# DeepGraphLearning/ultra_torchdrug

Measured on AMD Instinct MI355X. Metric: edges aggregated/sec, FB15k237-shaped 6L x 64d rspmm Bellman-Ford (predict: the reference's 18 rspmm layers per batch as 6 relation-graph + 6 entity-graph launches, tails and heads in one pass), higher is better.
Workload: dtype f32

## Files before the change

### include/ultra_rspmm.h

```cpp
#ifndef ULTRA_RSPMM_H
#define ULTRA_RSPMM_H

#include <stddef.h>
#include <stdint.h>

#ifdef __cplusplus
extern "C" {
#endif
#pragma GCC visibility push(default)

#define ULTRA_RSPMM_ABI_VERSION 8

enum ultra_sum_op { ULTRA_SUM_ADD = 0, ULTRA_SUM_MIN = 1, ULTRA_SUM_MAX = 2 };
enum ultra_mul_op { ULTRA_MUL_MUL = 0, ULTRA_MUL_ADD = 1 };

enum ultra_status {
    ULTRA_OK = 0,
    ULTRA_ERR_BAD_OP = 1,
    ULTRA_ERR_BAD_SHAPE = 2,
    ULTRA_ERR_NULL_POINTER = 3,
    ULTRA_ERR_WORKSPACE = 4,
    ULTRA_ERR_HIP = 5,
    ULTRA_ERR_NO_DEVICE = 6,
    ULTRA_ERR_ABI = 7
// ... 172 lines not shown
                                void *stream);

int ultra_candidate_tiles(const int64_t *t_index, int64_t n_batch, int64_t per_row, int64_t n_query, int64_t n_rows, int32_t *out,
                          void *stream);

int ultra_gather_boundary_rows_f32(const float *rows, const int32_t *node, int64_t n_query, float *out, void *stream);

int ultra_score_rows_forward_f32(const float *hidden, const float *query, const int64_t *t_index, const float *w1, const float *b1,
                                 const float *w2, const float *b2, float *h, float *in_rows, float *score, int64_t n_batch,
                                 int64_t per_row, void *stream);
int ultra_score_rows_backward_f32(const float *hidden, const float *query, const int64_t *t_index, const float *w1, const float *w2,
                                  const float *h, const float *in_rows, const float *grad, float *d_pre, float *partial,
                                  float *d_hidden, float *d_query, float *d_w1, float *d_b1, float *d_w2, float *d_b2,
                                  int64_t n_node, int64_t n_batch, int64_t per_row, void *stream);

int ultra_statistics_blocks(int64_t n_a);
int ultra_statistics_f32(const float *a, int64_t n_a, const float *b, int64_t n_b, int64_t b_repeat, double *partials,
                         float *out, void *stream);

int ultra_bce_adversarial_f32(const float *pred, int64_t rows, int64_t cols, float temperature, float *loss_rows,
                              float *dpred, void *stream);

int ultra_relation_project_backward_blocks(int device, int64_t batch, int64_t n_rel, int64_t n_layers, int64_t *blocks);
int ultra_relation_project_backward_f32(const float *relation, const float *const *w1, const float *const *b1,
                                        const float *const *w2, const float *const *grad, float *d_relation_layers,
                                        float *const *d_w1, float *const *d_b1, float *const *d_w2, float *const *d_b2,
                                        void *workspace, size_t workspace_bytes, int64_t n_layers, int64_t batch,
                                        int64_t n_rel, int64_t dim, void *stream);

int ultra_filtered_rank(const float *pred, int64_t n_query, int64_t n_cand, int64_t row_stride, const int64_t *target,
                        const int32_t *filt_ptr, const int32_t *filt_node, int64_t *rank, void *stream);


int ultra_filtered_rank_keys(const float *pred, int64_t n_query, int64_t n_cand, int64_t row_stride, const int64_t *target,
                             int64_t target_stride, const int64_t *keys, int64_t n_keys, const int64_t *anchor,
                             const int64_t *rel, int64_t index_stride, int64_t n_rel, int64_t *rank, int64_t rank_stride,
                             void *stream);
int ultra_strict_negative(const int64_t *keys, int64_t n_keys, const int64_t *anchor, const int64_t *rel, int64_t n_query,
                          int64_t n_rel, int64_t n_node, const float *rand, int64_t n_sample, int64_t *out, void *stream);
int ultra_edge_removal_weights(const ultra_segments *fwd, const ultra_segments *by_src, const ultra_segments *by_rel,
                               const int64_t *h, const int64_t *t, const int64_t *r, int64_t n_pattern,
                               int64_t n_base_rel, float *w_fwd, float *w_src, float *w_rel, int64_t slack, void *stream);
int ultra_edge_removal_marks(const ultra_segments *fwd, const ultra_segments *by_src, const ultra_segments *by_rel,
                             const int64_t *h, const int64_t *t, const int64_t *r, int64_t n_pattern, int64_t n_base_rel,
                             float *w_fwd, float *w_src, float *w_rel, int64_t slack, uint32_t *words_fwd, uint32_t *words_src,
                             uint32_t *words_rel, int64_t n_node, void *stream);


size_t ultra_relcsr_coalesce_temp_bytes(int64_t n_edges);
int ultra_relcsr_coalesce(const int64_t *row, const int64_t *col, const int64_t *rel, const float *weight,
                          int64_t n_edges, int64_t n_rows, int64_t n_cols, int64_t n_rel, int32_t *out_row,
                          int32_t *out_col, int32_t *out_rel, float *out_weight, int64_t *edge_of_input,
                          int64_t *n_unique_host, int *unit_weight_host, void *temp, size_t temp_bytes, void *stream);
size_t ultra_relcsr_plan_temp_bytes(int64_t n_edges, int64_t n_rows, int64_t piece_len);
int ultra_relcsr_plan(const int32_t *row, const int32_t *node_a, const int32_t *rel, int64_t n_edges, int64_t n_rows,
                      int64_t n_node_a, int64_t n_rel, int is_relation_plan, int wide_ids, int balance,
                      int64_t chunk_edges, int64_t chunk_rows, int64_t piece_len, int32_t *chunks,
                      int64_t cap_chunks, int32_t *long_rows, int64_t cap_long, int32_t *packed,
                      int64_t packed_slack, int64_t *counts_host, void *temp, size_t temp_bytes, void *stream);

size_t ultra_relcsr_dense_bytes(int64_t n_rows, int64_t n_cols, int kind);
int ultra_relcsr_dense(const ultra_segments *plan, int64_t n_rows, int64_t n_cols, int kind, uint32_t *dense, void *stream);

int ultra_dense_layer_supported(const ultra_segments *fwd, int64_t n_query);
int ultra_dense_layer_forward_f32(const ultra_segments *fwd, const float *relation, const float *input,
                                  const int32_t *boundary_node, const float *boundary_value, int64_t n_query, const float *weight,
                                  const float *bias, const float *ln_weight, const float *ln_bias, float ln_eps, int relu,
                                  int shortcut, float *out, void *stream);

int ultra_layer_forward_supported(const ultra_segments *fwd, int64_t n_query, int64_t n_rel);
int ultra_layer_forward_f32(const ultra_segments *fwd, const float *relation, const float *input, const int32_t *boundary_node,
                            const float *boundary_value, int64_t n_query, const float *weight, const float *bias,
                            const float *ln_weight, const float *ln_bias, float ln_eps, int relu, int shortcut, float *out,
                            int64_t n_rel, void *stream);

int ultra_second_layer_sources(const int32_t *col, int64_t n_edges, int64_t slack, const int32_t *row_list, const int32_t *list_count,
                               int64_t list_len, int64_t n_query, int64_t n_node, uint32_t *bitmap, int32_t *c_node,
                               int32_t *sources, void *stream);
int ultra_layer_forward_sources_f32(const ultra_segments *fwd, const int32_t *sources, const float *relation, const float *input,
                                    const int32_t *boundary_node, const float *boundary_value, int64_t n_query, const float *weight,
                                    const float *bias, const float *ln_weight, const float *ln_bias, float ln_eps, int relu,
                                    int shortcut, float *out, int64_t n_rel, void *stream);

int ultra_layer_score_supported(const ultra_segments *fwd, int64_t n_query, int64_t n_rel);
int ultra_layer_score_forward_f32(const ultra_segments *fwd, const float *relation, const float *input, const int32_t *boundary_node,
                                  const float *boundary_value, int64_t n_query, const float *weight, const float *bias,
                                  const float *ln_weight, const float *ln_bias, float ln_eps, int relu, int shortcut,
                                  const float *query, const float *w1, const float *b1, const float *w2, const float *b2,
                                  float *qbias, float *score, int64_t n_rel, void *stream);

int ultra_relation_graph_marks(const int32_t *head_ptr, const int32_t *head_rel, const int32_t *tail_ptr, const int32_t *tail_rel,
                               int64_t n_node, int64_t n_rel, uint8_t *marks, void *stream);

int ultra_calibrate_gather_f32(const float *table, int64_t n_rows, const int32_t *index, int64_t n_index, float *out,
                               int64_t *n_waves_host, void *stream);

#pragma GCC visibility pop
#ifdef __cplusplus
}
#endif
#endif
```

### ultra_torchdrug_amd/_lib.py

```python
import ctypes
import os

_HERE = os.path.dirname(os.path.abspath(__file__))
LIB_PATH = os.environ.get("ULTRA_RSPMM_LIB") or os.path.join(_HERE, "libultra_rspmm.so")
ABI_VERSION = 8

SUM_OPS = {"add": 0, "min": 1, "max": 2}
MUL_OPS = {"mul": 0, "add": 1}


class UltraSegments(ctypes.Structure):
    _fields_ = [
        ("struct_bytes", ctypes.c_uint32),
        ("abi_version", ctypes.c_uint32),
        ("n_rows", ctypes.c_int64),
        ("n_edges", ctypes.c_int64),
        ("row", ctypes.c_void_p),
        ("node_a", ctypes.c_void_p),
        ("node_b", ctypes.c_void_p),
        ("rel", ctypes.c_void_p),
        ("weight", ctypes.c_void_p),
        ("n_chunks", ctypes.c_int64),
        ("chunks", ctypes.c_void_p),
        ("n_long_rows", ctypes.c_int64),
# ... 11 lines not shown
        ("packed_dead", ctypes.c_void_p),
    ]

    def __init__(self, *args, **kwargs):
        super().__init__(*args, **kwargs)
        if not self.struct_bytes:
            self.struct_bytes = ctypes.sizeof(type(self))
        if not self.abi_version:
            self.abi_version = ABI_VERSION


EXPORTS = (
    "ultra_rspmm_abi_version",
    "ultra_segments_bytes",
    "ultra_rspmm_status_string",
    "ultra_rspmm_last_hip_error",
    "ultra_rspmm_device_info",
    "ultra_rspmm_profile_next",
    "ultra_rspmm_event_create",
    "ultra_rspmm_event_destroy",
    "ultra_rspmm_event_elapsed_ms",
    "ultra_rspmm_force_general_path",
    "ultra_rspmm_reserve_cus",
    "ultra_rspmm_workspace_bytes",
    "ultra_rspmm_forward_f32",
    "ultra_rspmm_fwd_f32",
    "ultra_rspmm_forward_boundary_f32",
    "ultra_rspmm_frontier_f32",
    "ultra_first_layer_sparse_supported",
    "ultra_first_layer_sparse_f32",
    "ultra_rspmm_backward_boundary_rows_f32",
    "ultra_rspmm_backward_boundary_rows_workspace",
    "ultra_rspmm_backward_f32",
    "ultra_rspmm_backward_accumulate_f32",
    "ultra_rspmm_backward_weight_f32",
    "ultra_beam_search_step_f32",
    "ultra_rspmm_backward_active_f32",
    "ultra_node_bitmap",
    "ultra_rspmm_drelation_boundary_f32",
    "ultra_combine_forward_f32",
    "ultra_combine_forward_boundary_f32",
    "ultra_combine_backward_waves",
    "ultra_combine_backward_f32",
    "ultra_combine_dxdu_f32",
    "ultra_combine_backward_fused_waves",
    "ultra_combine_backward_fused_f32",
    "ultra_linear_forward_f32",
    "ultra_score_forward_f32",
    "ultra_relation_project_f32",
    "ultra_relation_project_backward_blocks",
    "ultra_relation_project_backward_f32",
    "ultra_filtered_rank",
    "ultra_filtered_rank_keys",
    "ultra_strict_negative",
    "ultra_edge_removal_weights",
    "ultra_edge_removal_marks",
    "ultra_prepare_queries",
    "ultra_relation_stack_inputs",
    "ultra_statistics_blocks",
    "ultra_statistics_f32",
    "ultra_bce_adversarial_f32",
    "ultra_candidate_tiles",
    "ultra_score_rows_forward_f32",
    "ultra_score_rows_backward_f32",
    "ultra_gather_boundary_rows_f32",
    "ultra_relcsr_coalesce_temp_bytes",
    "ultra_relcsr_coalesce",
    "ultra_relcsr_plan_temp_bytes",
    "ultra_relcsr_plan",
    "ultra_relcsr_dense_bytes",
    "ultra_relcsr_dense",
    "ultra_relation_graph_marks",
    "ultra_calibrate_gather_f32",
    "ultra_first_layer_sparse_train_f32",
    "ultra_first_layer_epilogue_backward_workspace",
    "ultra_first_layer_epilogue_backward_f32",
    "ultra_column_sum_blocks",
    "ultra_column_sum_f32",
    "ultra_dense_layer_supported",
    "ultra_dense_layer_forward_f32",
    "ultra_layer_forward_supported",
    "ultra_layer_forward_f32",
    "ultra_second_layer_sources",
    "ultra_layer_forward_sources_f32",
    "ultra_layer_score_supported",
    "ultra_layer_score_forward_f32",
)

_lib = None


class UltraLibraryError(RuntimeError):
    pass


def load():
    global _lib
    if _lib is not None:
        return _lib
    if not os.path.exists(LIB_PATH):
        raise UltraLibraryError(
            "%s not found: build it with `make -C ultra_torchdrug_amd/csrc` (hipcc --offload-arch=gfx950) or "
            "`python -c 'import __graft_entry__ as g; g.build()'`. There is no CPU/PyTorch fallback." % LIB_PATH)
    try:
        lib = ctypes.CDLL(LIB_PATH)
    except OSError as err:
        raise UltraLibraryError("cannot load %s: %s" % (LIB_PATH, err)) from err
    missing = [name for name in EXPORTS if not hasattr(lib, name)]
    if missing:
        raise UltraLibraryError("%s lacks symbols %s" % (LIB_PATH, missing))

    vp, i64, i32, sz = ctypes.c_void_p, ctypes.c_int64, ctypes.c_int, ctypes.c_size_t
    seg = ctypes.POINTER(UltraSegments)
    lib.ultra_rspmm_abi_version.restype = i32
    lib.ultra_rspmm_abi_version.argtypes = []
    lib.ultra_layer_forward_supported.restype = i32
    lib.ultra_layer_forward_supported.argtypes = [seg, i64, i64]
    lib.ultra_layer_forward_f32.restype = i32
    lib.ultra_layer_forward_f32.argtypes = [seg, vp, vp, vp, vp, i64, vp, vp, vp, vp, ctypes.c_float, i32, i32, vp, i64, vp]
    lib.ultra_second_layer_sources.restype = i32
    lib.ultra_second_layer_sources.argtypes = [vp, i64, i64, vp, vp, i64, i64, i64, vp, vp, vp, vp]
    lib.ultra_layer_forward_sources_f32.restype = i32
    lib.ultra_layer_forward_sources_f32.argtypes = [seg, vp, vp, vp, vp, vp, i64, vp, vp, vp, vp, ctypes.c_float, i32, i32, vp, i64, vp]
    lib.ultra_layer_score_supported.restype = i32
    lib.ultra_layer_score_supported.argtypes = [seg, i64, i64]
    lib.ultra_layer_score_forward_f32.restype = i32
    lib.ultra_layer_score_forward_f32.argtypes = [seg, vp, vp, vp, vp, i64, vp, vp, vp, vp, ctypes.c_float, i32, i32, vp, vp, vp, vp,
                                                  vp, vp, vp, i64, vp]
    lib.ultra_relation_graph_marks.restype = i32
    lib.ultra_relation_graph_marks.argtypes = [vp, vp, vp, vp, i64, i64, vp, vp]
    lib.ultra_segments_bytes.restype = sz
    lib.ultra_segments_bytes.argtypes = []
    lib.ultra_rspmm_status_string.restype = ctypes.c_char_p
    lib.ultra_rspmm_status_string.argtypes = [i32]
    lib.ultra_rspmm_last_hip_error.restype = i32
    lib.ultra_rspmm_last_hip_error.argtypes = []
    lib.ultra_rspmm_device_info.restype = i32
    lib.ultra_rspmm_device_info.argtypes = [i32, ctypes.POINTER(i32), ctypes.POINTER(i32), ctypes.c_char_p, sz]
    lib.ultra_rspmm_profile_next.restype = i32
    lib.ultra_rspmm_profile_next.argtypes = [vp, vp]
    lib.ultra_rspmm_event_create.restype = i32
    lib.ultra_rspmm_event_create.argtypes = [ctypes.POINTER(vp)]
    lib.ultra_rspmm_event_destroy.restype = i32
    lib.ultra_rspmm_event_destroy.argtypes = [vp]
    lib.ultra_rspmm_event_elapsed_ms.restype = i32
    lib.ultra_rspmm_event_elapsed_ms.argtypes = [vp, vp, ctypes.POINTER(ctypes.c_float)]
    lib.ultra_rspmm_force_general_path.restype = i32
    lib.ultra_rspmm_force_general_path.argtypes = [i32]
    lib.ultra_rspmm_reserve_cus.restype = i32
    lib.ultra_rspmm_reserve_cus.argtypes = [i32]
    lib.ultra_rspmm_workspace_bytes.restype = sz
    lib.ultra_rspmm_workspace_bytes.argtypes = [seg, i64]
    lib.ultra_rspmm_forward_f32.restype = i32
    lib.ultra_rspmm_forward_f32.argtypes = [seg, vp, vp, vp, vp, vp, sz, i64, i64, i64, i32, i32, vp]
    lib.ultra_rspmm_fwd_f32.restype = i32
    lib.ultra_rspmm_fwd_f32.argtypes = [vp, vp, vp, vp, vp, vp, vp, i64, i64, i64, i64, i32, i32, vp]
    lib.ultra_rspmm_forward_boundary_f32.restype = i32
    lib.ultra_rspmm_forward_boundary_f32.argtypes = [seg, vp, vp, vp, vp, i64, vp, vp, sz, i64, i64, i64, i32, i32, vp]
    lib.ultra_rspmm_backward_boundary_rows_f32.restype = i32
    lib.ultra_rspmm_backward_boundary_rows_f32.argtypes = [seg, vp, vp, vp, vp, vp, vp, sz, i64, i64, i64, i32, vp]
    lib.ultra_rspmm_backward_boundary_rows_workspace.restype = sz
    lib.ultra_rspmm_backward_boundary_rows_workspace.argtypes = [i64]
    lib.ultra_rspmm_frontier_f32.restype = i32
    lib.ultra_rspmm_frontier_f32.argtypes = [seg, vp, vp, vp, vp, vp, i64, vp, i64, i64, i64, vp]
    lib.ultra_first_layer_sparse_supported.restype = i32
    lib.ultra_first_layer_sparse_supported.argtypes = [i64, i64, i64]
    lib.ultra_first_layer_sparse_f32.restype = i32
    lib.ultra_first_layer_sparse_f32.argtypes = [seg, vp, vp, vp, vp, vp, vp, i64, vp, vp, vp, vp, ctypes.c_float, i32, i32, vp, vp, i64, i64,
                                                 vp, i64, i64, vp]
    lib.ultra_rspmm_backward_f32.restype = i32
    lib.ultra_rspmm_backward_f32.argtypes = [seg, seg, vp, vp, vp, vp, vp, vp, vp, sz, i64, i64, i64, i64, i32, i32, vp]
    lib.ultra_rspmm_backward_accumulate_f32.restype = i32
    lib.ultra_rspmm_backward_accumulate_f32.argtypes = [seg, seg, vp, vp, vp, vp, vp, vp, vp, vp, sz, i64, i64, i64, i64, i32,
                                                        i32, vp]
    lib.ultra_rspmm_backward_active_f32.restype = i32
    lib.ultra_rspmm_backward_active_f32.argtypes = [seg, seg, vp, vp, vp, vp, vp, vp, vp, sz, i64, i64, i64, i64, i32, vp, i64, vp, vp]
    lib.ultra_node_bitmap.restype = i32
    lib.ultra_node_bitmap.argtypes = [vp, i64, i64, i64, vp, vp]
    lib.ultra_rspmm_drelation_boundary_f32.restype = i32
    lib.ultra_rspmm_drelation_boundary_f32.argtypes = [seg, vp, i64, vp, vp, vp, vp, vp, vp, vp, sz, i64, i64, i64, vp]
    lib.ultra_rspmm_backward_weight_f32.restype = i32
    lib.ultra_rspmm_backward_weight_f32.argtypes = [seg, vp, vp, vp, vp, vp, i64, i64, i32, i32, vp]
    lib.ultra_beam_search_step_f32.restype = i32
    lib.ultra_beam_search_step_f32.argtypes = [vp, vp, vp, vp, i64, i64, i64, i64, vp, vp, vp, vp]
    lib.ultra_combine_forward_f32.restype = i32
    lib.ultra_combine_forward_f32.argtypes = [vp, vp, vp, vp, vp, vp, ctypes.c_float, i32, i32, vp, vp, i64, i64, vp]
    lib.ultra_combine_forward_boundary_f32.restype = i32
    lib.ultra_combine_forward_boundary_f32.argtypes = [vp, vp, i64, vp, vp, vp, vp, vp, ctypes.c_float, i32, i32, vp, i64, i64, vp]
    lib.ultra_prepare_queries.restype = i32
    lib.ultra_prepare_queries.argtypes = [vp, vp, i64, i64, i64, i64, i64, vp, vp, vp, vp, vp]
    lib.ultra_statistics_blocks.restype = i32
    lib.ultra_statistics_blocks.argtypes = [i64]
    lib.ultra_statistics_f32.restype = i32
    lib.ultra_statistics_f32.argtypes = [vp, i64, vp, i64, i64, vp, vp, vp]
    lib.ultra_gather_boundary_rows_f32.restype = i32
    lib.ultra_gather_boundary_rows_f32.argtypes = [vp, vp, i64, vp, vp]
    lib.ultra_score_rows_forward_f32.restype = i32
    lib.ultra_score_rows_forward_f32.argtypes = [vp] * 10 + [i64, i64, vp]
    lib.ultra_score_rows_backward_f32.restype = i32
    lib.ultra_score_rows_backward_f32.argtypes = [vp] * 16 + [i64, i64, i64, vp]
    lib.ultra_candidate_tiles.restype = i32
    lib.ultra_candidate_tiles.argtypes = [vp, i64, i64, i64, i64, vp, vp]
    lib.ultra_bce_adversarial_f32.restype = i32
    lib.ultra_bce_adversarial_f32.argtypes = [vp, i64, i64, ctypes.c_float, vp, vp, vp]
# ... 90 lines not shown
```

### ultra_torchdrug_amd/csrc/frontier.inc

```

struct FrontierParams {
    const int32_t *src_ptr;
    const int32_t *dst;
    const int32_t *rel;
    const float *weight;
    const int32_t *fwd_rank;
    const float *relation;
    const int32_t *bnode;
    const float *bvec;
    float *out;
    long long F;
    int piece_len;
    int slices;
    int n_rel;
    int piece_shift;
    const int32_t *run_prefix;
    int32_t *row_list;
    const int32_t *list_offset;
    int list_len;
};

constexpr int kFrontierThreads = 256;
constexpr int kFrontierU = 4;

// ... 229 lines not shown
        r = p.rel[eu];
        k = p.fwd_rank[eu];
        w = 1.0f;
        if constexpr (!UNIT_W) w = p.weight[eu];
    };
    const int bp = (lane & 48) * 4;
    const int grp_shift = (lane >> 4) * 16;
    auto from = [&](int u, int v) -> int { return __builtin_amdgcn_ds_bpermute(bp + 4 * u, v); };

    int nd, nr, nk;
    float nw;
    load_ids(e, nd, nr, nk, nw);
    bool done = false;
    while (!done) {
        const int md = nd, mr = nr, mk = nk;
        const float mw = nw;
        load_ids(e + 16, nd, nr, nk, nw);
        const int mp = p.piece_shift >= 0 ? (mk >> p.piece_shift) : (mk / p.piece_len);
        const int prev_d = __builtin_amdgcn_update_dpp(cur, md, 0x111, 0xf, 0xf, false);
        const int prev_p = __builtin_amdgcn_update_dpp(cur_piece, mp, 0x111, 0xf, 0xf, false);
        const int n_valid = min(16, hi - e);
        const bool starts_run = (md != prev_d) && sub < n_valid;
        const bool starts_piece = (starts_run || mp != prev_p) && sub < n_valid;
        const uint32_t run_bits = (uint32_t)(__builtin_amdgcn_ballot_w64(starts_run) >> grp_shift) & 0xffffu;
        const uint32_t piece_bits = (uint32_t)(__builtin_amdgcn_ballot_w64(starts_piece) >> grp_shift) & 0xffffu;
        const int room = end - e;
        const uint32_t beyond = room >= 16 ? 0u : (room <= 0 ? 0xffffu : (0xffffu << room) & 0xffffu);
        const uint32_t stop_bits = run_bits & beyond;
        const int n_sum = min(n_valid, stop_bits ? __builtin_ctz(stop_bits) : 16);
        done = n_sum < 16;
#pragma unroll
        for (int half = 0; half < 2; ++half) {
            qf4 y[8];
#pragma unroll
            for (int v = 0; v < 8; ++v) {
                const int u = 8 * half + v;
                y[v] = msg[from(u, mr) * 16];
                if constexpr (!UNIT_W) y[v] = __builtin_bit_cast(float, from(u, __builtin_bit_cast(int, mw))) * y[v];
            }
            const uint32_t any = (run_bits | piece_bits) >> (8 * half) & 0xffu;
            if (any == 0u && n_sum >= 8 * half + 8) {
#pragma unroll
                for (int v = 0; v < 8; ++v) piece = piece + y[v];
                continue;
            }
#pragma unroll
            for (int v = 0; v < 8; ++v) {
                const int u = 8 * half + v;
                if (u < n_sum) {
                    if ((run_bits >> u) & 1u) {
                        close_run(u == 0 ? cur : from(u - 1, md));
                        have_total = false;
                        open = false;
                    }
                    if ((piece_bits >> u) & 1u) {
                        close_piece();
                        open = true;
                        piece = qf4{0.0f, 0.0f, 0.0f, 0.0f};
                    }
                    piece = piece + y[v];
                }
            }
        }
        if (n_sum > 0) {
            cur = from(n_sum - 1, md);
            cur_piece = from(n_sum - 1, mp);
        }
        e += 16;
    }
    close_run(cur);
}

constexpr int kSparseMaxQueries = 128;
struct ConstFillParams {
    qf4 *out;
    long long n4;
    const float *bias, *gamma, *beta;
    float eps;
    int relu, shortcut;
    const int32_t *src_ptr, *run_prefix, *bnode;
    int n_query;
    int list_len;
    int32_t *list_offset;
};

__global__ __launch_bounds__(256) void const_fill_kernel(const ConstFillParams p) {
    __shared__ __attribute__((aligned(16))) float c[64];
    __shared__ int slots[kSparseMaxQueries];
    if (threadIdx.x < 64) {
        const int j = threadIdx.x;
        float v = p.bias[j];
        if (p.gamma != nullptr) {
            float s0 = 0.0f, s1 = 0.0f;
            for (int k = 0; k < 32; ++k) { s0 = s0 + p.bias[k]; s1 = s1 + p.bias[32 + k]; }
            const float mean = (s0 + s1) * (1.0f / 64.0f);
            float q0 = 0.0f, q1 = 0.0f;
            for (int k = 0; k < 32; ++k) {
                const float d0 = p.bias[k] - mean, d1 = p.bias[32 + k] - mean;
                q0 = q0 + d0 * d0;
                q1 = q1 + d1 * d1;
            }
            const float var = (q0 + q1) * (1.0f / 64.0f);
            const float inv = 1.0f / sqrtf(var + p.eps);
            v = ((v - mean) * inv) * p.gamma[j] + p.beta[j];
        }
        if (p.relu) v = !(v <= 0.0f) ? v : 0.0f;
        c[j] = p.shortcut ? v + 0.0f : v;
    }
    if (blockIdx.x == 0) {
        if ((int)threadIdx.x < p.n_query) {
            const int h = p.bnode[threadIdx.x];
            const int lo = p.src_ptr[h], hi = p.src_ptr[h + 1];
            slots[threadIdx.x] = (hi > lo ? p.run_prefix[hi - 1] - p.run_prefix[lo] + 1 : 0) + 1;
        }
        __syncthreads();
        if (threadIdx.x == 0) {
            int total = 0;
            for (int b = 0; b < p.n_query; ++b) {
                p.list_offset[b] = total;
                total += slots[b];
            }
            p.list_offset[p.n_query] = total;
        }
    }
    __syncthreads();
    const qf4 *c4 = reinterpret_cast<const qf4 *>(c);
    for (long long i = (long long)blockIdx.x * 256 + threadIdx.x; i < p.n4; i += (long long)gridDim.x * 256) p.out[i] = c4[i & 15];
}

__global__ __launch_bounds__(256) void zero_fill_kernel(qf4 *out, long long n4) {
    const qf4 zero = {0.0f, 0.0f, 0.0f, 0.0f};
    for (long long i = (long long)blockIdx.x * 256 + threadIdx.x; i < n4; i += (long long)gridDim.x * 256) out[i] = zero;
}

struct BoundaryRowsParams {
    const int32_t *src_ptr;
    const int32_t *dst;
    const int32_t *rel;
    const float *weight;
    const float *relation;
    const float *grad;
    const int32_t *bnode;
    float *partial;
    float *d_input;
    long long F;
};

constexpr int kBRowsSlices = 64;
constexpr int kBRowsWaves = kBRowsSlices * 4;

template <bool UNIT_W, bool HAS_REL>
__global__ __launch_bounds__(256) void boundary_rows_partial_kernel(const BoundaryRowsParams p) {
    const int lane = threadIdx.x & 63;
    const int g = blockIdx.x * 4 + uniform(threadIdx.x >> 6);
    const int q = blockIdx.y;
    const int u = uniform(p.bnode[q]);
    const int lo = uniform(p.src_ptr[u]), hi = uniform(p.src_ptr[u + 1]);
    const int per = (hi - lo + kBRowsWaves - 1) / kBRowsWaves;
    const int a = lo + g * per;
    const int z = a + per < hi ? a + per : hi;
    const long long col = (long long)q * 64 + lane;
    float acc = 0.0f;
    auto ids = [&](int e0, int &v, int &r, float &wt) {
        int e = e0 + (lane & 7);
        e = e < z ? e : z - 1;
        v = p.dst[e];
        r = 0;
        if constexpr (HAS_REL) r = p.rel[e];
        wt = 1.0f;
        if constexpr (!UNIT_W) wt = p.weight[e];
    };
    int v = 0, r = 0;
    float wt = 1.0f;
    if (a < z) ids(a, v, r, wt);
    for (int e0 = a; e0 < z; e0 += 8) {
        int v_next = 0, r_next = 0;
        float wt_next = 1.0f;
        if (e0 + 8 < z) ids(e0 + 8, v_next, r_next, wt_next);
        float gr[8], rr[8];
#pragma unroll
        for (int k = 0; k < 8; ++k) {
            const long long vk = __builtin_amdgcn_readlane(v, k);
            gr[k] = p.grad[vk * p.F + col];
            rr[k] = 1.0f;
            if constexpr (HAS_REL) rr[k] = p.relation[(long long)__builtin_amdgcn_readlane(r, k) * p.F + col];
        }
#pragma unroll
        for (int k = 0; k < 8; ++k) {
            if (e0 + k < z) {
                float y = gr[k];
                if constexpr (!UNIT_W) y = y * __builtin_bit_cast(float, __builtin_amdgcn_readlane(__builtin_bit_cast(int, wt), k));
                if constexpr (HAS_REL) y = y * rr[k];
                acc = acc + y;
            }
        }
        v = v_next; r = r_next; wt = wt_next;
    }
    p.partial[((long long)q * kBRowsWaves + g) * 64 + lane] = acc;
}

__global__ __launch_bounds__(64) void boundary_rows_reduce_kernel(const BoundaryRowsParams p) {
    const int lane = threadIdx.x;
    const int q = blockIdx.x;
    const float *part = p.partial + (long long)q * kBRowsWaves * 64 + lane;
    float total = 0.0f;
#pragma unroll 16
    for (int g = 0; g < kBRowsWaves; ++g) total = total + part[g * 64];
    float *dst = p.d_input + (long long)p.bnode[q] * p.F + (long long)q * 64 + lane;
    *dst = *dst + total;
}
// ... 1 lines not shown
```

### ultra_torchdrug_amd/csrc/quad.inc

```
#ifndef ULTRA_QUAD_WORD_AUX
#define ULTRA_QUAD_WORD_AUX 0
#endif
#ifndef ULTRA_QUAD_STORE_AUX
#define ULTRA_QUAD_STORE_AUX 2
#endif
#ifndef ULTRA_QUAD_DEDUP
#define ULTRA_QUAD_DEDUP 0
#endif
typedef float qf4 __attribute__((ext_vector_type(4)));
typedef uint32_t qu4 __attribute__((ext_vector_type(4)));
typedef __attribute__((address_space(3))) const qf4 *lds_qf4_ptr;
typedef __attribute__((address_space(3))) char *lds_char_ptr;

__device__ __forceinline__ qf4 lds_read4(uint32_t byte_addr) { return *(lds_qf4_ptr)byte_addr; }

template <int RED>
__device__ __forceinline__ qf4 reduce4(qf4 a, qf4 y) {
    if constexpr (RED == ULTRA_SUM_ADD) {
        return a + y;
    } else {
        qf4 r;
        r.x = reduce<RED>(a.x, y.x); r.y = reduce<RED>(a.y, y.y); r.z = reduce<RED>(a.z, y.z); r.w = reduce<RED>(a.w, y.w);
        return r;
    }
}

template <int RED>
__device__ __forceinline__ qf4 identity4() {
    const float v = identity<RED>();
    qf4 r = {v, v, v, v};
    return r;
}

typedef __attribute__((address_space(3))) const uint32_t *lds_u32_ptr;
__device__ __forceinline__ uint32_t lds_read1(uint32_t byte_addr) { return *(lds_u32_ptr)byte_addr; }

template <int KIND, int SUM, int MUL, bool UNIT_W, bool X_LDS, int U, int ACT = 0, bool DEAD = false>
__global__ __launch_bounds__(kBlock) void quad_kernel(const PParams p) {
    static_assert(KIND == KIND_FWD || SUM == ULTRA_SUM_ADD, "quad path: forward, or the backward of sum-aggregation");
    static_assert(!DEAD || (UNIT_W && !X_LDS && SUM == ULTRA_SUM_ADD && MUL == ULTRA_MUL_MUL && ACT != 1),
                  "marked words: unit weights, gathers through descriptors, summed DistMult messages");
    static_assert(ACT == 0 || (!X_LDS && ((KIND == KIND_DX && ACT == 1) || (KIND == KIND_DREL && (ACT == 2 || ACT == 3)))),
                  "activity masks: d_input by destination, d_relation by destination or by the tile's source node");
    constexpr int RED = (KIND == KIND_FWD) ? SUM : ULTRA_SUM_ADD;
    constexpr bool TWO_GATHERS = (KIND == KIND_DREL);
    constexpr bool DIRECT_WORDS = X_LDS && !TWO_GATHERS;
    constexpr bool NEEDS_REL = (KIND == KIND_FWD) || (KIND == KIND_DX && MUL == ULTRA_MUL_MUL);
    extern __shared__ __attribute__((aligned(16))) float lds_raw[];
    int *ticket = reinterpret_cast<int *>(lds_raw);
    float *lds_rel = lds_raw + kLdsHeader / sizeof(float);
    const int lane = threadIdx.x & 63;
    const int grp = lane >> 4;
    const uint32_t lane_bytes = (uint32_t)(lane & 15) * 16u;
    const int label = blockIdx.x % kXcd;
    const int conc = p.concurrent > 1 ? p.concurrent : 1;
    const int team = (int)(blockIdx.x / kXcd) % conc;
    const int bl = (int)(blockIdx.x / kXcd) / conc;
    const int nb = p.blocks_per_label / conc;
    const long long F = p.F;
    const __amdgpu_buffer_rsrc_t rsrc =
        __builtin_amdgcn_make_buffer_rsrc(const_cast<float *>(p.gather), 0, p.gather_bytes, 0x00020000);
    const __amdgpu_buffer_rsrc_t rsrc_meta =
        __builtin_amdgcn_make_buffer_rsrc(const_cast<uint32_t *>(p.meta), 0, p.meta_bytes, 0x00020000);
    const __amdgpu_buffer_rsrc_t rsrc2 =
        __builtin_amdgcn_make_buffer_rsrc(const_cast<float *>(TWO_GATHERS ? p.gather2 : p.gather), 0,
                                          TWO_GATHERS ? p.gather2_bytes : 0u, 0x00020000);
    const __amdgpu_buffer_rsrc_t rsrc_meta2 =
        __builtin_amdgcn_make_buffer_rsrc(const_cast<uint32_t *>(TWO_GATHERS ? p.meta2 : p.meta), 0,
                                          TWO_GATHERS ? p.meta2_bytes : 0u, 0x00020000);
    const __amdgpu_buffer_rsrc_t rsrc_out = __builtin_amdgcn_make_buffer_rsrc(p.out, 0, p.out_bytes, 0x00020000);
    const __amdgpu_buffer_rsrc_t rsrc_add =
        __builtin_amdgcn_make_buffer_rsrc(const_cast<float *>(p.add_rows != nullptr ? p.add_rows : p.out), 0,
                                          p.add_rows != nullptr ? p.out_bytes : 0u, 0x00020000);
    const __amdgpu_buffer_rsrc_t rsrc_wt =
        __builtin_amdgcn_make_buffer_rsrc(const_cast<float *>(UNIT_W ? p.gather : p.weight), 0, UNIT_W ? 0u : p.meta_bytes, 0x00020000);
    if ((uint32_t)(uintptr_t)(lds_char_ptr)lds_raw != 0u) __builtin_trap();

    for (int s = label + kXcd * team; s < p.n_slots; s += kXcd * conc) {
        const int tile = s / p.split;
        const int part = s - tile * p.split;
        const long long col = (long long)tile * kTile + (lane & 15) * 4;
        const bool active = col < F;
        const uint32_t voff = (uint32_t)((active ? col : 0) * 4);
        float *lds_x = lds_rel + (NEEDS_REL ? p.n_rel * kTile : 0);
        if constexpr (NEEDS_REL) {
            const int total = p.n_rel * kTile;
            for (int i = threadIdx.x; i < total; i += kBlock) {
                const int r = i >> 6;
                const long long c = (long long)tile * kTile + (i & 63);
                lds_rel[i] = (c < F) ? p.relation[(long long)r * F + c] : 0.0f;
            }
        }
        if constexpr (X_LDS) {
            const int total = p.n_gather_rows * kTile;
            for (int i = threadIdx.x; i < total; i += kBlock) {
                const int r = i >> 6;
                const long long c = (long long)tile * kTile + (i & 63);
                lds_x[i] = (c < F) ? p.gather[(long long)r * F + c] : 0.0f;
            }
        }
        int b_node = -1;
        qf4 b_val = {0.0f, 0.0f, 0.0f, 0.0f};
        if (KIND == KIND_FWD && p.bnode != nullptr && active) {
            b_node = p.bnode[col / p.bdim];
            b_val = *reinterpret_cast<const qf4 *>(p.bvec + col);
        }
        int act_node = -1;
        if constexpr (ACT == 1 || ACT == 2) {
            uint32_t *lds_act = reinterpret_cast<uint32_t *>(lds_x);
            const uint32_t *bits = p.act_bits + (long long)tile * p.act_words;
            for (int i = threadIdx.x; i < p.act_words; i += kBlock) lds_act[i] = bits[i];
        }
        if constexpr (ACT == 3) act_node = p.act_node[tile];
        if (threadIdx.x == 0) *ticket = 0;
        __syncthreads();
        const uint32_t rel_base = (uint32_t)kLdsHeader;
        const uint32_t x_base = rel_base + (NEEDS_REL ? (uint32_t)p.n_rel * 256u : 0u);
        auto dead = [&](uint32_t key) -> uint32_t {
            if constexpr (ACT == 1 || ACT == 2) return ((lds_read1(x_base + (key >> 5) * 4u) >> (key & 31u)) & 1u) ? 0u : 0xffffffffu;
            if constexpr (ACT == 3) return (int)key == act_node ? 0u : 0xffffffffu;
            return 0u;
        };

        for (;;) {
            int t = 0;
            if (lane == 0) t = __hip_atomic_fetch_add(ticket, 1, __ATOMIC_RELAXED, __HIP_MEMORY_SCOPE_WORKGROUP);
            t = uniform(t);
            const int k_first = part + p.split * (4 * t * nb + bl);
            if (k_first >= p.n_chunks) break;
            const int q = 4 * t + grp;
            const int k = part + p.split * (q * nb + ((q & 1) ? (nb - 1 - bl) : bl));
            const bool has = k < p.n_chunks;
            int4 d = {0, 0, 0, 0};
            if (has) d = p.chunks[k];
            const int n = d.y - d.x;
            const uint32_t e_begin = (uint32_t)d.x;
            const bool is_piece = d.w < 0;
            const int row_base = d.z;
            const int n01 = max(__builtin_amdgcn_readlane(n, 0), __builtin_amdgcn_readlane(n, 16));
            const int n23 = max(__builtin_amdgcn_readlane(n, 32), __builtin_amdgcn_readlane(n, 48));
            const int m01 = min(__builtin_amdgcn_readlane(n, 0), __builtin_amdgcn_readlane(n, 16));
            const int m23 = min(__builtin_amdgcn_readlane(n, 32), __builtin_amdgcn_readlane(n, 48));
            const int n_max = uniform(max(n01, n23)), n_min = uniform(min(m01, m23));
            const uint32_t e_bytes = e_begin * 4u;

            uint32_t cur = 0;
            qf4 acc = identity4<RED>();
            const bool adds = (KIND != KIND_DREL) && p.add_rows != nullptr;
            const bool sparse_b = (KIND == KIND_FWD) && p.add_rows == nullptr && p.bnode != nullptr;
            const uint32_t base_off = (uint32_t)row_base * p.row_bytes + voff;
            auto load_add = [&](uint32_t off) -> qf4 {
                return __builtin_bit_cast(qf4, __builtin_amdgcn_raw_buffer_load_b128(rsrc_add, off, 0, 0));
            };

            auto store_row = [&](uint32_t dl, qf4 v) {
                if (active) {
                    if (adds) v = reduce4<RED>(v, load_add(base_off + __umul24(dl, p.row_bytes)));
                    if (sparse_b) v = reduce4<RED>(v, (row_base + (int)dl == b_node) ? b_val : qf4{0.0f, 0.0f, 0.0f, 0.0f});
                    __builtin_amdgcn_raw_buffer_store_b128(__builtin_bit_cast(qu4, v), rsrc_out, base_off + __umul24(dl, p.row_bytes), 0, ULTRA_QUAD_STORE_AUX);
                }
            };
            auto store_empty = [&](uint32_t dl) {
                if (active) {
                    const uint32_t off = base_off + dl * p.row_bytes;
                    qf4 v = identity4<RED>();
                    if (adds) v = reduce4<RED>(v, load_add(off));
                    if (sparse_b) v = reduce4<RED>(v, (row_base + (int)dl == b_node) ? b_val : qf4{0.0f, 0.0f, 0.0f, 0.0f});
                    __builtin_amdgcn_raw_buffer_store_b128(__builtin_bit_cast(qu4, v), rsrc_out, off, 0, ULTRA_QUAD_STORE_AUX);
                }
            };
            auto contribute = [&](qf4 a, qf4 rv, qf4 gv, float w) -> qf4 {
                if constexpr (KIND == KIND_FWD) {
                    qf4 y;
                    if constexpr (MUL == ULTRA_MUL_MUL) y = rv * gv; else y = rv + gv;
                    if constexpr (!UNIT_W) y = w * y;
                    return reduce4<RED>(a, y);
                } else {
                    qf4 c = gv;
                    if constexpr (!UNIT_W) c = c * w;
                    if constexpr (MUL == ULTRA_MUL_MUL) c = c * rv;
                    return a + c;
                }
            };
            const float ident = identity<RED>();
            auto next_row = [&](uint32_t dl) {
                store_row(cur, acc);
                for (uint32_t r = cur + 1; r < dl; ++r) store_empty(r);
                asm volatile("v_mov_b32 %0, %1" : "+v"(cur) : "v"(dl));
                asm volatile("v_mov_b32 %0, %1" : "+v"(acc.x) : "v"(ident));
                asm volatile("v_mov_b32 %0, %1" : "+v"(acc.y) : "v"(ident));
                asm volatile("v_mov_b32 %0, %1" : "+v"(acc.z) : "v"(ident));
                asm volatile("v_mov_b32 %0, %1" : "+v"(acc.w) : "v"(ident));
            };

            const uint32_t lane_word = (uint32_t)min(lane & 15, U - 1) * 4u;
            const int bp_base = (lane & 48) * 4;
            auto load_compact = [&](int i, uint32_t &m, uint32_t &m2) {
                const uint32_t off = e_bytes + (uint32_t)i * 4u + lane_word;
                m = __builtin_amdgcn_raw_buffer_load_b32(rsrc_meta, off, 0, ULTRA_QUAD_WORD_AUX);
                m2 = 0;
                if constexpr (TWO_GATHERS) m2 = __builtin_amdgcn_raw_buffer_load_b32(rsrc_meta2, off, 0, 0);
            };
            auto distribute = [&](uint32_t m, uint32_t m2, uint32_t (&w)[U], uint32_t (&w2)[U]) {
#pragma unroll
                for (int u = 0; u < U; ++u) {
                    w[u] = (uint32_t)__builtin_amdgcn_ds_bpermute(bp_base + 4 * u, (int)m);
                    w2[u] = 0;
                    if constexpr (TWO_GATHERS) w2[u] = (uint32_t)__builtin_amdgcn_ds_bpermute(bp_base + 4 * u, (int)m2);
                }
            };
            auto load_words = [&](int i, uint32_t (&w)[U], uint32_t (&w2)[U]) {
                const uint32_t w_off = e_bytes + (uint32_t)i * 4u;
#pragma unroll
                for (int u = 0; u < U; ++u) {
                    w[u] = __builtin_amdgcn_raw_buffer_load_b32(rsrc_meta, w_off + 4u * u, 0, ULTRA_QUAD_WORD_AUX);
                    w2[u] = 0;
                }
            };
            uint32_t wn[U], w2n[U];
            uint32_t mw = 0, mw2 = 0;
            constexpr bool DEDUP = ULTRA_QUAD_DEDUP && !TWO_GATHERS && !X_LDS && ACT == 0 && !DEAD;
            uint32_t prev_node = 0xffffffffu;
            qu4 prev_x = {0u, 0u, 0u, 0u};
            if constexpr (DIRECT_WORDS) {
                load_words(0, wn, w2n);
            } else {
                load_compact(0, mw, mw2);
                distribute(mw, mw2, wn, w2n);
                load_compact(U, mw, mw2);
            }

            auto batch = [&](auto tail_tag, int i) {
                constexpr bool TAIL = decltype(tail_tag)::value;
                uint32_t w[U], w2[U];
                float wt[U];
                qf4 xv[U], rv[U];
                uint32_t killm[U];
#pragma unroll
                for (int u = 0; u < U; ++u) { w[u] = wn[u]; w2[u] = w2n[u]; killm[u] = 0u; }
#pragma unroll
                for (int u = 0; u < U; ++u) {
                    const uint32_t node = w[u] >> p.src_shift;
                    if constexpr (TWO_GATHERS) {
                        uint32_t kill = 0u;
                        if constexpr (ACT == 2) kill = dead(w2[u]);
                        if constexpr (ACT == 3) kill = dead(node);
                        if constexpr (DEAD) kill |= (uint32_t)((int32_t)w[u] >> 31);
                        xv[u] = __builtin_bit_cast(qf4, __builtin_amdgcn_raw_buffer_load_b128(
                                                            rsrc2, (__umul24(w2[u], p.row_bytes) + voff) | kill, 0, 0));
                        rv[u] = qf4{0.0f, 0.0f, 0.0f, 0.0f};
                        if constexpr (MUL == ULTRA_MUL_MUL) {
                            if constexpr (X_LDS)
                                rv[u] = lds_read4(((node << 8) | lane_bytes) + x_base);
                            else
                                rv[u] = __builtin_bit_cast(qf4, __builtin_amdgcn_raw_buffer_load_b128(
                                                                    rsrc, (__umul24(node, p.row_bytes) + voff) | kill, 0, 0));
                        }
                        continue;
                    }
                    if constexpr (X_LDS) {
                        xv[u] = lds_read4(((node << 8) | lane_bytes) + x_base);
                    } else {
                        uint32_t kill = 0u;
                        if constexpr (ACT == 1) kill = dead(node);
                        if constexpr (DEAD) kill = (uint32_t)((int32_t)w[u] >> 31);
                        if constexpr (DEDUP) {
                            const uint32_t before = (u == 0) ? prev_node : (w[u > 0 ? u - 1 : 0] >> p.src_shift);
                            kill = (node == before) ? 0xffffffffu : 0u;
                            killm[u] = kill;
                        }
                        xv[u] = __builtin_bit_cast(qf4, __builtin_amdgcn_raw_buffer_load_b128(
                                                            rsrc, (__umul24(node, p.row_bytes) + voff) | kill, 0, 0));
                    }
                    if constexpr (NEEDS_REL)
                        rv[u] = lds_read4(((w[u] & p.rel_mask) | lane_bytes) + rel_base);
                    else
                        rv[u] = qf4{0.0f, 0.0f, 0.0f, 0.0f};
                }
                if constexpr (!UNIT_W && !DIRECT_WORDS) {
                    const int mine = (int)__builtin_amdgcn_raw_buffer_load_b32(rsrc_wt, e_bytes + (uint32_t)i * 4u + lane_word, 0, 0);
#pragma unroll
                    for (int u = 0; u < U; ++u) wt[u] = __builtin_bit_cast(float, __builtin_amdgcn_ds_bpermute(bp_base + 4 * u, mine));
                } else {
#pragma unroll
                    for (int u = 0; u < U; ++u) {
                        wt[u] = 1.0f;
                        if constexpr (!UNIT_W)
                            wt[u] = __builtin_bit_cast(float, __builtin_amdgcn_raw_buffer_load_b32(
                                                                  rsrc_wt, e_bytes + (uint32_t)i * 4u + 4u * u, 0, 0));
                    }
                }
                if constexpr (DIRECT_WORDS) {
                    if (i + U < n_max) load_words(i + U, wn, w2n);
                } else {
                    const uint32_t m = mw, m2 = mw2;
                    load_compact(i + 2 * U, mw, mw2);
                    distribute(m, m2, wn, w2n);
                }
                if constexpr (DEDUP) {
#pragma unroll
                    for (int u = 0; u < U; ++u) {
                        const qu4 before = (u == 0) ? prev_x : __builtin_bit_cast(qu4, xv[u > 0 ? u - 1 : 0]);
                        const qu4 got = __builtin_bit_cast(qu4, xv[u]);
                        qu4 v;
                        v.x = (before.x & killm[u]) | got.x; v.y = (before.y & killm[u]) | got.y;
                        v.z = (before.z & killm[u]) | got.z; v.w = (before.w & killm[u]) | got.w;
                        xv[u] = __builtin_bit_cast(qf4, v);
                    }
                    prev_x = __builtin_bit_cast(qu4, xv[U - 1]);
                    prev_node = w[U - 1] >> p.src_shift;
                }
                bool same_row = false;
                if constexpr (!TAIL) same_row = __builtin_amdgcn_ballot_w64((w[U - 1] & 0xffu) != cur) == 0ull;
                if (same_row) {
#pragma unroll
                    for (int u = 0; u < U; ++u) acc = contribute(acc, rv[u], xv[u], wt[u]);
                } else {
#pragma unroll
                    for (int u = 0; u < U; ++u) {
                        const bool valid = !TAIL || (i + u < n);
                        const uint32_t dl = w[u] & 0xffu;
                        if (valid) {
                            if (dl != cur) next_row(dl);
                            acc = contribute(acc, rv[u], xv[u], wt[u]);
                        }
                    }
                }
            };

            int i = 0;
            for (; i + U <= n_min; i += U) batch(std::false_type{}, i);
            for (; i < n_max; i += U) batch(std::true_type{}, i);

            if (has) {
                if (is_piece) {
                    if (active) *reinterpret_cast<qf4 *>(p.partial + (long long)(-d.w - 1) * F + col) = acc;
                } else {
                    store_row(cur, acc);
                    for (uint32_t r = cur + 1; r < (uint32_t)(d.w - row_base); ++r) store_empty(r);
                }
            }
        }
        __syncthreads();
    }
}
```

### ultra_torchdrug_amd/csrc/rspmm_kernels.hip

```cpp
#include <hip/hip_runtime.h>
#include <type_traits>

#include <algorithm>
#include <cstdint>
#include <cstdlib>
#include <cstring>
#include <mutex>

#include "relgraph_dense.h"
#include "ultra_rspmm.h"

thread_local int ultra_detail_last_hip_error = 0;

namespace {

constexpr int kTile = 64;
#ifndef ULTRA_BLOCK
#define ULTRA_BLOCK 1024
#endif
constexpr int kBlock = ULTRA_BLOCK;
#ifndef ULTRA_UNROLL
#define ULTRA_UNROLL 8
#endif
constexpr int kUnroll = ULTRA_UNROLL;
#ifndef ULTRA_UNROLL_BIG
#define ULTRA_UNROLL_BIG 8
#endif
#ifndef ULTRA_BIG_GATHER_AUX
#define ULTRA_BIG_GATHER_AUX 0
#endif
constexpr int kUnrollBig = ULTRA_UNROLL_BIG;
constexpr int kXcd = 8;
constexpr int kFixUnroll = 16;
constexpr int kMaxLdsBytes = 156 * 1024;
constexpr int kLdsHeader = 16;

enum Kind { KIND_FWD = 0, KIND_DX = 1, KIND_DREL = 2 };

struct KParams {
    const int32_t *row;
    const int32_t *node_a;
    const int32_t *node_b;
    const int32_t *rel;
    const float *weight;
    const int4 *chunks;
    const float *relation;
    const float *input;
    const float *output;
    const float *grad;
    const float *add_rows;
    const int32_t *bnode;
    const float *bvec;
    int bdim;
    float *out;
    float *partial;
    long long F;
    int n_chunks;
    int n_rel;
    int n_tiles;
    int split;
    int n_slots;
    int blocks_per_label;
    const uint32_t *act_bits;
    int act_words;
    const int32_t *act_node;
};

struct FixParams {
    const int32_t *long_rows;
    const float *partial;
    const float *add_rows;
    const int32_t *bnode;
    const float *bvec;
    int bdim;
    float *out;
    long long F;
    int n_long;
    int n_tiles;
};

template <int SUM>
__device__ __forceinline__ float identity() {
    if constexpr (SUM == ULTRA_SUM_ADD) return 0.0f;
    else if constexpr (SUM == ULTRA_SUM_MIN) return 3.402823466e+38f;
    else return -3.402823466e+38f;
}

template <int SUM>
__device__ __forceinline__ float reduce(float acc, float y) {
    if constexpr (SUM == ULTRA_SUM_ADD) return acc + y;
    else if constexpr (SUM == ULTRA_SUM_MIN) return (y < acc) ? y : acc;
    else return (y > acc) ? y : acc;
}

template <int MUL>
__device__ __forceinline__ float binary(float r, float x) {
    if constexpr (MUL == ULTRA_MUL_MUL) return r * x;
    else return r + x;
}

__device__ __forceinline__ int uniform(int v) { return __builtin_amdgcn_readfirstlane(v); }

template <int KIND, int SUM, int MUL, bool UNIT_W, bool REL_LDS>
struct ChunkWalker {
    static constexpr int RED = (KIND == KIND_FWD) ? SUM : ULTRA_SUM_ADD;
    static constexpr bool MASKED = (KIND != KIND_FWD) && (SUM != ULTRA_SUM_ADD);
    static constexpr bool NEED_REL_ID = (KIND == KIND_FWD) || (KIND == KIND_DX && (MASKED || MUL == ULTRA_MUL_MUL));

    const KParams &p;
    const long long F;
    const long long col;
    const long long lcol;
    const bool active;
    const float *lds_rel;
    const int lane;
    int cur;
    float acc;
    bool is_piece;

    __device__ __forceinline__ float load_rel(int r) const {
        if constexpr (REL_LDS) return lds_rel[r * kTile + lane];
        else return p.relation[(long long)r * F + lcol];
    }
    __device__ __forceinline__ void store_row(int r, float v) const {
        if (active) {
            if constexpr (KIND != KIND_DREL) {
                if (p.add_rows != nullptr) v = reduce<RED>(v, p.add_rows[(long long)r * F + col]);
                else if (KIND == KIND_FWD && p.bnode != nullptr) v = reduce<RED>(v, (r == p.bnode[col / p.bdim]) ? p.bvec[col] : 0.0f);
            }
            p.out[(long long)r * F + col] = v;
        }
    }

    template <bool FULL>
    __device__ __forceinline__ void batch(const int e0, const int n) {
        int ia[kUnroll], ib[kUnroll], ir[kUnroll], irow[kUnroll];
        float wv[kUnroll];
        float v0[kUnroll], v1[kUnroll], v2[kUnroll];
#pragma unroll
        for (int u = 0; u < kUnroll; ++u) {
            const int e = FULL ? e0 + u : e0 + min(u, n - 1);
            ia[u] = p.node_a[e];
            irow[u] = p.row[e];
            if constexpr (NEED_REL_ID) ir[u] = p.rel[e];
            if constexpr (KIND == KIND_DREL) ib[u] = p.node_b[e];
            if constexpr (!UNIT_W) wv[u] = p.weight[e];
        }
#pragma unroll
// ... 60 lines not shown
            store_row(cur, acc);
            for (int q = cur + 1; q < d.w; ++q) store_row(q, identity<RED>());
        }
    }
};

template <int KIND, int SUM, int MUL, bool UNIT_W, bool REL_LDS>
__global__ __launch_bounds__(kBlock) void segment_kernel(const KParams p) {
    extern __shared__ __attribute__((aligned(16))) float lds_raw[];
    int *ticket = reinterpret_cast<int *>(lds_raw);
    float *lds_rel = lds_raw + kLdsHeader / sizeof(float);
    const int lane = threadIdx.x & 63;
    const int label = blockIdx.x % kXcd;
    const int bl = blockIdx.x / kXcd;
    const int nb = p.blocks_per_label;

    for (int s = label; s < p.n_slots; s += kXcd) {
        const int tile = s / p.split;
        const int part = s - tile * p.split;
        const long long col = (long long)tile * kTile + lane;
        const bool active = col < p.F;
        if constexpr (REL_LDS) {
            const int total = p.n_rel * kTile;
            for (int i = threadIdx.x; i < total; i += kBlock) {
                const int r = i >> 6;
                const long long c = (long long)tile * kTile + (i & 63);
                lds_rel[i] = (c < p.F) ? p.relation[(long long)r * p.F + c] : 0.0f;
            }
        }
        if (threadIdx.x == 0) *ticket = 0;
        __syncthreads();
        for (;;) {
            int t = 0;
            if (lane == 0) t = __hip_atomic_fetch_add(ticket, 1, __ATOMIC_RELAXED, __HIP_MEMORY_SCOPE_WORKGROUP);
            t = uniform(t);
            const int k = part + p.split * (t * nb + ((t & 1) ? (nb - 1 - bl) : bl));
            if (k >= p.n_chunks) break;
            const int4 d = p.chunks[uniform(k)];
            ChunkWalker<KIND, SUM, MUL, UNIT_W, REL_LDS> walker{p, p.F, col, active ? col : p.F - 1, active, lds_rel, lane,
                                                                0, 0.0f, false};
            walker.run(d);
        }
        __syncthreads();
    }
}

struct PParams {
    const uint32_t *meta;
    const uint32_t *meta2;
    const float *weight;
    const int4 *chunks;
    const float *relation;
    const float *gather;
    const float *gather2;
    const float *add_rows;
    const int32_t *bnode;
    const float *bvec;
    int bdim;
    float *out;
    float *partial;
    long long F;
    uint32_t gather_bytes;
    uint32_t meta_bytes;
    uint32_t meta2_bytes;
    uint32_t out_bytes;
    uint32_t gather2_bytes;
    uint32_t relation_bytes;
    int n_gather_rows;
    const int32_t *hot_nodes;
    int n_hot;
    uint32_t row_bytes;
    uint32_t src_shift;
    uint32_t rel_mask;
    int n_chunks;
    int n_rel;
    int n_tiles;
    int split;
    int n_slots;
    int blocks_per_label;
    int concurrent;
    const uint32_t *act_bits;
    int act_words;
    const int32_t *act_node;
};

template <int KIND, int SUM, int MUL, bool UNIT_W, int VAR, int UN = kUnroll>
__global__ __launch_bounds__(kBlock) void packed_kernel(const PParams p) {
    constexpr bool X_LDS = (VAR == 1);
    constexpr bool BIG = (VAR == 2 || VAR == 3);
    constexpr bool REL_GLOBAL = (VAR == 2);
    constexpr bool HOT = (VAR == 4);
    static_assert(VAR == 0 || KIND != KIND_DREL, "variants 1-4 are for the single-gather kinds");
    static_assert(KIND == KIND_FWD || SUM == ULTRA_SUM_ADD, "packed path: forward, or the backward of sum-aggregation");
    constexpr int RED = (KIND == KIND_FWD) ? SUM : ULTRA_SUM_ADD;
    constexpr bool NEEDS_REL = (KIND == KIND_FWD) || (KIND == KIND_DX && MUL == ULTRA_MUL_MUL);
    constexpr bool TWO_GATHERS = (KIND == KIND_DREL);
    extern __shared__ __attribute__((aligned(16))) float lds_raw[];
    int *ticket = reinterpret_cast<int *>(lds_raw);
    float *lds_rel = lds_raw + kLdsHeader / sizeof(float);
    const int lane = threadIdx.x & 63;
    const int label = blockIdx.x % kXcd;
    const int bl = blockIdx.x / kXcd;
    const int nb = p.blocks_per_label;
    const long long F = p.F;
    const __amdgpu_buffer_rsrc_t rsrc =
        __builtin_amdgcn_make_buffer_rsrc(const_cast<float *>(p.gather), 0, p.gather_bytes, 0x00020000);
    const __amdgpu_buffer_rsrc_t rsrc2 =
        __builtin_amdgcn_make_buffer_rsrc(const_cast<float *>(TWO_GATHERS ? p.gather2 : p.gather), 0,
                                          TWO_GATHERS ? p.gather2_bytes : p.gather_bytes, 0x00020000);
    const __amdgpu_buffer_rsrc_t rsrc_rel =
        __builtin_amdgcn_make_buffer_rsrc(const_cast<float *>(p.relation), 0, p.relation_bytes, 0x00020000);

    for (int s = label; s < p.n_slots; s += kXcd) {
        const int tile = s / p.split;
        const int part = s - tile * p.split;
        const long long col = (long long)tile * kTile + lane;
        const bool active = col < F;
        const uint32_t voff = (uint32_t)((active ? col : F - 1) * 4);
        float *lds_x = lds_rel + (NEEDS_REL ? p.n_rel * kTile : 0);
        if constexpr (NEEDS_REL && !REL_GLOBAL) {
            const int total = p.n_rel * kTile;
            for (int i = threadIdx.x; i < total; i += kBlock) {
                const int r = i >> 6;
                const long long c = (long long)tile * kTile + (i & 63);
                lds_rel[i] = (c < F) ? p.relation[(long long)r * F + c] : 0.0f;
            }
        }
        if constexpr (X_LDS) {
            const int total = p.n_gather_rows * kTile;
            for (int i = threadIdx.x; i < total; i += kBlock) {
                const int r = i >> 6;
                const long long c = (long long)tile * kTile + (i & 63);
                lds_x[i] = (c < F) ? p.gather[(long long)r * F + c] : 0.0f;
            }
        }
        if constexpr (HOT) {
            const int total = p.n_hot * kTile;
            for (int i = threadIdx.x; i < total; i += kBlock) {
                const long long r = p.hot_nodes[i >> 6];
                const long long c = (long long)tile * kTile + (i & 63);
                lds_x[i] = (c < F) ? p.gather[r * F + c] : 0.0f;
            }
        }
        if (threadIdx.x == 0) *ticket = 0;
        __syncthreads();
        const char *lds_lane = reinterpret_cast<const char *>(lds_rel) + lane * 4;
        const char *lds_x_lane = reinterpret_cast<const char *>(lds_x) + lane * 4;
        auto gather_one = [&](uint32_t word) -> float {
            if constexpr (X_LDS) {
                return *reinterpret_cast<const float *>(lds_x_lane + ((word >> p.src_shift) << 8));
            } else if constexpr (HOT) {
                const uint32_t g = word >> p.src_shift;
                if (g < (uint32_t)p.n_hot) return *reinterpret_cast<const float *>(lds_x_lane + (g << 8));
                return __builtin_bit_cast(float, __builtin_amdgcn_raw_buffer_load_b32(
                                                     rsrc, voff, (g - (uint32_t)p.n_hot) * p.row_bytes, 0));
            } else {
                return __builtin_bit_cast(float, __builtin_amdgcn_raw_buffer_load_b32(
                                                     rsrc, voff, (word >> p.src_shift) * p.row_bytes, 0));
            }
        };

        int b_node = -1;
        float b_val = 0.0f;
        if (KIND == KIND_FWD && p.bnode != nullptr && active) {
            b_node = p.bnode[col / p.bdim];
            b_val = p.bvec[col];
// ... 157 lines not shown
    const int row = p.long_rows[lr * 3 + 0];
    const int first = p.long_rows[lr * 3 + 1];
    const int n = p.long_rows[lr * 3 + 2];
    float acc = identity<RED>();
    for (int k0 = 0; k0 < n; k0 += UN) {
        float v[UN];
#pragma unroll
        for (int u = 0; u < UN; ++u) {
            const int k = min(k0 + u, n - 1);
            v[u] = p.partial[(long long)(first + k) * p.F + col];
        }
#pragma unroll
        for (int u = 0; u < UN; ++u)
            if (k0 + u < n) acc = reduce<RED>(acc, v[u]);
    }
    if (p.add_rows != nullptr) acc = reduce<RED>(acc, p.add_rows[(long long)row * p.F + col]);
    else if (p.bnode != nullptr) acc = reduce<RED>(acc, (row == p.bnode[col / p.bdim]) ? p.bvec[col] : 0.0f);
    p.out[(long long)row * p.F + col] = acc;
}

#include "quad.inc"
#include "frontier.inc"
#include "rowgroup.inc"

template <int SUM, int MUL, bool UNIT_W>
__global__ __launch_bounds__(256) void weight_grad_kernel(const int32_t *row, const int32_t *src, const int32_t *rel,
                                                          const float *weight, const float *relation,
                                                          const float *input, const float *output, const float *grad,
                                                          float *d_weight, long long F, long long n_edges) {
    const int lane = threadIdx.x & 63;
    const long long waves_total = ((long long)gridDim.x * blockDim.x) >> 6;
    long long e = ((long long)blockIdx.x * blockDim.x + threadIdx.x) >> 6;
    for (; e < n_edges; e += waves_total) {
        const int v = row[e], u = src[e], r = rel[e];
        float wk = 1.0f;
        if constexpr (!UNIT_W) wk = weight[e];
        float acc = 0.0f;
        for (long long f = lane; f < F; f += 64) {
            const float m = binary<MUL>(relation[(long long)r * F + f], input[(long long)u * F + f]);
            float g = grad[(long long)v * F + f];
            if constexpr (SUM != ULTRA_SUM_ADD) {
                float y = m;
                if constexpr (!UNIT_W) y = wk * m;
                g = g * ((output[(long long)v * F + f] == y) ? 1.0f : 0.0f);
            }
            acc = acc + g * m;
        }
#pragma unroll
        for (int off = 32; off > 0; off >>= 1) acc += __shfl_down(acc, off, 64);
        if (lane == 0) d_weight[e] = acc;
    }
}


constexpr int kCbRows = 32;
constexpr int kCbStride = 132;
constexpr int kCbWaves = 4;
constexpr int kCbTileFloats = kCbRows * kCbStride;
constexpr int kCbLdsQueries = 128;
static_assert(kCbLdsQueries == kSparseMaxQueries, "const_fill_kernel lays out one slot range per LDS-resident query");

typedef float f32x4 __attribute__((ext_vector_type(4)));
typedef float f32x16 __attribute__((ext_vector_type(16)));

struct CombineParams {
    const float *input;
    const float *update;
    const float *weight;
    const float *bias;
    const float *gamma;
    const float *beta;
    float *out;
    long long rows;
    float eps;
    int relu;
    int shortcut;
    float *z_out;
    const int32_t *in_bnode;
    const float *in_bvec;
    int rpn;
    const int32_t *row_list;
    const int32_t *list_count;
    int list_len;
};

template <bool PF, int BND = 0, bool ZOUT = false>
__global__ __launch_bounds__(kCbWaves * 64, PF ? 1 : 2) void combine_kernel(const CombineParams p) {
    extern __shared__ __attribute__((aligned(16))) float cb_lds[];
    const int lane = threadIdx.x & 63;
    const int wl = uniform(threadIdx.x >> 6);
    float *tile = cb_lds + wl * kCbTileFloats;
    const int i = lane & 31, h = lane >> 5;
    int n_list = 0;
    if constexpr (BND == 3) n_list = min(uniform(p.list_count[0]), p.list_len);
    const long long n_tiles = BND == 3 ? ((long long)n_list + kCbRows - 1) / kCbRows : (p.rows + kCbRows - 1) / kCbRows;
    const long long wave_global = (long long)blockIdx.x * kCbWaves + wl;
    const long long wave_total = (long long)gridDim.x * kCbWaves;

    float w0[64], w1[64];
#pragma unroll
    for (int q = 0; q < 16; ++q) {
        const f32x4 a = *reinterpret_cast<const f32x4 *>(p.weight + (long long)i * 128 + 64 * h + 4 * q);
        const f32x4 b = *reinterpret_cast<const f32x4 *>(p.weight + (long long)(i + 32) * 128 + 64 * h + 4 * q);
        w0[4 * q + 0] = a.x; w0[4 * q + 1] = a.y; w0[4 * q + 2] = a.z; w0[4 * q + 3] = a.w;
        w1[4 * q + 0] = b.x; w1[4 * q + 1] = b.y; w1[4 * q + 2] = b.z; w1[4 * q + 3] = b.w;
    }
    const float bias0 = p.bias[i], bias1 = p.bias[i + 32];
    const int ln_row = lane >> 1, ln_half = lane & 1;
    float *gb = cb_lds + kCbWaves * kCbTileFloats;
    if (p.gamma != nullptr && threadIdx.x < 128) gb[threadIdx.x] = threadIdx.x < 64 ? p.gamma[threadIdx.x] : p.beta[threadIdx.x - 64];
    float *bv_lds = gb + 128;
    int *bn_lds = reinterpret_cast<int *>(bv_lds + (size_t)p.rpn * 64);
    if constexpr (BND == 1 || BND == 3) {
        for (int j = threadIdx.x; j < p.rpn; j += kCbWaves * 64) bn_lds[j] = p.in_bnode[j];
        for (int j = threadIdx.x; j < p.rpn * 16; j += kCbWaves * 64)
            reinterpret_cast<f32x4 *>(bv_lds)[j] = reinterpret_cast<const f32x4 *>(p.in_bvec)[j];
    }
    __syncthreads();

    const long long last = p.rows - 1;
    f32x4 pa[8], pb[8];
    int rid[8];
    auto fetch = [&](long long t) {
        if constexpr (BND == 3) {
#pragma unroll
            for (int q = 0; q < 8; ++q) {
                const int r = 4 * q + (lane >> 4), c = (lane & 15) * 4;
                const long long slot = t * kCbRows + r;
                int row = slot < n_list ? p.row_list[slot] : -1;
                if ((long long)row >= p.rows) row = -1;
                rid[q] = row;
                const unsigned gr = row >= 0 ? (unsigned)row : 0u;
                const unsigned node = gr / (unsigned)p.rpn, query = gr - node * (unsigned)p.rpn;
                const f32x4 zero = {0.0f, 0.0f, 0.0f, 0.0f};
                const f32x4 v = *reinterpret_cast<const f32x4 *>(bv_lds + query * 64 + c);
                pa[q] = ((int)node == bn_lds[query]) ? v : zero;
                pb[q] = *reinterpret_cast<const f32x4 *>(p.update + (long long)gr * 64 + c);
            }
            return;
        }
        long long node0 = 0;
        int query0 = 0;
        if constexpr (BND != 0) {
            node0 = (t * kCbRows) / p.rpn;
            query0 = (int)(t * kCbRows - node0 * p.rpn);
        }
#pragma unroll
        for (int q = 0; q < 8; ++q) {
            const int r = 4 * q + (lane >> 4), c = (lane & 15) * 4;
            long long gr = t * kCbRows + r;
            gr = gr < last ? gr : last;
            if constexpr (BND == 0) {
                pa[q] = *reinterpret_cast<const f32x4 *>(p.input + gr * 64 + c);
            } else {
                const unsigned qq = (unsigned)(query0 + r);
                const unsigned step = p.rpn >= kCbRows ? (qq >= (unsigned)p.rpn ? 1u : 0u) : qq / (unsigned)p.rpn;
                const int query = (int)(qq - step * (unsigned)p.rpn);
                const f32x4 zero = {0.0f, 0.0f, 0.0f, 0.0f};
                if constexpr (BND == 1) {
                    const f32x4 v = *reinterpret_cast<const f32x4 *>(bv_lds + query * 64 + c);
                    pa[q] = (node0 + step == (long long)bn_lds[query]) ? v : zero;
                } else {
                    pa[q] = (node0 + step == (long long)p.in_bnode[query]) ? *reinterpret_cast<const f32x4 *>(p.in_bvec + query * 64 + c) : zero;
                }
            }
            pb[q] = *reinterpret_cast<const f32x4 *>(p.update + gr * 64 + c);
        }
    };
    if constexpr (PF) {
        if (wave_global < n_tiles) fetch(wave_global);
    }
    for (long long t = wave_global; t < n_tiles; t += wave_total) {
        const long long row0 = t * kCbRows;
        if constexpr (!PF) fetch(t);
#pragma unroll
        for (int q = 0; q < 8; ++q) {
            const int r = 4 * q + (lane >> 4), c = (lane & 15) * 4;
            *reinterpret_cast<f32x4 *>(tile + r * kCbStride + c) = pa[q];
            *reinterpret_cast<f32x4 *>(tile + r * kCbStride + 64 + c) = pb[q];
        }
        if constexpr (PF) {
            asm volatile("s_waitcnt lgkmcnt(0)" ::: "memory");
            if (t + wave_total < n_tiles) fetch(t + wave_total);
        } else {
            asm volatile("s_waitcnt vmcnt(0) lgkmcnt(0)" ::: "memory");
        }

        f32x16 acc0, acc1;
#pragma unroll
        for (int r = 0; r < 16; ++r) { acc0[r] = bias0; acc1[r] = bias1; }
#pragma unroll
        for (int q = 0; q < 16; ++q) {
            const f32x4 av = *reinterpret_cast<const f32x4 *>(tile + i * kCbStride + 64 * h + 4 * q);
            acc0 = __builtin_amdgcn_mfma_f32_32x32x2f32(av.x, w0[4 * q + 0], acc0, 0, 0, 0);
            acc1 = __builtin_amdgcn_mfma_f32_32x32x2f32(av.x, w1[4 * q + 0], acc1, 0, 0, 0);
            acc0 = __builtin_amdgcn_mfma_f32_32x32x2f32(av.y, w0[4 * q + 1], acc0, 0, 0, 0);
            acc1 = __builtin_amdgcn_mfma_f32_32x32x2f32(av.y, w1[4 * q + 1], acc1, 0, 0, 0);
            acc0 = __builtin_amdgcn_mfma_f32_32x32x2f32(av.z, w0[4 * q + 2], acc0, 0, 0, 0);
            acc1 = __builtin_amdgcn_mfma_f32_32x32x2f32(av.z, w1[4 * q + 2], acc1, 0, 0, 0);
            acc0 = __builtin_amdgcn_mfma_f32_32x32x2f32(av.w, w0[4 * q + 3], acc0, 0, 0, 0);
            acc1 = __builtin_amdgcn_mfma_f32_32x32x2f32(av.w, w1[4 * q + 3], acc1, 0, 0, 0);
        }
        asm volatile("s_waitcnt lgkmcnt(0)" ::: "memory");

#pragma unroll
        for (int r = 0; r < 16; ++r) {
            const int row = (r & 3) + 8 * (r >> 2) + 4 * h;
            tile[row * kCbStride + 64 + i] = acc0[r];
            tile[row * kCbStride + 96 + i] = acc1[r];
        }
        asm volatile("s_waitcnt lgkmcnt(0)" ::: "memory");

        float v[32];
#pragma unroll
        for (int q = 0; q < 8; ++q) {
            const f32x4 d = *reinterpret_cast<const f32x4 *>(tile + ln_row * kCbStride + 64 + 32 * ln_half + 4 * q);
            v[4 * q + 0] = d.x; v[4 * q + 1] = d.y; v[4 * q + 2] = d.z; v[4 * q + 3] = d.w;
            if constexpr (ZOUT) {
                const long long left_z = p.rows - row0;
                const __amdgpu_buffer_rsrc_t rsrc_z = __builtin_amdgcn_make_buffer_rsrc(
                    p.z_out + row0 * 64, 0, (int)(left_z < kCbRows ? left_z : kCbRows) * 256, 0x00020000);
                __builtin_amdgcn_raw_buffer_store_b128(__builtin_bit_cast(qu4, d), rsrc_z, ln_row * 256 + ln_half * 128 + 16 * q, 0, 0);
            }
        }
        if (p.gamma != nullptr) {
            float s = 0.0f;
#pragma unroll
            for (int c = 0; c < 32; ++c) s = s + v[c];
            const float so = __shfl_xor(s, 1, 64);
            const float mean = (ln_half == 0 ? s + so : so + s) * (1.0f / 64.0f);
            float ss = 0.0f;
#pragma unroll
            for (int c = 0; c < 32; ++c) { const float dlt = v[c] - mean; ss = ss + dlt * dlt; }
            const float sso = __shfl_xor(ss, 1, 64);
            const float var = (ln_half == 0 ? ss + sso : sso + ss) * (1.0f / 64.0f);
            const float inv = 1.0f / sqrtf(var + p.eps);
#pragma unroll
            for (int q = 0; q < 8; ++q) {
                const f32x4 gq = *reinterpret_cast<const f32x4 *>(gb + 32 * ln_half + 4 * q);
                const f32x4 bq = *reinterpret_cast<const f32x4 *>(gb + 64 + 32 * ln_half + 4 * q);
                v[4 * q + 0] = ((v[4 * q + 0] - mean) * inv) * gq.x + bq.x;
                v[4 * q + 1] = ((v[4 * q + 1] - mean) * inv) * gq.y + bq.y;
                v[4 * q + 2] = ((v[4 * q + 2] - mean) * inv) * gq.z + bq.z;
                v[4 * q + 3] = ((v[4 * q + 3] - mean) * inv) * gq.w + bq.w;
            }
        }
        if (p.relu) {
#pragma unroll
            for (int c = 0; c < 32; ++c) v[c] = !(v[c] <= 0.0f) ? v[c] : 0.0f;
// ... 167 lines not shown
            if (rel_lds) return launch_instance<KIND, SUM, MUL, true, true>(p, grid, lds, stream);
            return launch_instance<KIND, SUM, MUL, true, false>(p, grid, lds, stream);
        }
        if (rel_lds) return launch_instance<KIND, SUM, MUL, false, true>(p, grid, lds, stream);
        return launch_instance<KIND, SUM, MUL, false, false>(p, grid, lds, stream);
    }
}

template <int KIND>
int launch_ops(const KParams &p, int sum_op, int mul_op, bool unit_w, bool rel_lds, int grid, size_t lds,
               hipStream_t stream) {
#define ULTRA_CASE(S, M)                                                    \
    if (sum_op == S && mul_op == M) return launch_wl<KIND, S, M>(p, unit_w, rel_lds, grid, lds, stream);
    ULTRA_CASE(ULTRA_SUM_ADD, ULTRA_MUL_MUL)
    ULTRA_CASE(ULTRA_SUM_ADD, ULTRA_MUL_ADD)
    ULTRA_CASE(ULTRA_SUM_MIN, ULTRA_MUL_MUL)
    ULTRA_CASE(ULTRA_SUM_MIN, ULTRA_MUL_ADD)
    ULTRA_CASE(ULTRA_SUM_MAX, ULTRA_MUL_MUL)
    ULTRA_CASE(ULTRA_SUM_MAX, ULTRA_MUL_ADD)
#undef ULTRA_CASE
    return ULTRA_ERR_BAD_OP;
}

inline bool segments_abi_ok(const ultra_segments *s) {
    return s->struct_bytes == (uint32_t)sizeof(ultra_segments) && s->abi_version == (uint32_t)ULTRA_RSPMM_ABI_VERSION;
}

int check_segments(const ultra_segments *s) {
    if (s == nullptr) return ULTRA_ERR_NULL_POINTER;
    if (!segments_abi_ok(s)) return ULTRA_ERR_ABI;
    if (s->n_rows < 0 || s->n_edges < 0 || s->n_chunks < 0 || s->n_pieces < 0 || s->n_long_rows < 0)
        return ULTRA_ERR_BAD_SHAPE;
    if (s->n_rows > 0x7fffffffLL || s->n_edges > 0x7fffffffLL || s->n_chunks > 0x7fffffffLL) return ULTRA_ERR_BAD_SHAPE;
    if (s->n_edges > 0 && (s->row == nullptr || s->node_a == nullptr || s->rel == nullptr)) return ULTRA_ERR_NULL_POINTER;
    if (s->n_chunks > 0 && s->chunks == nullptr) return ULTRA_ERR_NULL_POINTER;
    if (s->n_long_rows > 0 && s->long_rows == nullptr) return ULTRA_ERR_NULL_POINTER;
    return ULTRA_OK;
}

template <int KIND, int SUM, int MUL>
int launch_packed_w(const PParams &p, bool unit_w, int var, int grid, size_t lds, hipStream_t stream) {
#define ULTRA_VAR(V)                                                                                                  \
    if (var == V) {                                                                                                   \
        constexpr int UN = (V == 2 || V == 3) ? kUnrollBig : kUnroll;                                                 \
        if (unit_w) return launch_with_lds(packed_kernel<KIND, SUM, MUL, true, V, UN>, p, grid, lds, stream);        \
        return launch_with_lds(packed_kernel<KIND, SUM, MUL, false, V, UN>, p, grid, lds, stream);                   \
    }
    if constexpr (KIND != KIND_DREL) {
        ULTRA_VAR(1)
        ULTRA_VAR(2)
        ULTRA_VAR(3)
        ULTRA_VAR(4)
    }
    ULTRA_VAR(0)
#undef ULTRA_VAR
    return ULTRA_ERR_BAD_OP;
}

template <int KIND>
int launch_packed(const PParams &p, int sum_op, int mul_op, bool unit_w, int var, int grid, size_t lds,
                  hipStream_t stream) {
    if constexpr (KIND == KIND_FWD) {
#define ULTRA_PCASE(S, M) \
    if (sum_op == S && mul_op == M) return launch_packed_w<KIND_FWD, S, M>(p, unit_w, var, grid, lds, stream);
        ULTRA_PCASE(ULTRA_SUM_ADD, ULTRA_MUL_MUL)
        ULTRA_PCASE(ULTRA_SUM_ADD, ULTRA_MUL_ADD)
        ULTRA_PCASE(ULTRA_SUM_MIN, ULTRA_MUL_MUL)
        ULTRA_PCASE(ULTRA_SUM_MIN, ULTRA_MUL_ADD)
        ULTRA_PCASE(ULTRA_SUM_MAX, ULTRA_MUL_MUL)
        ULTRA_PCASE(ULTRA_SUM_MAX, ULTRA_MUL_ADD)
#undef ULTRA_PCASE
    } else if constexpr (KIND == KIND_DX) {
        if (mul_op == ULTRA_MUL_MUL) return launch_packed_w<KIND_DX, ULTRA_SUM_ADD, ULTRA_MUL_MUL>(p, unit_w, var, grid, lds, stream);
        return launch_packed_w<KIND_DX, ULTRA_SUM_ADD, ULTRA_MUL_ADD>(p, unit_w, var, grid, lds, stream);
    } else {
        if (mul_op == ULTRA_MUL_MUL) return launch_packed_w<KIND_DREL, ULTRA_SUM_ADD, ULTRA_MUL_MUL>(p, unit_w, 0, grid, kLdsHeader, stream);
        return launch_packed_w<KIND_DREL, ULTRA_SUM_ADD, ULTRA_MUL_ADD>(p, unit_w, 0, grid, kLdsHeader, stream);
    }
    return ULTRA_ERR_BAD_OP;
}

template <int KIND, int SUM, int MUL>
int launch_quad_w(const PParams &p, bool unit_w, bool x_lds, int grid, size_t lds, hipStream_t stream, bool dead = false) {
    if constexpr (SUM == ULTRA_SUM_ADD && MUL == ULTRA_MUL_MUL) {
        if (dead && !x_lds && p.act_node == nullptr) {
            if constexpr (KIND == KIND_DREL) {
                if (p.act_bits != nullptr)
                    return launch_with_lds(quad_kernel<KIND, SUM, MUL, true, false, kQuadU, 2, true>, p, grid, lds, stream);
            }
            return launch_with_lds(quad_kernel<KIND, SUM, MUL, true, false, kQuadU, 0, true>, p, grid, lds, stream);
        }
    }
    if constexpr (KIND == KIND_DREL) {
        if (p.act_bits != nullptr && !x_lds) {
            if (unit_w) return launch_with_lds(quad_kernel<KIND, SUM, MUL, true, false, kQuadU, 2>, p, grid, lds, stream);
            return launch_with_lds(quad_kernel<KIND, SUM, MUL, false, false, kQuadUW, 2>, p, grid, lds, stream);
        }
        if (p.act_node != nullptr && !x_lds) {
            if (unit_w) return launch_with_lds(quad_kernel<KIND, SUM, MUL, true, false, kQuadU, 3>, p, grid, lds, stream);
            return launch_with_lds(quad_kernel<KIND, SUM, MUL, false, false, kQuadUW, 3>, p, grid, lds, stream);
        }
    }
    if constexpr (KIND != KIND_DREL || MUL == ULTRA_MUL_MUL) {
        if (x_lds) {
            if (unit_w) return launch_with_lds(quad_kernel<KIND, SUM, MUL, true, true, kQuadUX>, p, grid, lds, stream);
            return launch_with_lds(quad_kernel<KIND, SUM, MUL, false, true, kQuadUW>, p, grid, lds, stream);
        }
    }
    if (unit_w) return launch_with_lds(quad_kernel<KIND, SUM, MUL, true, false, kQuadU>, p, grid, lds, stream);
    return launch_with_lds(quad_kernel<KIND, SUM, MUL, false, false, kQuadUW>, p, grid, lds, stream);
}

template <int KIND>
int launch_quad(const PParams &p, int sum_op, int mul_op, bool unit_w, bool x_lds, int grid, size_t lds,
                hipStream_t stream, bool dead = false) {
    if constexpr (KIND == KIND_FWD) {
#define ULTRA_QCASE(S, M) \
    if (sum_op == S && mul_op == M) return launch_quad_w<KIND_FWD, S, M>(p, unit_w, x_lds, grid, lds, stream, dead);
        ULTRA_QCASE(ULTRA_SUM_ADD, ULTRA_MUL_MUL)
        ULTRA_QCASE(ULTRA_SUM_ADD, ULTRA_MUL_ADD)
        ULTRA_QCASE(ULTRA_SUM_MIN, ULTRA_MUL_MUL)
        ULTRA_QCASE(ULTRA_SUM_MIN, ULTRA_MUL_ADD)
        ULTRA_QCASE(ULTRA_SUM_MAX, ULTRA_MUL_MUL)
        ULTRA_QCASE(ULTRA_SUM_MAX, ULTRA_MUL_ADD)
#undef ULTRA_QCASE
    } else if constexpr (KIND == KIND_DX) {
        if (mul_op == ULTRA_MUL_MUL) return launch_quad_w<KIND_DX, ULTRA_SUM_ADD, ULTRA_MUL_MUL>(p, unit_w, x_lds, grid, lds, stream, dead);
        return launch_quad_w<KIND_DX, ULTRA_SUM_ADD, ULTRA_MUL_ADD>(p, unit_w, x_lds, grid, lds, stream);
    } else {
        if (mul_op == ULTRA_MUL_MUL) return launch_quad_w<KIND_DREL, ULTRA_SUM_ADD, ULTRA_MUL_MUL>(p, unit_w, x_lds, grid, lds, stream, dead);
        return launch_quad_w<KIND_DREL, ULTRA_SUM_ADD, ULTRA_MUL_ADD>(p, unit_w, false, grid, p.act_bits != nullptr ? lds : (size_t)kLdsHeader, stream);
    }
    return ULTRA_ERR_BAD_OP;
}

template <int SUM, int MUL, bool BACKWARD, int G>
int launch_rowgroup_w(const RowGroupParams &p, bool unit_w, int rel, bool needs_rel, int grid, size_t lds,
                      hipStream_t stream) {
#define ULTRA_RG(UW, RL, NR) return launch_with_lds(rowgroup_kernel<SUM, MUL, UW, RL, NR, BACKWARD, G>, p, grid, lds, stream, kRgBlock)
    if (!needs_rel) {
        if (unit_w) ULTRA_RG(true, kRelL2, false);
        ULTRA_RG(false, kRelL2, false);
    }
    if (unit_w) {
        if (rel == kRelLds) ULTRA_RG(true, kRelLds, true);
        if (rel == kRelPart) ULTRA_RG(true, kRelPart, true);
        ULTRA_RG(true, kRelL2, true);
    }
    if (rel == kRelLds) ULTRA_RG(false, kRelLds, true);
    if (rel == kRelPart) ULTRA_RG(false, kRelPart, true);
    ULTRA_RG(false, kRelL2, true);
#undef ULTRA_RG
}

template <int G>
int launch_rowgroup_g(const RowGroupParams &p, bool backward, int sum_op, int mul_op, bool unit_w, int rel, int grid,
                      size_t lds, hipStream_t stream) {
    if (backward) {
        if (mul_op == ULTRA_MUL_MUL)
            return launch_rowgroup_w<ULTRA_SUM_ADD, ULTRA_MUL_MUL, true, G>(p, unit_w, rel, true, grid, lds, stream);
        return launch_rowgroup_w<ULTRA_SUM_ADD, ULTRA_MUL_ADD, true, G>(p, unit_w, kRelL2, false, grid, kLdsHeader, stream);
    }
#define ULTRA_RCASE(S, M) \
    if (sum_op == S && mul_op == M) return launch_rowgroup_w<S, M, false, G>(p, unit_w, rel, true, grid, lds, stream);
    ULTRA_RCASE(ULTRA_SUM_ADD, ULTRA_MUL_MUL)
    ULTRA_RCASE(ULTRA_SUM_ADD, ULTRA_MUL_ADD)
    ULTRA_RCASE(ULTRA_SUM_MIN, ULTRA_MUL_MUL)
    ULTRA_RCASE(ULTRA_SUM_MIN, ULTRA_MUL_ADD)
    ULTRA_RCASE(ULTRA_SUM_MAX, ULTRA_MUL_MUL)
    ULTRA_RCASE(ULTRA_SUM_MAX, ULTRA_MUL_ADD)
#undef ULTRA_RCASE
    return ULTRA_ERR_BAD_OP;
}

int launch_rowgroup(RowGroupParams &q, bool backward, int sum_op, int mul_op, bool unit_w, long long gather_rows, int n_cu,
                    hipStream_t stream) {
    const long long F = q.F;
    if (F >= (1LL << 30)) return ULTRA_ERR_BAD_SHAPE;
    const bool dram = g_wide_groups || (double)gather_rows * (double)F * 4.0 > 256.0 * 1024 * 1024;
    const int group = (dram && F % 256 == 0) ? 64 : ((dram && F % 128 == 0) ? 32 : 16);
    const int width = 4 * group;
    q.n_tiles = (int)((F + width - 1) / width);
    q.split = kXcd / gcd_int(q.n_tiles, kXcd);
    while (((long long)q.n_rows + q.split - 1) / q.split * F * 4 >= (1LL << 32) - 65536 && q.split < (1 << 20)) q.split *= 2;
    q.n_slots = q.n_tiles * q.split;
    q.blocks_per_label = (n_cu + kXcd - 1) / kXcd;
    const size_t lds_need = (size_t)q.n_rel * width * sizeof(float);
    const bool rel_fits = q.n_rel > 0 && lds_need <= (size_t)kMaxLdsBytes;
    const int grid = q.blocks_per_label * kXcd;
    int rel = rel_fits ? kRelLds : kRelL2;
    q.n_rel_lds = rel_fits ? q.n_rel : 0;
    size_t lds = kLdsHeader + (rel_fits ? lds_need : 0);
    const int part_rows = (int)((size_t)kMaxLdsBytes / ((size_t)width * sizeof(float)));
    if (!rel_fits && q.n_rel > 0 && (long long)part_rows * 4 >= q.n_rel) {
        rel = kRelPart;
        q.n_rel_lds = part_rows;
        lds = kLdsHeader + (size_t)part_rows * width * sizeof(float);
    }
    if (group == 64) return launch_rowgroup_g<64>(q, backward, sum_op, mul_op, unit_w, rel, grid, lds, stream);
    if (group == 32) return launch_rowgroup_g<32>(q, backward, sum_op, mul_op, unit_w, rel, grid, lds, stream);
    return launch_rowgroup_g<16>(q, backward, sum_op, mul_op, unit_w, rel, grid, lds, stream);
}

bool g_no_rowgroup = false;
bool g_no_concurrent_tiles = false;
bool g_no_dense = false;


template <int KIND>
int run_plan(const ultra_segments *seg, KParams p, int64_t gather_rows, int64_t gather2_rows, int64_t n_rel, int64_t F,
             int sum_op, int mul_op, bool wants_rel_lds, void *workspace, size_t workspace_bytes, hipStream_t stream) {
    int rc = check_segments(seg);
    if (rc) return rc;
    if (F <= 0 || n_rel < 0 || n_rel > 0x7fffffffLL) return ULTRA_ERR_BAD_SHAPE;
    if (sum_op < 0 || sum_op > 2 || mul_op < 0 || mul_op > 1) return ULTRA_ERR_BAD_OP;
    const size_t need = ultra_rspmm_workspace_bytes(seg, F);
    if (need > 0 && (workspace == nullptr || workspace_bytes < need)) return ULTRA_ERR_WORKSPACE;
    if (seg->n_rows == 0) return ULTRA_OK;

    int dev = 0;
    HIP_TRY(hipGetDevice(&dev));
    DeviceInfo *di = nullptr;
    rc = device_info(dev, &di);
    if (rc) return rc;

    const int n_tiles = (int)((F + kTile - 1) / kTile);
    const int split = kXcd / gcd_int(n_tiles, kXcd);
    const size_t lds_need = (size_t)n_rel * kTile * sizeof(float);
    const bool rel_lds = wants_rel_lds && n_rel > 0 && lds_need <= (size_t)kMaxLdsBytes;
    const int blocks_per_label = (di->n_cu + kXcd - 1) / kXcd;

    p.row = seg->row;
    p.node_a = seg->node_a;
    p.node_b = seg->node_b;
    p.rel = seg->rel;
    p.weight = seg->weight;
    p.chunks = reinterpret_cast<const int4 *>(seg->chunks);
    p.partial = static_cast<float *>(workspace);
    p.F = F;
    p.n_chunks = (int)seg->n_chunks;
    p.n_rel = (int)n_rel;
    p.n_tiles = n_tiles;
    p.split = split;
    p.n_slots = n_tiles * split;
    p.blocks_per_label = blocks_per_label;

    const int grid = blocks_per_label * kXcd;
    hipEvent_t ev_start = g_prof_start, ev_stop = g_prof_stop;
    g_prof_start = g_prof_stop = nullptr;
    if (ev_start != nullptr || ev_stop != nullptr) {
        hipStreamCaptureStatus cs = hipStreamCaptureStatusNone;
        HIP_TRY(hipStreamIsCapturing(stream, &cs));
        if (cs != hipStreamCaptureStatusNone) ev_start = ev_stop = nullptr;
    }
    auto stamp = [&](hipEvent_t ev) -> hipError_t { return hipEventRecord(ev, stream); };
    if (ev_start != nullptr) HIP_TRY(stamp(ev_start));
    if (seg->dense != nullptr && !g_no_dense && !g_force_general && !g_no_quad && !g_no_x_lds &&
        std::strncmp(di->arch, "gfx950", 6) == 0) {
        ultra_detail::DenseCall call{seg, KIND, sum_op, mul_op, p.relation, p.input, p.grad, p.add_rows, p.bnode, p.bvec, p.bdim,
                                     p.out, workspace, workspace_bytes, gather_rows, gather2_rows, n_rel, F};
        if (ultra_detail::dense_applies(call)) {
            rc = ultra_detail::dense_launch(call, stream);
            if (rc) return rc;
            if (ev_stop != nullptr) HIP_TRY(stamp(ev_stop));
            return ULTRA_OK;
        }
    }
    bool use_rowgroup = false;
    if constexpr (KIND != KIND_DREL) {
        auto aligned16 = [](const void *ptr) { return (reinterpret_cast<uintptr_t>(ptr) & 15u) == 0; };
        const float *gather = (KIND == KIND_DX) ? p.grad : p.input;
        use_rowgroup = !g_force_general && !g_no_rowgroup && seg->row_ptr != nullptr && seg->packed_src_shift >= 32 &&
                       seg->n_long_rows == 0 && (F % 4) == 0 && (KIND == KIND_FWD || sum_op == ULTRA_SUM_ADD) &&
                       aligned16(gather) && aligned16(p.out) && aligned16(p.relation) && aligned16(p.add_rows) &&
                       aligned16(p.bvec) && (p.bnode == nullptr || p.bdim % 4 == 0);
        if (use_rowgroup) {
            RowGroupParams q{};
            q.row_ptr = seg->row_ptr;
            q.col = seg->node_a;
            q.rel = seg->rel;
            q.weight = seg->weight;
            q.relation = p.relation;
            q.gather = gather;
            q.add_rows = p.add_rows;
            q.bnode = p.bnode;
            q.bvec = p.bvec;
            q.bdim = p.bdim;
            q.out = p.out;
            q.F = F;
            q.n_rows = (int)seg->n_rows;
            q.n_rel = (int)n_rel;
            rc = launch_rowgroup(q, KIND == KIND_DX, sum_op, mul_op, seg->weight == nullptr, gather_rows, di->n_cu, stream);
            if (rc) return rc;
        }
    }
    bool use_packed = false;
    if (!use_rowgroup) {
        const float *gather = (KIND == KIND_DX) ? p.grad : p.input;
        const unsigned long long gather_bytes = (unsigned long long)gather_rows * (unsigned long long)F * 4ull;
        const unsigned long long gather2_bytes = (unsigned long long)gather2_rows * (unsigned long long)F * 4ull;
// ... 8 lines not shown
            PParams q{};
            q.meta = seg->packed;
            q.meta2 = reinterpret_cast<const uint32_t *>(big ? seg->node_a : seg->node_b);
            q.weight = seg->weight;
            q.chunks = p.chunks;
            q.relation = p.relation;
            q.gather = gather;
            q.gather2 = p.grad;
            q.add_rows = p.add_rows;
            q.bnode = p.bnode;
            q.bvec = p.bvec;
            q.bdim = p.bdim;
            q.out = p.out;
            q.partial = p.partial;
            q.F = F;
            q.gather_bytes = (uint32_t)gather_bytes;
            q.gather2_bytes = (uint32_t)gather2_bytes;
            q.relation_bytes = (uint32_t)(relation_bytes < 0xffff0000ull ? relation_bytes : 0);
            q.row_bytes = (uint32_t)(F * 4);
            q.src_shift = (uint32_t)seg->packed_src_shift;
            q.rel_mask = big ? 0xffffff00u : ((1u << (seg->packed_src_shift - 8)) - 1u) << 8;
            q.n_chunks = p.n_chunks;
            q.n_rel = p.n_rel;
            q.n_tiles = n_tiles;
            q.split = split;
            q.n_slots = p.n_slots;
            q.blocks_per_label = blocks_per_label;
            const bool needs_rel = (KIND == KIND_FWD) || (KIND == KIND_DX && mul_op == ULTRA_MUL_MUL);
            const size_t lds_x_bytes = (size_t)gather_rows * kTile * sizeof(float);
            int var = 0;
            size_t lds_bytes = needs_rel ? lds_need : 0;
            if (big) {
                var = (needs_rel && !rel_fits) ? 2 : 3;
                if (var == 2) lds_bytes = 0;
            } else if (seg->n_hot > 0) {
                const size_t hot_bytes = (size_t)seg->n_hot * kTile * sizeof(float);
                if (lds_bytes + hot_bytes > (size_t)kMaxLdsBytes) return ULTRA_ERR_BAD_SHAPE;
                var = 4;
                lds_bytes += hot_bytes;
                q.hot_nodes = seg->hot_nodes;
                q.n_hot = (int)seg->n_hot;
            } else if ((KIND != KIND_DREL || mul_op == ULTRA_MUL_MUL) && !g_no_x_lds && gather_rows > 0 &&
                       lds_bytes + lds_x_bytes <= (size_t)kMaxLdsBytes) {
                var = 1;
                lds_bytes += lds_x_bytes;
            }
            q.n_gather_rows = (int)gather_rows;
            auto aligned16 = [](const void *ptr) { return (reinterpret_cast<uintptr_t>(ptr) & 15u) == 0; };
            const unsigned long long meta_bytes = ((unsigned long long)seg->n_edges + 16ull) * 4ull;
            q.meta_bytes = (uint32_t)(meta_bytes < 0xffff0000ull ? meta_bytes : 0);
            q.meta2_bytes = (uint32_t)((unsigned long long)seg->n_edges * 4ull);
            const unsigned long long out_bytes = (unsigned long long)seg->n_rows * (unsigned long long)F * 4ull;
            q.out_bytes = (uint32_t)(out_bytes < 0xffff0000ull ? out_bytes : 0);
            const bool quad = !g_no_quad && (var == 0 || var == 1) && (F % 4) == 0 && q.out_bytes != 0 &&
                              q.meta_bytes != 0 && (unsigned long long)F * 4ull < (1ull << 24) &&
                              (KIND != KIND_DREL || gather2_rows < (1ll << 24)) && aligned16(gather) && aligned16(p.grad) &&
                              aligned16(p.out) && aligned16(p.add_rows) && aligned16(p.partial) && aligned16(p.bvec) &&
                              (p.bnode == nullptr || p.bdim % 4 == 0);
            if (quad) {
                const int slots_per_label = (q.n_slots + kXcd - 1) / kXcd;
                int conc = 1;
                while (!g_no_concurrent_tiles && conc * 2 <= slots_per_label && blocks_per_label % (conc * 2) == 0 &&
                       blocks_per_label / (conc * 2) >= 4)
                    conc *= 2;
                if (const char *force = getenv("ULTRA_CONC")) {
                    const int want = atoi(force);
                    const char *min_rows = getenv("ULTRA_CONC_MIN_ROWS");
                    if (want >= 1 && blocks_per_label % want == 0 && (min_rows == nullptr || gather_rows >= atoll(min_rows)))
                        conc = want;
                }
                q.concurrent = conc;
                size_t act_bytes = 0;
                if (KIND == KIND_DREL && var == 0 && F % kTile == 0) {
                    if (p.act_bits != nullptr && p.act_words > 0 && lds_bytes + (size_t)p.act_words * 4 <= (size_t)kMaxLdsBytes) {
                        q.act_bits = p.act_bits;
                        q.act_words = p.act_words;
                        act_bytes = (size_t)p.act_words * 4;
                    } else if (KIND == KIND_DREL && p.act_node != nullptr && mul_op == ULTRA_MUL_MUL) {
                        q.act_node = p.act_node;
                    }
                }
                const bool dead = seg->packed_dead != nullptr && !g_no_dead_words && var == 0 && q.act_node == nullptr &&
                                  sum_op == ULTRA_SUM_ADD && mul_op == ULTRA_MUL_MUL;
                if (dead) { q.meta = seg->packed_dead; q.weight = nullptr; }
                rc = launch_quad<KIND>(q, sum_op, mul_op, dead || seg->weight == nullptr, var == 1, grid,
                                       kLdsHeader + lds_bytes + act_bytes, stream, dead);
            }
            if (!quad) rc = launch_packed<KIND>(q, sum_op, mul_op, seg->weight == nullptr, var, grid, kLdsHeader + lds_bytes, stream);
            if (rc) return rc;
        }
    }
    if (!use_packed && !use_rowgroup) {
        rc = launch_ops<KIND>(p, sum_op, mul_op, seg->weight == nullptr, rel_lds, grid,
                              kLdsHeader + (rel_lds ? lds_need : 0), stream);
        if (rc) return rc;
    }
    if (ev_stop != nullptr) HIP_TRY(stamp(ev_stop));

    if (seg->n_long_rows > 0) {
        FixParams fp;
        fp.long_rows = seg->long_rows;
        fp.partial = p.partial;
        fp.add_rows = p.add_rows;
        fp.bnode = p.bnode;
        fp.bvec = p.bvec;
        fp.bdim = p.bdim;
        fp.out = p.out;
        fp.F = F;
        fp.n_long = (int)seg->n_long_rows;
        fp.n_tiles = n_tiles;
        const long long waves = (long long)fp.n_long * n_tiles;
        const int fgrid = (int)((waves + 3) / 4);
        const int red = (KIND == KIND_FWD) ? sum_op : ULTRA_SUM_ADD;
        const bool many_pieces = seg->n_pieces >= 128 * seg->n_long_rows;
        if (red == ULTRA_SUM_ADD && many_pieces)
            hipLaunchKernelGGL((fixup_kernel<ULTRA_SUM_ADD, 64>), dim3(fgrid), dim3(256), 0, stream, fp);
        else if (red == ULTRA_SUM_ADD) hipLaunchKernelGGL(fixup_kernel<ULTRA_SUM_ADD>, dim3(fgrid), dim3(256), 0, stream, fp);
        else if (red == ULTRA_SUM_MIN) hipLaunchKernelGGL(fixup_kernel<ULTRA_SUM_MIN>, dim3(fgrid), dim3(256), 0, stream, fp);
        else hipLaunchKernelGGL(fixup_kernel<ULTRA_SUM_MAX>, dim3(fgrid), dim3(256), 0, stream, fp);
        HIP_TRY(hipGetLastError());
    }
    return ULTRA_OK;
}

}

namespace ultra_detail {
int persistent_cus(int *n_cu) {
    int dev = 0;
    HIP_TRY(hipGetDevice(&dev));
    DeviceInfo *di = nullptr;
    const int rc = device_info(dev, &di);
    if (rc) return rc;
    *n_cu = di->n_cu;
    return ULTRA_OK;
}
bool wide_groups_forced() { return g_wide_groups; }
}

extern "C" {

int ultra_rspmm_abi_version(void) { return ULTRA_RSPMM_ABI_VERSION; }

size_t ultra_segments_bytes(void) { return sizeof(ultra_segments); }

const char *ultra_rspmm_status_string(int status) {
    switch (status) {
        case ULTRA_OK: return "ok";
        case ULTRA_ERR_BAD_OP: return "unknown sum/mul operator code";
        case ULTRA_ERR_BAD_SHAPE: return "bad shape (negative size, F <= 0 or index range beyond int32)";
        case ULTRA_ERR_NULL_POINTER: return "required pointer is NULL";
        case ULTRA_ERR_WORKSPACE: return "workspace is NULL or smaller than ultra_rspmm_workspace_bytes()";
        case ULTRA_ERR_HIP: return "HIP runtime error (see ultra_rspmm_last_hip_error)";
        case ULTRA_ERR_NO_DEVICE: return "no usable HIP device";
        case ULTRA_ERR_ABI: return "ultra_segments.struct_bytes / abi_version are not this library's (binding written against another include/ultra_rspmm.h)";
        default: return "unknown status";
    }
}

int ultra_rspmm_last_hip_error(void) { return ultra_detail_last_hip_error; }

int ultra_rspmm_reserve_cus(int n) {
    if (n < 0) return ULTRA_ERR_BAD_SHAPE;
    g_reserve_cus = n;
    for (DeviceInfo &d : g_dev)
        if (d.valid) d.n_cu = std::max(kXcd, d.n_cu_total - n);
    return ULTRA_OK;
}

int ultra_rspmm_device_info(int device, int *n_cu, int *lds_bytes, char *arch_host, size_t arch_len) {
    DeviceInfo *di = nullptr;
    int rc = device_info(device, &di);
    if (rc) return rc;
    if (n_cu) *n_cu = di->n_cu_total;
    if (lds_bytes) *lds_bytes = di->lds_bytes;
// ... 101 lines not shown
    if (fwd == nullptr) return ULTRA_ERR_NULL_POINTER;
    if (!segments_abi_ok(fwd)) return ULTRA_ERR_ABI;
    if (boundary_node == nullptr || boundary_value == nullptr) return ULTRA_ERR_NULL_POINTER;
    if (fwd->n_rows > 0 && out == nullptr) return ULTRA_ERR_NULL_POINTER;
    if (fwd->n_edges > 0 && (relation == nullptr || input == nullptr)) return ULTRA_ERR_NULL_POINTER;
    if (block <= 0 || block > 0x7fffffffLL || F <= 0 || F % block != 0) return ULTRA_ERR_BAD_SHAPE;
    KParams p{};
    p.relation = relation;
    p.input = input;
    p.bnode = boundary_node;
    p.bvec = boundary_value;
    p.bdim = (int)block;
    p.out = out;
    return run_plan<KIND_FWD>(fwd, p, n_src, 0, n_rel, F, sum_op, mul_op, true, workspace, workspace_bytes,
                              static_cast<hipStream_t>(stream));
}

int ultra_rspmm_frontier_f32(const ultra_segments *by_src, const int32_t *src_ptr, const int32_t *fwd_rank,
                             const float *relation, const int32_t *boundary_node, const float *boundary_value,
                             int64_t block, float *out, int64_t n_dst, int64_t n_rel, int64_t F, void *stream) {
    int rc = check_segments(by_src);
    if (rc) return rc;
    if (src_ptr == nullptr || boundary_node == nullptr || boundary_value == nullptr) return ULTRA_ERR_NULL_POINTER;
    if (by_src->n_edges > 0 && (fwd_rank == nullptr || relation == nullptr)) return ULTRA_ERR_NULL_POINTER;
    if (block != 64 || F <= 0 || F % 64 != 0 || n_dst < 0 || n_rel < 0 || by_src->piece_len <= 0) return ULTRA_ERR_BAD_SHAPE;
    if (n_dst == 0) return ULTRA_OK;
    if (out == nullptr) return ULTRA_ERR_NULL_POINTER;
    if ((reinterpret_cast<uintptr_t>(out) | reinterpret_cast<uintptr_t>(relation) |
         reinterpret_cast<uintptr_t>(boundary_value)) & 15u) return ULTRA_ERR_BAD_SHAPE;
    hipStream_t s = static_cast<hipStream_t>(stream);
    hipEvent_t ev_start = g_prof_start, ev_stop = g_prof_stop;
    g_prof_start = g_prof_stop = nullptr;
    if (ev_start != nullptr || ev_stop != nullptr) {
        hipStreamCaptureStatus cs = hipStreamCaptureStatusNone;
        HIP_TRY(hipStreamIsCapturing(s, &cs));
        if (cs != hipStreamCaptureStatusNone) ev_start = ev_stop = nullptr;
    }
    if (ev_start != nullptr) HIP_TRY(hipEventRecord(ev_start, s));
    {
        const long long n4 = (long long)n_dst * F / 4;
        const unsigned blocks = (unsigned)((n4 + 256 * 8 - 1) / (256 * 8) < 4096 ? (n4 + 256 * 8 - 1) / (256 * 8) : 4096);
        hipLaunchKernelGGL(zero_fill_kernel, dim3(blocks ? blocks : 1), dim3(256), 0, s, reinterpret_cast<qf4 *>(out), n4);
        HIP_TRY(hipGetLastError());
    }
    FrontierParams p{};
    p.src_ptr = src_ptr;
    p.dst = by_src->node_a;
    p.rel = by_src->rel;
    p.weight = by_src->weight;
    p.fwd_rank = fwd_rank;
    p.relation = relation;
    p.bnode = boundary_node;
    p.bvec = boundary_value;
    p.out = out;
    p.F = F;
    p.piece_len = (int)by_src->piece_len;
    p.n_rel = (int)n_rel;
    p.piece_shift = -1;
    for (int sh = 0; sh < 31; ++sh)
        if ((1LL << sh) == by_src->piece_len) p.piece_shift = sh;
    const size_t msg_bytes = (size_t)n_rel * kTile * sizeof(float);
    if (!g_force_general && n_rel > 0 && msg_bytes <= (size_t)kMaxLdsBytes) {
        p.slices = kFrontierLdsSlices;
        const int grid = (int)(F / 64) * p.slices;
        int rc = by_src->weight == nullptr
                     ? launch_with_lds(frontier_lds_kernel<true>, p, grid, msg_bytes, s, kFrontierLdsThreads)
                     : launch_with_lds(frontier_lds_kernel<false>, p, grid, msg_bytes, s, kFrontierLdsThreads);
        if (rc) return rc;
    } else {
        p.slices = 64;
        const dim3 grid((unsigned)(F / 64), (unsigned)p.slices);
        if (by_src->weight == nullptr) hipLaunchKernelGGL(frontier_kernel<true>, grid, dim3(kFrontierThreads), 0, s, p);
        else hipLaunchKernelGGL(frontier_kernel<false>, grid, dim3(kFrontierThreads), 0, s, p);
        HIP_TRY(hipGetLastError());
    }
    if (ev_stop != nullptr) HIP_TRY(hipEventRecord(ev_stop, s));
    return ULTRA_OK;
}

int ultra_first_layer_sparse_supported(int64_t n_dst, int64_t n_rel, int64_t n_query) {
    return n_query > 0 && n_query <= kCbLdsQueries && n_rel > 0 && n_dst > 0 && n_dst * n_query < 0x7fffffffLL;
}

static int first_layer_sparse_impl(const ultra_segments *by_src, const int32_t *src_ptr, const int32_t *fwd_rank,
                                   const int32_t *run_prefix, const float *relation, const int32_t *boundary_node,
                                   const float *boundary_value, int64_t n_query, const float *weight, const float *bias,
                                   const float *ln_weight, const float *ln_bias, float ln_eps, int relu, int shortcut,
                                   float *update, float *out, int32_t *row_list, int64_t row_list_len, int64_t max_runs,
                                   int32_t *list_offset, int64_t n_dst, int64_t n_rel, void *stream) {
    int rc = check_segments(by_src);
    if (rc) return rc;
    if (!ultra_first_layer_sparse_supported(n_dst, n_rel, n_query) || by_src->piece_len <= 0 || max_runs < 0 ||
        max_runs > n_dst || row_list_len < n_query * (max_runs + 1) || row_list_len > 0x7fffffffLL)
        return ULTRA_ERR_BAD_SHAPE;
    if (src_ptr == nullptr || fwd_rank == nullptr || run_prefix == nullptr || relation == nullptr || boundary_node == nullptr ||
        boundary_value == nullptr || weight == nullptr || bias == nullptr || out == nullptr || update == nullptr ||
        row_list == nullptr || list_offset == nullptr)
        return ULTRA_ERR_NULL_POINTER;
    if (ln_weight != nullptr && ln_bias == nullptr) return ULTRA_ERR_NULL_POINTER;
    const long long F = n_query * 64;
    if ((reinterpret_cast<uintptr_t>(out) | reinterpret_cast<uintptr_t>(update) | reinterpret_cast<uintptr_t>(relation) |
         reinterpret_cast<uintptr_t>(boundary_value)) & 15u)
        return ULTRA_ERR_BAD_SHAPE;
    hipStream_t s = static_cast<hipStream_t>(stream);
    int dev = 0;
    HIP_TRY(hipGetDevice(&dev));
    DeviceInfo *di = nullptr;
    rc = device_info(dev, &di);
    if (rc) return rc;
    CombineParams cp{};
    cp.weight = weight; cp.bias = bias; cp.gamma = ln_weight; cp.beta = ln_bias;
    cp.eps = ln_eps; cp.relu = relu; cp.shortcut = shortcut;
    cp.in_bnode = boundary_node; cp.in_bvec = boundary_value; cp.rpn = (int)n_query;
    const size_t lds_cb = (size_t)(kCbWaves * kCbTileFloats + 128 + n_query * 65) * sizeof(float);
    rc = ensure_lds_attribute(reinterpret_cast<const void *>(combine_kernel<false, 3>), lds_cb);
    if (rc) return rc;
    {
        ConstFillParams fp{};
        fp.out = reinterpret_cast<qf4 *>(out); fp.n4 = (long long)n_dst * F / 4;
        fp.bias = bias; fp.gamma = ln_weight; fp.beta = ln_bias; fp.eps = ln_eps; fp.relu = relu; fp.shortcut = shortcut;
        fp.src_ptr = src_ptr; fp.run_prefix = run_prefix; fp.bnode = boundary_node; fp.n_query = (int)n_query;
        fp.list_offset = list_offset; fp.list_len = (int)row_list_len;
        const unsigned blocks = (unsigned)((fp.n4 + 256 * 8 - 1) / (256 * 8) < 4096 ? (fp.n4 + 256 * 8 - 1) / (256 * 8) : 4096);
        hipLaunchKernelGGL(const_fill_kernel, dim3(blocks ? blocks : 1), dim3(256), 0, s, fp);
        HIP_TRY(hipGetLastError());
    }
    FrontierParams p{};
    p.src_ptr = src_ptr; p.dst = by_src->node_a; p.rel = by_src->rel; p.weight = by_src->weight; p.fwd_rank = fwd_rank;
    p.relation = relation; p.bnode = boundary_node; p.bvec = boundary_value; p.out = update; p.F = F;
    p.piece_len = (int)by_src->piece_len; p.n_rel = (int)n_rel; p.piece_shift = -1;
    for (int sh = 0; sh < 31; ++sh)
        if ((1LL << sh) == by_src->piece_len) p.piece_shift = sh;
    p.run_prefix = run_prefix; p.row_list = row_list; p.list_offset = list_offset; p.list_len = (int)row_list_len;
    const size_t msg_bytes = (size_t)n_rel * kTile * sizeof(float);
    if (!g_force_general && msg_bytes <= (size_t)kMaxLdsBytes) {
        p.slices = kFrontierLdsSlices;
        const int fgrid = (int)n_query * p.slices;
        rc = by_src->weight == nullptr ? launch_with_lds(frontier_lds_kernel<true>, p, fgrid, msg_bytes, s, kFrontierLdsThreads)
                                       : launch_with_lds(frontier_lds_kernel<false>, p, fgrid, msg_bytes, s, kFrontierLdsThreads);
        if (rc) return rc;
    } else {
        p.slices = 64;
        const dim3 fgrid((unsigned)n_query, (unsigned)p.slices);
        if (by_src->weight == nullptr) hipLaunchKernelGGL(frontier_kernel<true>, fgrid, dim3(kFrontierThreads), 0, s, p);
        else hipLaunchKernelGGL(frontier_kernel<false>, fgrid, dim3(kFrontierThreads), 0, s, p);
        HIP_TRY(hipGetLastError());
    }
    cp.update = update; cp.out = out; cp.rows = n_dst * n_query; cp.row_list = row_list; cp.list_count = list_offset + n_query;
    cp.list_len = (int)row_list_len;
    hipLaunchKernelGGL((combine_kernel<false, 3>), dim3((unsigned)(2 * di->n_cu)), dim3(kCbWaves * 64), lds_cb, s, cp);
    HIP_TRY(hipGetLastError());
    return ULTRA_OK;
}

int ultra_first_layer_sparse_f32(const ultra_segments *by_src, const int32_t *src_ptr, const int32_t *fwd_rank,
                                 const int32_t *run_prefix, const float *relation, const int32_t *boundary_node,
                                 const float *boundary_value, int64_t n_query, const float *weight, const float *bias,
                                 const float *ln_weight, const float *ln_bias, float ln_eps, int relu, int shortcut,
                                 float *out, int32_t *row_list, int64_t row_list_len, int64_t max_runs, int32_t *list_offset,
                                 int64_t n_dst, int64_t n_rel, void *stream) {
    return first_layer_sparse_impl(by_src, src_ptr, fwd_rank, run_prefix, relation, boundary_node, boundary_value, n_query, weight,
                                   bias, ln_weight, ln_bias, ln_eps, relu, shortcut, out, out, row_list, row_list_len, max_runs,
                                   list_offset, n_dst, n_rel, stream);
}

int ultra_first_layer_sparse_train_f32(const ultra_segments *by_src, const int32_t *src_ptr, const int32_t *fwd_rank,
                                       const int32_t *run_prefix, const float *relation, const int32_t *boundary_node,
                                       const float *boundary_value, int64_t n_query, const float *weight, const float *bias,
                                       const float *ln_weight, const float *ln_bias, float ln_eps, int relu, int shortcut,
                                       float *update, float *out, int32_t *row_list, int64_t row_list_len, int64_t max_runs,
                                       int32_t *list_offset, int64_t n_dst, int64_t n_rel, void *stream) {
    if (update == nullptr) return ULTRA_ERR_NULL_POINTER;
    if (update == out) return ULTRA_ERR_BAD_SHAPE;
    return first_layer_sparse_impl(by_src, src_ptr, fwd_rank, run_prefix, relation, boundary_node, boundary_value, n_query, weight,
                                   bias, ln_weight, ln_bias, ln_eps, relu, shortcut, update, out, row_list, row_list_len, max_runs,
                                   list_offset, n_dst, n_rel, stream);
}

size_t ultra_rspmm_backward_boundary_rows_workspace(int64_t n_query) {
    return n_query <= 0 ? 0 : (size_t)n_query * kBRowsWaves * 64 * sizeof(float);
}

int ultra_rspmm_backward_boundary_rows_f32(const ultra_segments *by_src, const int32_t *src_ptr, const float *relation,
                                           const float *output_grad, const int32_t *boundary_node, float *d_input,
                                           float *workspace, size_t workspace_bytes, int64_t n_src, int64_t n_query, int64_t F,
                                           int mul_op, void *stream) {
    int rc = check_segments(by_src);
    if (rc) return rc;
    if (n_src < 0 || n_query < 0 || n_query > 65535 || F != n_query * 64 || (mul_op != ULTRA_MUL_MUL && mul_op != ULTRA_MUL_ADD))
        return ULTRA_ERR_BAD_SHAPE;
    if (n_query == 0 || n_src == 0) return ULTRA_OK;
    if (src_ptr == nullptr || boundary_node == nullptr || d_input == nullptr || workspace == nullptr) return ULTRA_ERR_NULL_POINTER;
    if (by_src->n_edges > 0 && (output_grad == nullptr || (mul_op == ULTRA_MUL_MUL && relation == nullptr))) return ULTRA_ERR_NULL_POINTER;
    if (workspace_bytes < ultra_rspmm_backward_boundary_rows_workspace(n_query)) return ULTRA_ERR_WORKSPACE;
    BoundaryRowsParams p;
    p.src_ptr = src_ptr; p.dst = by_src->node_a; p.rel = by_src->rel; p.weight = by_src->weight;
    p.relation = mul_op == ULTRA_MUL_MUL ? relation : nullptr; p.grad = output_grad; p.bnode = boundary_node;
    p.partial = workspace; p.d_input = d_input; p.F = F;
    hipStream_t s = static_cast<hipStream_t>(stream);
    const dim3 grid(kBRowsSlices, (unsigned)n_query), block(256);
    const bool unit_w = by_src->weight == nullptr, has_rel = mul_op == ULTRA_MUL_MUL;
    if (unit_w && has_rel) hipLaunchKernelGGL((boundary_rows_partial_kernel<true, true>), grid, block, 0, s, p);
    else if (unit_w) hipLaunchKernelGGL((boundary_rows_partial_kernel<true, false>), grid, block, 0, s, p);
    else if (has_rel) hipLaunchKernelGGL((boundary_rows_partial_kernel<false, true>), grid, block, 0, s, p);
    else hipLaunchKernelGGL((boundary_rows_partial_kernel<false, false>), grid, block, 0, s, p);
    HIP_TRY(hipGetLastError());
    hipLaunchKernelGGL(boundary_rows_reduce_kernel, dim3((unsigned)n_query), dim3(64), 0, s, p);
    HIP_TRY(hipGetLastError());
    return ULTRA_OK;
}

int ultra_rspmm_backward_f32(const ultra_segments *by_src, const ultra_segments *by_rel, const float *relation,
                             const float *input, const float *output, const float *output_grad, float *d_input,
                             float *d_relation, void *workspace, size_t workspace_bytes, int64_t n_src, int64_t n_dst,
                             int64_t n_rel, int64_t F, int sum_op, int mul_op, void *stream) {
    return ultra_rspmm_backward_accumulate_f32(by_src, by_rel, relation, input, output, output_grad, nullptr, d_input,
                                               d_relation, workspace, workspace_bytes, n_src, n_dst, n_rel, F, sum_op,
                                               mul_op, stream);
}

int ultra_rspmm_backward_accumulate_f32(const ultra_segments *by_src, const ultra_segments *by_rel, const float *relation,
                                        const float *input, const float *output, const float *output_grad,
                                        const float *d_input_add, float *d_input, float *d_relation, void *workspace,
                                        size_t workspace_bytes, int64_t n_src, int64_t n_dst, int64_t n_rel, int64_t F,
                                        int sum_op, int mul_op, void *stream) {
    if (output_grad == nullptr || relation == nullptr || input == nullptr) return ULTRA_ERR_NULL_POINTER;
    if (d_input_add != nullptr && sum_op != ULTRA_SUM_ADD) return ULTRA_ERR_BAD_OP;
    if (sum_op != ULTRA_SUM_ADD && output == nullptr) return ULTRA_ERR_NULL_POINTER;
    hipStream_t s = static_cast<hipStream_t>(stream);
    if (d_input != nullptr) {
        if (by_src == nullptr) return ULTRA_ERR_NULL_POINTER;
        KParams p{};
        p.relation = relation;
        p.input = input;
        p.output = output;
        p.grad = output_grad;
        p.out = d_input;
        p.add_rows = d_input_add;
        const bool needs_rel = (mul_op == ULTRA_MUL_MUL) || (sum_op != ULTRA_SUM_ADD);
        int rc = run_plan<KIND_DX>(by_src, p, n_dst, 0, n_rel, F, sum_op, mul_op, needs_rel, workspace, workspace_bytes, s);
        if (rc) return rc;
    }
    if (d_relation != nullptr) {
        if (by_rel == nullptr) return ULTRA_ERR_NULL_POINTER;
        if (!segments_abi_ok(by_rel)) return ULTRA_ERR_ABI;
        if (by_rel->n_edges > 0 && by_rel->node_b == nullptr) return ULTRA_ERR_NULL_POINTER;
// ... 30 lines not shown
    if (d_relation != nullptr) {
        if (by_rel == nullptr) return ULTRA_ERR_NULL_POINTER;
        if (!segments_abi_ok(by_rel)) return ULTRA_ERR_ABI;
        if (by_rel->n_edges > 0 && by_rel->node_b == nullptr) return ULTRA_ERR_NULL_POINTER;
        KParams p{};
        p.relation = relation; p.input = input; p.grad = output_grad; p.out = d_relation;
        p.act_bits = dst_active_bits; p.act_words = (int)active_words; p.act_node = src_active_node;
        int rc = run_plan<KIND_DREL>(by_rel, p, n_src, n_dst, n_rel, F, ULTRA_SUM_ADD, mul_op, false, workspace, workspace_bytes, s);
        if (rc) return rc;
    }
    return ULTRA_OK;
}

int ultra_rspmm_backward_weight_f32(const ultra_segments *fwd, const float *relation, const float *input,
                                    const float *output, const float *output_grad, float *d_weight, int64_t n_rel,
                                    int64_t F, int sum_op, int mul_op, void *stream) {
    int rc = check_segments(fwd);
    if (rc) return rc;
    (void)n_rel;
    if (F <= 0) return ULTRA_ERR_BAD_SHAPE;
    if (sum_op < 0 || sum_op > 2 || mul_op < 0 || mul_op > 1) return ULTRA_ERR_BAD_OP;
    if (fwd->n_edges == 0) return ULTRA_OK;
    if (relation == nullptr || input == nullptr || output_grad == nullptr || d_weight == nullptr)
        return ULTRA_ERR_NULL_POINTER;
    if (sum_op != ULTRA_SUM_ADD && output == nullptr) return ULTRA_ERR_NULL_POINTER;
    hipStream_t s = static_cast<hipStream_t>(stream);
    const bool unit = fwd->weight == nullptr;
    long long blocks = (fwd->n_edges + 3) / 4;
    if (blocks > 8192) blocks = 8192;
#define ULTRA_WCASE(S, M)                                                                                          \
    if (sum_op == S && mul_op == M) {                                                                              \
        if (unit)                                                                                                  \
            hipLaunchKernelGGL((weight_grad_kernel<S, M, true>), dim3((int)blocks), dim3(256), 0, s, fwd->row,     \
                               fwd->node_a, fwd->rel, fwd->weight, relation, input, output, output_grad, d_weight, \
                               (long long)F, (long long)fwd->n_edges);                                             \
        else                                                                                                       \
            hipLaunchKernelGGL((weight_grad_kernel<S, M, false>), dim3((int)blocks), dim3(256), 0, s, fwd->row,    \
                               fwd->node_a, fwd->rel, fwd->weight, relation, input, output, output_grad, d_weight, \
                               (long long)F, (long long)fwd->n_edges);                                             \
    }
    ULTRA_WCASE(ULTRA_SUM_ADD, ULTRA_MUL_MUL)
    ULTRA_WCASE(ULTRA_SUM_ADD, ULTRA_MUL_ADD)
    ULTRA_WCASE(ULTRA_SUM_MIN, ULTRA_MUL_MUL)
    ULTRA_WCASE(ULTRA_SUM_MIN, ULTRA_MUL_ADD)
    ULTRA_WCASE(ULTRA_SUM_MAX, ULTRA_MUL_MUL)
    ULTRA_WCASE(ULTRA_SUM_MAX, ULTRA_MUL_ADD)
#undef ULTRA_WCASE
    HIP_TRY(hipGetLastError());
    return ULTRA_OK;
}


static int combine_launch(const CombineParams &p, void *stream) {
    int dev = 0;
    HIP_TRY(hipGetDevice(&dev));
    DeviceInfo *di = nullptr;
    int rc = device_info(dev, &di);
    if (rc) return rc;
    const long long n_tiles = (p.rows + kCbRows - 1) / kCbRows;
    long long blocks = (n_tiles + kCbWaves - 1) / kCbWaves;
    const bool prefetch = n_tiles >= (long long)di->n_cu * kCbWaves * 4;
    const long long resident = (long long)di->n_cu * (prefetch ? 1 : 2);
    if (blocks > resident) blocks = resident;
    const size_t lds_max = (size_t)(kCbWaves * kCbTileFloats + 128 + kCbLdsQueries * 65) * sizeof(float);
    const size_t lds = (size_t)(kCbWaves * kCbTileFloats + 128 + (p.in_bnode != nullptr && p.rpn <= kCbLdsQueries ? p.rpn * 65 : 0)) * sizeof(float);
    static bool attr_set[16] = {false};
    if (dev >= 0 && dev < 16 && !attr_set[dev]) {
        HIP_TRY(hipFuncSetAttribute(reinterpret_cast<const void *>(combine_kernel<false, 0>),
                                    hipFuncAttributeMaxDynamicSharedMemorySize, (int)lds_max));
        HIP_TRY(hipFuncSetAttribute(reinterpret_cast<const void *>(combine_kernel<true, 0>),
                                    hipFuncAttributeMaxDynamicSharedMemorySize, (int)lds_max));
        HIP_TRY(hipFuncSetAttribute(reinterpret_cast<const void *>(combine_kernel<false, 1>),
                                    hipFuncAttributeMaxDynamicSharedMemorySize, (int)lds_max));
        HIP_TRY(hipFuncSetAttribute(reinterpret_cast<const void *>(combine_kernel<true, 1>),
                                    hipFuncAttributeMaxDynamicSharedMemorySize, (int)lds_max));
        HIP_TRY(hipFuncSetAttribute(reinterpret_cast<const void *>(combine_kernel<false, 2>),
                                    hipFuncAttributeMaxDynamicSharedMemorySize, (int)lds_max));
        HIP_TRY(hipFuncSetAttribute(reinterpret_cast<const void *>(combine_kernel<true, 2>),
                                    hipFuncAttributeMaxDynamicSharedMemorySize, (int)lds_max));
        HIP_TRY(hipFuncSetAttribute(reinterpret_cast<const void *>(combine_kernel<false, 0, true>),
                                    hipFuncAttributeMaxDynamicSharedMemorySize, (int)lds_max));
        HIP_TRY(hipFuncSetAttribute(reinterpret_cast<const void *>(combine_kernel<true, 0, true>),
                                    hipFuncAttributeMaxDynamicSharedMemorySize, (int)lds_max));
        attr_set[dev] = true;
    }
    const dim3 grid((unsigned)blocks), block(kCbWaves * 64);
    hipStream_t st = static_cast<hipStream_t>(stream);
    if (p.in_bnode != nullptr && p.rpn <= kCbLdsQueries) {
        if (prefetch) hipLaunchKernelGGL((combine_kernel<true, 1>), grid, block, lds, st, p);
        else hipLaunchKernelGGL((combine_kernel<false, 1>), grid, block, lds, st, p);
    } else if (p.in_bnode != nullptr) {
        if (prefetch) hipLaunchKernelGGL((combine_kernel<true, 2>), grid, block, lds, st, p);
        else hipLaunchKernelGGL((combine_kernel<false, 2>), grid, block, lds, st, p);
    } else if (p.z_out != nullptr) {
        if (prefetch) hipLaunchKernelGGL((combine_kernel<true, 0, true>), grid, block, lds, st, p);
        else hipLaunchKernelGGL((combine_kernel<false, 0, true>), grid, block, lds, st, p);
    } else {
        if (prefetch) hipLaunchKernelGGL((combine_kernel<true, 0>), grid, block, lds, st, p);
        else hipLaunchKernelGGL((combine_kernel<false, 0>), grid, block, lds, st, p);
    }
    HIP_TRY(hipGetLastError());
    return ULTRA_OK;
}

int ultra_combine_forward_f32(const float *input, const float *update, const float *weight, const float *bias,
                              const float *ln_weight, const float *ln_bias, float ln_eps, int relu, int shortcut,
                              float *out, float *z_out, int64_t rows, int64_t dim, void *stream) {
    if (dim != 64) return ULTRA_ERR_BAD_SHAPE;
    if (rows < 0) return ULTRA_ERR_BAD_SHAPE;
    if (rows == 0) return ULTRA_OK;
    if (input == nullptr || update == nullptr || weight == nullptr || bias == nullptr || out == nullptr)
        return ULTRA_ERR_NULL_POINTER;
    if (ln_weight != nullptr && ln_bias == nullptr) return ULTRA_ERR_NULL_POINTER;
    CombineParams p{};
    p.input = input; p.update = update; p.weight = weight; p.bias = bias; p.gamma = ln_weight; p.beta = ln_bias;
    p.out = out; p.rows = rows; p.eps = ln_eps; p.relu = relu; p.shortcut = shortcut;
    p.z_out = z_out;
    return combine_launch(p, stream);
}

int ultra_combine_forward_boundary_f32(const int32_t *boundary_node, const float *boundary_value, int64_t n_query,
                                       const float *update, const float *weight, const float *bias, const float *ln_weight,
                                       const float *ln_bias, float ln_eps, int relu, int shortcut, float *out, int64_t rows,
                                       int64_t dim, void *stream) {
    if (dim != 64 || rows < 0 || n_query <= 0 || n_query > 0x7fffffffLL || rows % n_query != 0) return ULTRA_ERR_BAD_SHAPE;
    if (rows == 0) return ULTRA_OK;
    if (boundary_node == nullptr || boundary_value == nullptr || update == nullptr || weight == nullptr || bias == nullptr ||
        out == nullptr)
        return ULTRA_ERR_NULL_POINTER;
    if (ln_weight != nullptr && ln_bias == nullptr) return ULTRA_ERR_NULL_POINTER;
    if (reinterpret_cast<uintptr_t>(boundary_value) & 15u) return ULTRA_ERR_BAD_SHAPE;
    CombineParams p{};
    p.input = nullptr; p.update = update; p.weight = weight; p.bias = bias; p.gamma = ln_weight; p.beta = ln_bias;
    p.out = out; p.rows = rows; p.eps = ln_eps; p.relu = relu; p.shortcut = shortcut;
    p.in_bnode = boundary_node; p.in_bvec = boundary_value; p.rpn = (int)n_query;
    return combine_launch(p, stream);
}

}

#include "combine_train.inc"
#include "combine_fused_bwd.inc"
#include "first_layer_train.inc"
#include "dense.inc"
#include "project_bwd.inc"
#include "sampler.inc"
#include "score_rows.inc"
```

### ultra_torchdrug_amd/functional.py

```python
import collections

import torch

from . import _lib, _torch_ext
from .relcsr import RelCSR

__all__ = ["generalized_rspmm", "rspmm_forward", "first_layer_forward", "dense_layer_forward", "combine_forward", "combine", "linear_forward", "linear_supported", "score_all_entities", "relation_stack_inputs", "statistics", "bce_adversarial_loss", "candidate_tiles", "candidate_rows", "score_candidates", "RelCSR"]

_sparse_cache = collections.OrderedDict()
_SPARSE_CACHE_ENTRIES = 4


def accepts(tensor):
    return bool(tensor.is_cuda)


def _ops(sum, mul):
    if sum not in _lib.SUM_OPS:
        raise ValueError("Can't find a rspmm operator for sum=`%s` (expected add, min or max)" % sum)
    if mul not in _lib.MUL_OPS:
        raise ValueError("Can't find a rspmm operator for mul=`%s` (expected mul or add)" % mul)
    return _lib.SUM_OPS[sum], _lib.MUL_OPS[mul]


# ... 80 lines not shown
    if boundary is not None:
        with torch.cuda.device(input.device):
            _lib.check(lib.ultra_rspmm_forward_boundary_f32(
                seg.pointer, relation.data_ptr(), input.data_ptr(), b_node.data_ptr(), b_value.data_ptr(),
                b_value.shape[1], out.data_ptr(), ws.data_ptr() if ws is not None else None, ws_bytes, csr.shape[1],
                csr.shape[2], F, sum_op, mul_op, _stream()))
        return out
    with torch.cuda.device(input.device):
        _lib.check(lib.ultra_rspmm_forward_f32(
            seg.pointer, relation.data_ptr(), input.data_ptr(), add_rows.data_ptr() if add_rows is not None else None,
            out.data_ptr(), ws.data_ptr() if ws is not None else None, ws_bytes, csr.shape[1], csr.shape[2], F, sum_op,
            mul_op, _stream()))
    return out


def rspmm_forward_csr(row_ptr, src, rel, weight, relation, input, sum="add", mul="mul"):
    sum_op, mul_op = _ops(sum, mul)
    if input.dim() != 2 or relation.dim() != 2 or relation.shape[1] != input.shape[1]:
        raise RuntimeError("relation (R, F) and input (N_src, F) expected, got %s and %s"
                           % (tuple(relation.shape), tuple(input.shape)))
    tensors = [row_ptr, src, rel, relation, input] + ([weight] if weight is not None else [])
    if any(not t.is_cuda or t.device != input.device for t in tensors):
        raise RuntimeError("rspmm_forward_csr runs on an MI355X (HIP) device only. There is no CPU fallback.")
    if row_ptr.dtype != torch.int32 or src.dtype != torch.int32 or rel.dtype != torch.int32:
        raise RuntimeError("rspmm_forward_csr: row_ptr / src / rel must be int32")
    if input.dtype != torch.float32 or relation.dtype != torch.float32 or (weight is not None and weight.dtype != torch.float32):
        raise RuntimeError("rspmm is fp32 only (TF32 is disabled in the reference, script/run_full.py:19-20)")
    F = input.shape[1]
    if F % 4:
        raise RuntimeError("rspmm_forward_csr needs 16-byte rows (F % 4 == 0); use a RelCSR plan for other widths")
    n_rows, n_edges = row_ptr.numel() - 1, src.numel()
    relation, input = relation.contiguous(), input.contiguous()
    out = torch.empty(n_rows, F, dtype=torch.float32, device=input.device)
    if out.numel() == 0:
        return out
    lib = _lib.load()
    with torch.cuda.device(input.device):
        _lib.check(lib.ultra_rspmm_fwd_f32(
            row_ptr.contiguous().data_ptr(), src.contiguous().data_ptr(), rel.contiguous().data_ptr(),
            weight.contiguous().data_ptr() if weight is not None else None, relation.data_ptr(), input.data_ptr(),
            out.data_ptr(), n_rows, n_edges, relation.shape[0], F, sum_op, mul_op, _stream()))
    return out


def frontier_supported(sum, mul, F):
    return sum == "add" and mul == "mul" and F % 64 == 0


def rspmm_frontier(csr, relation, boundary):
    b_node, b_value = boundary
    b_value = b_value.contiguous()
    n_dst, n_src, n_rel = csr.shape
    F = b_value.numel()
    if relation.dim() != 2 or relation.shape != (n_rel, F) or relation.dtype != torch.float32 or not relation.is_cuda:
        raise RuntimeError("rspmm_frontier: relation must be fp32 (%d, %d) on the HIP device" % (n_rel, F))
    if (b_node.dtype != torch.int32 or b_node.dim() != 1 or b_value.dtype != torch.float32 or b_value.dim() != 2
            or b_value.shape != (b_node.shape[0], 64) or not b_node.is_contiguous()
            or b_node.device != relation.device or b_value.device != relation.device or csr.device != relation.device):
        raise RuntimeError("rspmm_frontier: boundary must be (int32 (B,), fp32 (B, 64)) on %s" % relation.device)
    if n_dst != n_src:
        raise RuntimeError("rspmm_frontier: the boundary rows index the source nodes of a square adjacency")
    relation = relation.contiguous()
    out = torch.empty(n_dst, F, dtype=torch.float32, device=relation.device)
    if out.numel() == 0:
        return out
    src_ptr, fwd_rank = csr.frontier_index
    lib = _lib.load()
    with torch.cuda.device(relation.device):
        _lib.check(lib.ultra_rspmm_frontier_f32(
            csr.by_src.pointer, src_ptr.data_ptr(), fwd_rank.data_ptr(), relation.data_ptr(), b_node.data_ptr(),
            b_value.data_ptr(), 64, out.data_ptr(), n_dst, n_rel, F, _stream()))
    return out


SPARSE_FIRST_LAYER = __import__("os").environ.get("ULTRA_SPARSE_FIRST_LAYER", "1") != "0"
SPARSE_FIRST_LAYER_MIN_ROWS = 1 << 17


SPARSE_FIRST_LAYER_MAX_LIST = float(__import__("os").environ.get("ULTRA_SPARSE_FIRST_LAYER_MAX_LIST", "1.0"))
SPARSE_FIRST_LAYER_TRAIN_MAX_BYTES = int(__import__("os").environ.get("ULTRA_SPARSE_FIRST_LAYER_TRAIN_MAX_BYTES", str(2 << 30)))


def first_layer_forward(csr, relation, boundary, weight, bias, ln_weight=None, ln_bias=None, ln_eps=1e-5, relu=True,
                        shortcut=False, want_list=False):
    if not SPARSE_FIRST_LAYER:
        return None
    b_node, b_value = boundary
    n_dst, n_src, n_rel = csr.shape
    n_query = b_node.shape[0]
    lib = _lib.load()
    if (n_dst != n_src or n_dst * n_query < SPARSE_FIRST_LAYER_MIN_ROWS
            or not lib.ultra_first_layer_sparse_supported(n_dst, n_rel, n_query)
            or csr.frontier_runs[1] + 1 > SPARSE_FIRST_LAYER_MAX_LIST * n_dst):
        return None
    F = n_query * 64
    b_value = b_value.contiguous()
    tensors = [relation, b_value, weight, bias] + ([ln_weight, ln_bias] if ln_weight is not None else [])
    if (relation.dim() != 2 or tuple(relation.shape) != (n_rel, F) or tuple(b_value.shape) != (n_query, 64) or b_node.dtype != torch.int32
            or not b_node.is_contiguous() or tuple(weight.shape) != (64, 128)
            or any(t.dtype != torch.float32 or not t.is_cuda or t.device != relation.device for t in tensors)
            or b_node.device != relation.device or csr.device != relation.device):
        raise RuntimeError("first_layer_forward: relation fp32 (%d, %d), boundary (int32 (Q,), fp32 (Q, 64)), a (64, 128) weight, "
                           "all on one HIP device" % (n_rel, F))
    relation = relation.contiguous()
    dev = relation.device
    src_ptr, fwd_rank = csr.frontier_index
    run_prefix, max_runs = csr.frontier_runs
    out = torch.empty(n_dst, n_query, 64, dtype=torch.float32, device=dev)
    row_list = torch.empty(n_query * (max_runs + 1), dtype=torch.int32, device=dev)
    list_offset = torch.empty(n_query + 1, dtype=torch.int32, device=dev)
    with torch.cuda.device(dev):
        _lib.check(lib.ultra_first_layer_sparse_f32(
            csr.by_src.pointer, src_ptr.data_ptr(), fwd_rank.data_ptr(), run_prefix.data_ptr(), relation.data_ptr(),
            b_node.data_ptr(), b_value.data_ptr(), n_query, weight.contiguous().data_ptr(), bias.contiguous().data_ptr(),
            ln_weight.contiguous().data_ptr() if ln_weight is not None else None,
            ln_bias.contiguous().data_ptr() if ln_weight is not None else None, float(ln_eps), int(bool(relu)), int(bool(shortcut)),
            out.data_ptr(), row_list.data_ptr(), row_list.numel(), int(max_runs), list_offset.data_ptr(), n_dst, n_rel, _stream()))
    if want_list:
        return out, row_list, list_offset[n_query:]
    return out


SPARSE_FIRST_LAYER_TRAIN = __import__("os").environ.get("ULTRA_SPARSE_FIRST_LAYER_TRAIN", "1") != "0"
SPARSE_FIRST_LAYER_TRAIN_MAX_FRACTION = float(__import__("os").environ.get("ULTRA_SPARSE_FIRST_LAYER_TRAIN_MAX_FRACTION", "0.2"))


def first_layer_train_forward(csr, relation, boundary, weight, bias, ln_weight=None, ln_bias=None, ln_eps=1e-5, relu=True,
                              shortcut=False):
    if not SPARSE_FIRST_LAYER_TRAIN:
        return None
    b_node, b_value = boundary
    n_dst, n_src, n_rel = csr.shape
    n_query = b_node.shape[0]
    lib = _lib.load()
    if (n_dst != n_src or n_dst * n_query < SPARSE_FIRST_LAYER_MIN_ROWS or n_dst * n_query > (1 << 24) - 64
            or not lib.ultra_first_layer_sparse_supported(n_dst, n_rel, n_query)
            or csr.frontier_fraction > SPARSE_FIRST_LAYER_TRAIN_MAX_FRACTION
            or csr.frontier_runs[1] + 1 > SPARSE_FIRST_LAYER_MAX_LIST * n_dst
            or n_query * (csr.frontier_runs[1] + 1) * 5 * 256 > SPARSE_FIRST_LAYER_TRAIN_MAX_BYTES):
        return None
    F = n_query * 64
    b_value = b_value.contiguous()
    if (tuple(relation.shape) != (n_rel, F) or tuple(b_value.shape) != (n_query, 64) or b_node.dtype != torch.int32
            or not b_node.is_contiguous() or tuple(weight.shape) != (64, 128)):
        return None
    relation = relation.contiguous()
    dev = relation.device
    src_ptr, fwd_rank = csr.frontier_index
    run_prefix, max_runs = csr.frontier_runs
    update = torch.empty(n_dst, n_query, 64, dtype=torch.float32, device=dev)
    out = torch.empty(n_dst, n_query, 64, dtype=torch.float32, device=dev)
    row_list = torch.empty(n_query * (max_runs + 1), dtype=torch.int32, device=dev)
    list_offset = torch.empty(n_query + 1, dtype=torch.int32, device=dev)
    with torch.cuda.device(dev):
        _lib.check(lib.ultra_first_layer_sparse_train_f32(
            csr.by_src.pointer, src_ptr.data_ptr(), fwd_rank.data_ptr(), run_prefix.data_ptr(), relation.data_ptr(),
            b_node.data_ptr(), b_value.data_ptr(), n_query, weight.contiguous().data_ptr(), bias.contiguous().data_ptr(),
            ln_weight.contiguous().data_ptr() if ln_weight is not None else None,
            ln_bias.contiguous().data_ptr() if ln_weight is not None else None, float(ln_eps), int(bool(relu)), int(bool(shortcut)),
            update.data_ptr(), out.data_ptr(), row_list.data_ptr(), row_list.numel(), int(max_runs), list_offset.data_ptr(),
            n_dst, n_rel, _stream()))
    return update, out, row_list, list_offset[n_query:]


FUSED_LAYER = __import__("os").environ.get("ULTRA_FUSED_LAYER", "1") != "0"
FUSED_SCORE = __import__("os").environ.get("ULTRA_FUSED_SCORE", "1") != "0"


SECOND_LAYER_SOURCES = __import__("os").environ.get("ULTRA_SECOND_LAYER_SOURCES", "1") != "0"


def second_layer_sources(csr, row_list, list_count, n_query):
    if not SECOND_LAYER_SOURCES or not FUSED_LAYER:
        return None
    n_dst, n_src, n_rel = csr.shape
    plan = csr.fwd
    lib = _lib.load()
    if (n_dst != n_src or not lib.ultra_layer_forward_supported(plan.pointer, n_query, n_rel)
            or row_list.numel() * 64 > n_src or row_list.numel() + 1 >= n_src):
        return None
    dev = row_list.device
    E = plan.n_edges
    slack = plan.node_a.numel() - E
    sources = torch.empty(E + slack, dtype=torch.int32, device=dev)
    bitmap = torch.empty((n_src + 31) // 32, dtype=torch.int32, device=dev)
    c_node = torch.empty(1, dtype=torch.int32, device=dev)
    with torch.cuda.device(dev):
        _lib.check(lib.ultra_second_layer_sources(plan.node_a.data_ptr(), E, slack, row_list.data_ptr(), list_count.data_ptr(),
                                                  row_list.numel(), n_query, n_src, bitmap.data_ptr(), c_node.data_ptr(),
                                                  sources.data_ptr(), _stream()))
    return sources


def layer_forward(csr, relation, input, boundary, weight, bias, ln_weight=None, ln_bias=None, ln_eps=1e-5, relu=True,
                  shortcut=False, sources=None):
    if not FUSED_LAYER or input.dim() != 3 or input.shape[-1] != 64:
        return None
    n_dst, n_src, n_rel = csr.shape
    n_query = input.shape[1]
    lib = _lib.load()
    plan = csr.fwd
    if n_dst != n_src or input.shape[0] != n_src or not lib.ultra_layer_forward_supported(plan.pointer, n_query, n_rel):
        return None
    F = n_query * 64
    b_node, b_value = (None, None) if boundary is None else boundary
    tensors = [relation, input, weight, bias] + ([ln_weight, ln_bias] if ln_weight is not None else []) + ([b_value] if b_value is not None else [])
    if (ln_weight is not None and ln_bias is None) or any(t.numel() != 64 for t in tensors[3:4 + (2 if ln_weight is not None else 0)]):
        return None
    if (tuple(relation.shape) != (n_rel, F) or tuple(weight.shape) != (64, 128)
            or any(t.dtype != torch.float32 or not t.is_cuda or t.device != input.device for t in tensors)
            or (b_node is not None and (b_node.dtype != torch.int32 or tuple(b_node.shape) != (n_query,) or tuple(b_value.shape) != (n_query, 64)))):
        return None
    relation, input = relation.contiguous(), input.contiguous()
    out = torch.empty_like(input)
    if sources is not None:
        if sources.dtype != torch.int32 or sources.numel() != plan.node_a.numel() or sources.device != input.device:
            raise RuntimeError("layer_forward: sources must be second_layer_sources() of this plan")
        with torch.cuda.device(input.device):
            _lib.check(lib.ultra_layer_forward_sources_f32(
                plan.pointer, sources.data_ptr(), relation.data_ptr(), input.data_ptr(),
                b_node.contiguous().data_ptr() if b_node is not None else None,
                b_value.contiguous().data_ptr() if b_value is not None else None, n_query, weight.contiguous().data_ptr(),
                bias.contiguous().data_ptr(), ln_weight.contiguous().data_ptr() if ln_weight is not None else None,
                ln_bias.contiguous().data_ptr() if ln_weight is not None else None, float(ln_eps), int(bool(relu)), int(bool(shortcut)),
                out.data_ptr(), n_rel, _stream()))
        return out
    with torch.cuda.device(input.device):
        _lib.check(lib.ultra_layer_forward_f32(
            plan.pointer, relation.data_ptr(), input.data_ptr(), b_node.contiguous().data_ptr() if b_node is not None else None,
            b_value.contiguous().data_ptr() if b_value is not None else None, n_query, weight.contiguous().data_ptr(),
            bias.contiguous().data_ptr(), ln_weight.contiguous().data_ptr() if ln_weight is not None else None,
            ln_bias.contiguous().data_ptr() if ln_weight is not None else None, float(ln_eps), int(bool(relu)), int(bool(shortcut)),
            out.data_ptr(), n_rel, _stream()))
    return out


def layer_score_forward(csr, relation, input, boundary, weight, bias, ln_weight, ln_bias, ln_eps, relu, shortcut, query, w1, b1, w2,
                        b2):
    if not FUSED_LAYER or not FUSED_SCORE or input.dim() != 3 or input.shape[-1] != 64:
        return None
    n_dst, n_src, n_rel = csr.shape
    n_query = input.shape[1]
    lib = _lib.load()
    plan = csr.fwd
    if n_dst != n_src or input.shape[0] != n_src or not lib.ultra_layer_score_supported(plan.pointer, n_query, n_rel):
        return None
    F = n_query * 64
    b_node, b_value = (None, None) if boundary is None else boundary
    tensors = [relation, input, weight, bias, query, w1, b1, w2, b2] + ([ln_weight, ln_bias] if ln_weight is not None else []) \
        + ([b_value] if b_value is not None else [])
    if (ln_weight is not None and ln_bias is None) or bias.numel() != 64 or b1.numel() != 128 \
            or (ln_weight is not None and (ln_weight.numel() != 64 or ln_bias.numel() != 64)):
        return None
    if (tuple(relation.shape) != (n_rel, F) or tuple(weight.shape) != (64, 128) or tuple(w1.shape) != (128, 128) or w2.numel() != 128
            or b2.numel() != 1 or tuple(query.shape) != (n_query, 64)
            or any(t.dtype != torch.float32 or not t.is_cuda or t.device != input.device for t in tensors)
            or (b_node is not None and (b_node.dtype != torch.int32 or tuple(b_node.shape) != (n_query,) or tuple(b_value.shape) != (n_query, 64)))):
        return None
    relation, input = relation.contiguous(), input.contiguous()
    score = torch.empty(n_query, n_src, dtype=torch.float32, device=input.device)
    qbias = torch.empty(n_query, 128, dtype=torch.float32, device=input.device)
    with torch.cuda.device(input.device):
        _lib.check(lib.ultra_layer_score_forward_f32(
            plan.pointer, relation.data_ptr(), input.data_ptr(), b_node.contiguous().data_ptr() if b_node is not None else None,
            b_value.contiguous().data_ptr() if b_value is not None else None, n_query, weight.contiguous().data_ptr(),
            bias.contiguous().data_ptr(), ln_weight.contiguous().data_ptr() if ln_weight is not None else None,
            ln_bias.contiguous().data_ptr() if ln_weight is not None else None, float(ln_eps), int(bool(relu)), int(bool(shortcut)),
            query.contiguous().data_ptr(), w1.contiguous().data_ptr(), b1.contiguous().data_ptr(), w2.contiguous().data_ptr(),
            b2.contiguous().data_ptr(), qbias.data_ptr(), score.data_ptr(), n_rel, _stream()))
    return score


DENSE_LAYER = __import__("os").environ.get("ULTRA_DENSE_LAYER", "1") != "0"

# ... 940 lines not shown
```

### ultra_torchdrug_amd/model.py

```python
from collections.abc import Sequence

import torch
from torch import nn
from torch.nn import functional as F

from . import backend, layer
from .graph import Graph


class TransferNBFNet(nn.Module):
    check_indices = True
    cut_after = "auto"
    last_cuts = None
    record_cuts = False

    def cut_at(self):
        if self.cut_after == "auto":
            return len(self.layers) // 2
        return self.cut_after

    def __init__(self, input_dim, hidden_dims, num_relation=None, symmetric=False, message_func="distmult",
                 aggregate_func="pna", short_cut=False, layer_norm=False, activation="relu", concat_hidden=False,
                 num_mlp_layer=2, project=True, remove_one_hop=False, num_beam=10, path_topk=10, mod=False):
        super().__init__()
# ... 236 lines not shown
        triples = packed[n_val:].view(n_layer, take, n_layer, 3).tolist()
        weights, paths = [], []
        for i in range(n_layer):
            for k in range(take):
                d = values[i][k]
                if d == float("-inf"):
                    break
                paths.append([tuple(x) for x in triples[i][k][:i + 1]])
                weights.append(d / (i + 1))
        if not paths:
            return (), ()
        weights, paths = zip(*sorted(zip(weights, paths), reverse=True)[:topk])
        return paths, weights

    def _relation_tables(self, batch_size):
        ops = backend.get()
        convs = list(self.layers)
        training = torch.is_grad_enabled()
        if not convs or (training and len(convs) > 8):
            return None
        relation = getattr(convs[0], "relation", None)
        if relation is None or not ops.accepts(relation) or relation.dim() != 3 or relation.shape[0] != batch_size \
                or relation.shape[-1] != 64 or relation.dtype != torch.float32:
            return None
        weights = []
        for conv in convs:
            mlp = getattr(conv, "relation_projection", None)
            ok = (getattr(conv, "project", False) and conv.relation is relation and mlp is not None
                  and len(mlp.layers) == 2 and not mlp.short_cut and mlp.activation is torch.nn.functional.relu
                  and all(l.in_features == 64 and l.out_features == 64 and l.bias is not None for l in mlp.layers))
            if not ok:
                return None
            weights.append((mlp.layers[0].weight, mlp.layers[0].bias, mlp.layers[1].weight, mlp.layers[1].bias))
        tables = ops.relation_project_train(relation, weights) if training else ops.relation_project(relation, weights)
        return {id(conv): table for conv, table in zip(convs, tables)}

    def _fast_stack(self):
        F = torch.nn.functional
        if not self.layers or self.concat_hidden or self.symmetric or not layer.FRONTIER_FIRST_LAYER:
            return None
        stack = []
        for conv in self.layers:
            mlp = getattr(conv, "relation_projection", None)
            ok = (isinstance(conv, layer.GeneralizedRelationalConvNBFMod) and conv.project and conv.message_func == "distmult"
                  and conv.aggregate_func == "sum" and conv.input_dim == 64 and conv.output_dim == 64
                  and tuple(conv.linear.weight.shape) == (64, 128) and conv.linear.bias is not None
                  and (conv.activation is F.relu or not conv.activation)
                  and (conv.layer_norm is None or (conv.layer_norm.elementwise_affine and conv.layer_norm.bias is not None))
                  and mlp is not None and len(mlp.layers) == 2 and not mlp.short_cut and mlp.activation is F.relu
                  and all(l.in_features == 64 and l.out_features == 64 and l.bias is not None for l in mlp.layers))
            if not ok:
                return None
            ln = conv.layer_norm
            stack.append(dict(
                project=(mlp.layers[0].weight, mlp.layers[0].bias, mlp.layers[1].weight, mlp.layers[1].bias),
                combine=(conv.linear.weight, conv.linear.bias, ln.weight if ln else None, ln.bias if ln else None,
                         ln.eps if ln else 1e-5, conv.activation is F.relu)))
        return stack

    def score_both_sides(self, graph, rel_rep, batch):
        ops = backend.get()
        if (not getattr(ops, "FAST_INFERENCE", False) or torch.is_grad_enabled() or not graph.num_relation
                or not self._fused_head_ok(batch, None) or rel_rep.dim() != 3 or rel_rep.shape[0] != batch.shape[0]
                or rel_rep.shape[-1] != 64 or rel_rep.dtype != torch.float32 or rel_rep.shape[1] != 2 * graph.num_relation):
            return None
        stack = self._fast_stack()
        if stack is None:
            return None
        und = self._undirected(graph)
        if und.requires_grad or graph.requires_grad:
            return None
        csr = und.relcsr
        n_query = 2 * batch.shape[0]
        if not ops.frontier_supported("add", "mul", 64 * n_query):
            return None
        anchor, anchor32, relation, query = ops.prepare_queries(batch, rel_rep, graph.num_relation)
        tables = ops.relation_project(rel_rep, [entry["project"] for entry in stack], repeat=2)
        if not layer._frontier_tables_finite(tables[0]):
            return None
        boundary = (anchor32, query)
        n_node = und.num_node
        hidden = None
        listed = None
        for i, entry in enumerate(stack):
            w, b, g, beta, eps, relu = entry["combine"]
            if i == 0:
                first_out = ops.first_layer_forward(csr, tables[0], boundary, w, b, g, beta, eps, relu, self.short_cut, want_list=True)
                hidden, listed = (None, None) if first_out is None else (first_out[0], first_out[1:])
                if hidden is None:
                    update = ops.rspmm_frontier(csr, tables[0], boundary).view(n_node, n_query, 64)
                    hidden = ops.combine_forward(None, update, w, b, g, beta, eps, relu, self.short_cut, reuse_update=True,
                                                 input_boundary=boundary)
            else:
                if i == len(stack) - 1:
                    first, second = self.mlp.layers
                    score = ops.layer_score_forward(csr, tables[i], hidden, boundary, w, b, g, beta, eps, relu, self.short_cut, query,
                                                    first.weight, first.bias, second.weight, second.bias)
                    if score is not None:
                        return score
                sources = ops.second_layer_sources(csr, listed[0], listed[1], n_query) if (i == 1 and listed is not None) else None
                fused = ops.layer_forward(csr, tables[i], hidden, boundary, w, b, g, beta, eps, relu, self.short_cut, sources=sources)
                if fused is not None:
                    hidden = fused
                    continue
                update = ops.rspmm_forward(csr, tables[i], hidden.flatten(1), "add", "mul", boundary=boundary)
                hidden = ops.combine_forward(hidden, update.view(n_node, n_query, 64), w, b, g, beta, eps, relu, self.short_cut,
                                             reuse_update=True)
        first, second = self.mlp.layers
        return ops.score_all_entities(hidden, query, first.weight, first.bias, second.weight, second.bias)

    def score_all_entities(self, graph, rel_query_list, h_index, r_index):
        if not graph.num_relation or not self._fused_head_ok(h_index, None):
            return None
        self.query = rel_query_list[0]
        for i, conv in enumerate(self.layers):
            conv.relation = rel_query_list[i + 1] if len(rel_query_list) > 1 else rel_query_list[0]
        graph = self._undirected(graph)
        parts = self.bellmanford(graph, h_index, r_index, want_feature=False)
        first, second = self.mlp.layers
        return backend.get().score_all_entities(parts["hidden"], parts["query"], first.weight, first.bias,
                                                 second.weight, second.bias)

    def forward(self, graph, rel_query_list, h_index, t_index, r_index=None, all_loss=None, metric=None,
                all_entities=False):
        keep, removal = None, None
        if self.check_indices:
            n_node, n_rel = graph.num_node, max(graph.num_relation or 0, 1)
            bad = (h_index < 0) | (h_index >= n_node) | (t_index < 0) | (t_index >= n_node)
            if r_index is not None:
                bad = bad | (r_index < 0) | (r_index >= n_rel)
            if bool(bad.any()):
                r_lo, r_hi = (int(r_index.min()), int(r_index.max())) if r_index is not None else (0, 0)
                raise IndexError("entity ids must lie in [0, %d) and relation ids in [0, %d): got h in [%d, %d], t in [%d, %d], "
                                 "r in [%d, %d]" % (n_node, n_rel, int(h_index.min()), int(h_index.max()), int(t_index.min()),
                                                    int(t_index.max()), r_lo, r_hi))
        if all_loss is not None:
            if (graph.num_relation and r_index is not None and not self.remove_one_hop
                    and self._removal_by_zero_weight(sums_only=True)):
                removal = (h_index, t_index, r_index)
            else:
                keep = self.easy_edge_mask(graph, h_index, t_index, r_index)
                if not (graph.num_relation and self._removal_by_zero_weight()):
                    graph, keep = graph.edge_mask(keep), None

        self.query = rel_query_list[0]
        if len(rel_query_list) > 1:
            assert len(rel_query_list) == len(self.layers) + 1
            for i, conv in enumerate(self.layers):
                conv.relation = rel_query_list[i + 1]
        else:
            for conv in self.layers:
                conv.relation = rel_query_list[0]
        if metric is not None:
            q = self.query.detach()
            ops = backend.get()
            if ops.accepts(q) and q.dtype == torch.float32:
                metric["query_norm"], metric["query_mean"], metric["query_std"] = ops.statistics(q).unbind(0)
            else:
                metric["query_norm"], metric["query_mean"], metric["query_std"] = q.norm(), q.mean(), q.std()

        shape = h_index.shape
        if graph.num_relation:
            num_relations = graph.num_relation
            graph = self._undirected(graph)
            if keep is not None:
                graph = graph.reweighted(graph.edge_weight * keep.repeat_interleave(2))
            if removal is not None:
                graph = backend.get().remove_triples(graph, *removal, num_relations)
            h_index, t_index, r_index = self.negative_sample_to_tail(h_index, t_index, r_index, num_relations)
        else:
            graph = self.as_relational_graph(graph)
            h_index = h_index.view(-1, 1)
            t_index = t_index.view(-1, 1)
            r_index = torch.zeros_like(h_index)

# ... 88 lines not shown
```

Before: 43.63 billion.

## Substitute constant vector for unlisted first-layer rows in second layer

After the sparse first layer, rows that received no messages all hold the same value (combine applied to a zero update). The first layer now records that shared vector plus bitmaps of which rows were actually written. The second layer's quad gather and its combine read real hidden rows only where the bit is set and use the cached constant elsewhere. This cuts gather and input traffic for the mostly-constant first-layer output, at the cost of bitmap construction, extra LDS use and a new kernel specialisation.

```diff
diff --git a/include/ultra_rspmm.h b/include/ultra_rspmm.h
--- a/include/ultra_rspmm.h
+++ b/include/ultra_rspmm.h
@@ -278,6 +278,21 @@
                                     const float *bias, const float *ln_weight, const float *ln_bias, float ln_eps, int relu,
                                     int shortcut, float *out, int64_t n_rel, void *stream);
 
+size_t ultra_listed_bits_words(int64_t n_dst, int64_t n_query);
+int ultra_first_layer_sparse_const_f32(const ultra_segments *by_src, const int32_t *src_ptr, const int32_t *fwd_rank,
+                                       const int32_t *run_prefix, const float *relation, const int32_t *boundary_node,
+                                       const float *boundary_value, int64_t n_query, const float *weight, const float *bias,
+                                       const float *ln_weight, const float *ln_bias, float ln_eps, int relu, int shortcut,
+                                       float *out, int32_t *row_list, int64_t row_list_len, int64_t max_runs, int32_t *list_offset,
+                                       int64_t n_dst, int64_t n_rel, uint32_t *listed_bits, int64_t listed_words, float *const_vec,
+                                       void *stream);
+int ultra_second_layer_const_supported(const ultra_segments *fwd, int64_t n_src, int64_t n_query, int64_t n_rel);
+int ultra_second_layer_const_f32(const ultra_segments *fwd, const float *relation, const float *input, const int32_t *boundary_node,
+                                 const float *boundary_value, const uint32_t *listed_bits, int64_t listed_words,
+                                 const float *const_vec, int64_t n_query, const float *weight, const float *bias,
+                                 const float *ln_weight, const float *ln_bias, float ln_eps, int relu, int shortcut, float *out,
+                                 void *workspace, size_t workspace_bytes, int64_t n_src, int64_t n_rel, void *stream);
+
 int ultra_layer_score_supported(const ultra_segments *fwd, int64_t n_query, int64_t n_rel);
 int ultra_layer_score_forward_f32(const ultra_segments *fwd, const float *relation, const float *input, const int32_t *boundary_node,
                                   const float *boundary_value, int64_t n_query, const float *weight, const float *bias,
diff --git a/ultra_torchdrug_amd/_lib.py b/ultra_torchdrug_amd/_lib.py
--- a/ultra_torchdrug_amd/_lib.py
+++ b/ultra_torchdrug_amd/_lib.py
@@ -117,6 +117,10 @@
     "ultra_layer_forward_supported",
     "ultra_layer_forward_f32",
     "ultra_second_layer_sources",
+    "ultra_listed_bits_words",
+    "ultra_first_layer_sparse_const_f32",
+    "ultra_second_layer_const_supported",
+    "ultra_second_layer_const_f32",
     "ultra_layer_forward_sources_f32",
     "ultra_layer_score_supported",
     "ultra_layer_score_forward_f32",
@@ -155,6 +159,16 @@
     lib.ultra_layer_forward_f32.argtypes = [seg, vp, vp, vp, vp, i64, vp, vp, vp, vp, ctypes.c_float, i32, i32, vp, i64, vp]
     lib.ultra_second_layer_sources.restype = i32
     lib.ultra_second_layer_sources.argtypes = [vp, i64, i64, vp, vp, i64, i64, i64, vp, vp, vp, vp]
+    lib.ultra_listed_bits_words.restype = sz
+    lib.ultra_listed_bits_words.argtypes = [i64, i64]
+    lib.ultra_first_layer_sparse_const_f32.restype = i32
+    lib.ultra_first_layer_sparse_const_f32.argtypes = [seg, vp, vp, vp, vp, vp, vp, i64, vp, vp, vp, vp, ctypes.c_float, i32, i32, vp, vp,
+                                                       i64, i64, vp, i64, i64, vp, i64, vp, vp]
+    lib.ultra_second_layer_const_supported.restype = i32
+    lib.ultra_second_layer_const_supported.argtypes = [seg, i64, i64, i64]
+    lib.ultra_second_layer_const_f32.restype = i32
+    lib.ultra_second_layer_const_f32.argtypes = [seg, vp, vp, vp, vp, vp, i64, vp, i64, vp, vp, vp, vp, ctypes.c_float, i32, i32, vp, vp,
+                                                 sz, i64, i64, vp]
     lib.ultra_layer_forward_sources_f32.restype = i32
     lib.ultra_layer_forward_sources_f32.argtypes = [seg, vp, vp, vp, vp, vp, i64, vp, vp, vp, vp, ctypes.c_float, i32, i32, vp, i64, vp]
     lib.ultra_layer_score_supported.restype = i32
diff --git a/ultra_torchdrug_amd/csrc/frontier.inc b/ultra_torchdrug_amd/csrc/frontier.inc
--- a/ultra_torchdrug_amd/csrc/frontier.inc
+++ b/ultra_torchdrug_amd/csrc/frontier.inc
@@ -335,6 +335,9 @@
     int n_query;
     int list_len;
     int32_t *list_offset;
+    float *const_vec;
+    uint32_t *bits;
+    long long n_bits;
 };
 
 __global__ __launch_bounds__(256) void const_fill_kernel(const ConstFillParams p) {
@@ -379,6 +382,20 @@
     __syncthreads();
     const qf4 *c4 = reinterpret_cast<const qf4 *>(c);
     for (long long i = (long long)blockIdx.x * 256 + threadIdx.x; i < p.n4; i += (long long)gridDim.x * 256) p.out[i] = c4[i & 15];
+    if (p.const_vec != nullptr && blockIdx.x == 0 && threadIdx.x < 64) p.const_vec[threadIdx.x] = c[threadIdx.x];
+    for (long long i = (long long)blockIdx.x * 256 + threadIdx.x; i < p.n_bits; i += (long long)gridDim.x * 256) p.bits[i] = 0u;
+}
+
+__global__ __launch_bounds__(256) void list_bits_kernel(const int32_t *row_list, const int32_t *list_count, int list_len, int n_query,
+                                                        long long n_rows, long long node_words, uint32_t *node_bits, uint32_t *row_bits) {
+    const int n = min(list_count[0], list_len);
+    for (int i = blockIdx.x * 256 + threadIdx.x; i < n; i += gridDim.x * 256) {
+        const int r = row_list[i];
+        if (r < 0 || (long long)r >= n_rows) continue;
+        const int node = r / n_query, q = r - node * n_query;
+        atomicOr(row_bits + (r >> 5), 1u << (r & 31));
+        atomicOr(node_bits + (long long)q * node_words + (node >> 5), 1u << (node & 31));
+    }
 }
 
 __global__ __launch_bounds__(256) void zero_fill_kernel(qf4 *out, long long n4) {
diff --git a/ultra_torchdrug_amd/csrc/quad.inc b/ultra_torchdrug_amd/csrc/quad.inc
--- a/ultra_torchdrug_amd/csrc/quad.inc
+++ b/ultra_torchdrug_amd/csrc/quad.inc
@@ -40,8 +40,11 @@
     static_assert(KIND == KIND_FWD || SUM == ULTRA_SUM_ADD, "quad path: forward, or the backward of sum-aggregation");
     static_assert(!DEAD || (UNIT_W && !X_LDS && SUM == ULTRA_SUM_ADD && MUL == ULTRA_MUL_MUL && ACT != 1),
                   "marked words: unit weights, gathers through descriptors, summed DistMult messages");
-    static_assert(ACT == 0 || (!X_LDS && ((KIND == KIND_DX && ACT == 1) || (KIND == KIND_DREL && (ACT == 2 || ACT == 3)))),
-                  "activity masks: d_input by destination, d_relation by destination or by the tile's source node");
+    static_assert(ACT == 0 || (!X_LDS && ((KIND == KIND_DX && ACT == 1) || (KIND == KIND_DREL && (ACT == 2 || ACT == 3)) ||
+                                         (KIND == KIND_FWD && ACT == 4 && UNIT_W && !DEAD && SUM == ULTRA_SUM_ADD &&
+                                          MUL == ULTRA_MUL_MUL))),
+                  "activity masks: d_input by destination, d_relation by destination or by the tile's source node, "
+                  "summed DistMult forward by listed source");
     constexpr int RED = (KIND == KIND_FWD) ? SUM : ULTRA_SUM_ADD;
     constexpr bool TWO_GATHERS = (KIND == KIND_DREL);
     constexpr bool DIRECT_WORDS = X_LDS && !TWO_GATHERS;
@@ -106,10 +109,11 @@
             b_val = *reinterpret_cast<const qf4 *>(p.bvec + col);
         }
         int act_node = -1;
-        if constexpr (ACT == 1 || ACT == 2) {
+        if constexpr (ACT == 1 || ACT == 2 || ACT == 4) {
             uint32_t *lds_act = reinterpret_cast<uint32_t *>(lds_x);
             const uint32_t *bits = p.act_bits + (long long)tile * p.act_words;
             for (int i = threadIdx.x; i < p.act_words; i += kBlock) lds_act[i] = bits[i];
+            if (ACT == 4 && threadIdx.x < kTile) lds_x[((p.act_words + 3) & ~3) + threadIdx.x] = p.const_vec[threadIdx.x];
         }
         if constexpr (ACT == 3) act_node = p.act_node[tile];
         if (threadIdx.x == 0) *ticket = 0;
@@ -117,7 +121,7 @@
         const uint32_t rel_base = (uint32_t)kLdsHeader;
         const uint32_t x_base = rel_base + (NEEDS_REL ? (uint32_t)p.n_rel * 256u : 0u);
         auto dead = [&](uint32_t key) -> uint32_t {
-            if constexpr (ACT == 1 || ACT == 2) return ((lds_read1(x_base + (key >> 5) * 4u) >> (key & 31u)) & 1u) ? 0u : 0xffffffffu;
+            if constexpr (ACT == 1 || ACT == 2 || ACT == 4) return ((lds_read1(x_base + (key >> 5) * 4u) >> (key & 31u)) & 1u) ? 0u : 0xffffffffu;
             if constexpr (ACT == 3) return (int)key == act_node ? 0u : 0xffffffffu;
             return 0u;
         };
@@ -236,6 +240,7 @@
                 float wt[U];
                 qf4 xv[U], rv[U];
                 uint32_t killm[U];
+                uint32_t unl = 0u;
 #pragma unroll
                 for (int u = 0; u < U; ++u) { w[u] = wn[u]; w2[u] = w2n[u]; killm[u] = 0u; }
 #pragma unroll
@@ -262,7 +267,8 @@
                         xv[u] = lds_read4(((node << 8) | lane_bytes) + x_base);
                     } else {
                         uint32_t kill = 0u;
-                        if constexpr (ACT == 1) kill = dead(node);
+                        if constexpr (ACT == 1 || ACT == 4) kill = dead(node);
+                        if constexpr (ACT == 4) unl |= (kill & 1u) << u;
                         if constexpr (DEAD) kill = (uint32_t)((int32_t)w[u] >> 31);
                         if constexpr (DEDUP) {
                             const uint32_t before = (u == 0) ? prev_node : (w[u > 0 ? u - 1 : 0] >> p.src_shift);
@@ -310,6 +316,11 @@
                     prev_x = __builtin_bit_cast(qu4, xv[U - 1]);
                     prev_node = w[U - 1] >> p.src_shift;
                 }
+                if constexpr (ACT == 4) {
+                    const qf4 cv = lds_read4(x_base + (((uint32_t)p.act_words + 3u) & ~3u) * 4u + lane_bytes);
+#pragma unroll
+                    for (int u = 0; u < U; ++u) xv[u] = ((unl >> u) & 1u) ? cv : xv[u];
+                }
                 bool same_row = false;
                 if constexpr (!TAIL) same_row = __builtin_amdgcn_ballot_w64((w[U - 1] & 0xffu) != cur) == 0ull;
                 if (same_row) {
diff --git a/ultra_torchdrug_amd/csrc/rspmm_kernels.hip b/ultra_torchdrug_amd/csrc/rspmm_kernels.hip
--- a/ultra_torchdrug_amd/csrc/rspmm_kernels.hip
+++ b/ultra_torchdrug_amd/csrc/rspmm_kernels.hip
@@ -64,6 +64,7 @@
     const uint32_t *act_bits;
     int act_words;
     const int32_t *act_node;
+    const float *const_vec;
 };
 
 struct FixParams {
@@ -290,6 +291,7 @@
     const uint32_t *act_bits;
     int act_words;
     const int32_t *act_node;
+    const float *const_vec;
 };
 
 template <int KIND, int SUM, int MUL, bool UNIT_W, int VAR, int UN = kUnroll>
@@ -613,9 +615,11 @@
     const int32_t *row_list;
     const int32_t *list_count;
     int list_len;
+    const uint32_t *in_bits;
+    const float *in_cvec;
 };
 
-template <bool PF, int BND = 0, bool ZOUT = false>
+template <bool PF, int BND = 0, bool ZOUT = false, bool CIN = false>
 __global__ __launch_bounds__(kCbWaves * 64, PF ? 1 : 2) void combine_kernel(const CombineParams p) {
     extern __shared__ __attribute__((aligned(16))) float cb_lds[];
     const int lane = threadIdx.x & 63;
@@ -650,6 +654,14 @@
     __syncthreads();
 
     const long long last = p.rows - 1;
+    f32x4 cin = {0.0f, 0.0f, 0.0f, 0.0f};
+    const __amdgpu_buffer_rsrc_t rsrc_in =
+        __builtin_amdgcn_make_buffer_rsrc(const_cast<float *>(p.input), 0, CIN ? (int)(uint32_t)(p.rows * 256) : 0, 0x00020000);
+    uint32_t listed_next = 0u;
+    if constexpr (CIN) {
+        cin = *reinterpret_cast<const f32x4 *>(p.in_cvec + (lane & 15) * 4);
+        listed_next = p.in_bits[wave_global < n_tiles ? wave_global : 0];
+    }
     f32x4 pa[8], pb[8];
     int rid[8];
     auto fetch = [&](long long t) {
@@ -676,12 +688,18 @@
             node0 = (t * kCbRows) / p.rpn;
             query0 = (int)(t * kCbRows - node0 * p.rpn);
         }
+        const uint32_t listed = listed_next;
 #pragma unroll
         for (int q = 0; q < 8; ++q) {
             const int r = 4 * q + (lane >> 4), c = (lane & 15) * 4;
             long long gr = t * kCbRows + r;
             gr = gr < last ? gr : last;
-            if constexpr (BND == 0) {
+            if constexpr (BND == 0 && CIN) {
+                const bool on = (listed >> (uint32_t)(gr - t * kCbRows)) & 1u;
+                const uint32_t off = on ? (uint32_t)gr * 256u + (uint32_t)c * 4u : 0xffffffffu;
+                const f32x4 v = __builtin_bit_cast(f32x4, __builtin_amdgcn_raw_buffer_load_b128(rsrc_in, off, 0, 0));
+                pa[q] = on ? v : cin;
+            } else if constexpr (BND == 0) {
                 pa[q] = *reinterpret_cast<const f32x4 *>(p.input + gr * 64 + c);
             } else {
                 const unsigned qq = (unsigned)(query0 + r);
@@ -696,6 +714,10 @@
                 }
             }
             pb[q] = *reinterpret_cast<const f32x4 *>(p.update + gr * 64 + c);
+        }
+        if constexpr (CIN) {
+            const long long tn = t + wave_total;
+            listed_next = p.in_bits[tn < n_tiles ? tn : n_tiles - 1];
         }
     };
     if constexpr (PF) {
@@ -1029,6 +1051,9 @@
 
 template <int KIND, int SUM, int MUL>
 int launch_quad_w(const PParams &p, bool unit_w, bool x_lds, int grid, size_t lds, hipStream_t stream, bool dead = false) {
+    if constexpr (KIND == KIND_FWD && SUM == ULTRA_SUM_ADD && MUL == ULTRA_MUL_MUL) {
+        if (p.const_vec != nullptr) return launch_with_lds(quad_kernel<KIND, SUM, MUL, true, false, 6, 4>, p, grid, lds, stream);
+    }
     if constexpr (SUM == ULTRA_SUM_ADD && MUL == ULTRA_MUL_MUL) {
         if (dead && !x_lds && p.act_node == nullptr) {
             if constexpr (KIND == KIND_DREL) {
@@ -1163,6 +1188,9 @@
     if (sum_op < 0 || sum_op > 2 || mul_op < 0 || mul_op > 1) return ULTRA_ERR_BAD_OP;
     const size_t need = ultra_rspmm_workspace_bytes(seg, F);
     if (need > 0 && (workspace == nullptr || workspace_bytes < need)) return ULTRA_ERR_WORKSPACE;
+    if (p.const_vec != nullptr && (KIND != KIND_FWD || seg->dense != nullptr || seg->packed == nullptr ||
+                                   seg->packed_src_shift >= 32 || g_force_general))
+        return ULTRA_ERR_BAD_SHAPE;
     if (seg->n_rows == 0) return ULTRA_OK;
 
     int dev = 0;
@@ -1337,15 +1365,27 @@
                 }
                 const bool dead = seg->packed_dead != nullptr && !g_no_dead_words && var == 0 && q.act_node == nullptr &&
                                   sum_op == ULTRA_SUM_ADD && mul_op == ULTRA_MUL_MUL;
+                if (KIND == KIND_FWD && p.const_vec != nullptr) {
+                    const size_t bytes = (size_t)((p.act_words + 3) & ~3) * 4 + kTile * sizeof(float);
+                    if (var != 0 || dead || seg->weight != nullptr || sum_op != ULTRA_SUM_ADD || mul_op != ULTRA_MUL_MUL ||
+                        F % kTile != 0 || p.act_bits == nullptr || p.act_words <= 0 || lds_bytes + bytes > (size_t)kMaxLdsBytes)
+                        return ULTRA_ERR_BAD_SHAPE;
+                    q.act_bits = p.act_bits;
+                    q.act_words = p.act_words;
+                    q.const_vec = p.const_vec;
+                    act_bytes = bytes;
+                }
                 if (dead) { q.meta = seg->packed_dead; q.weight = nullptr; }
                 rc = launch_quad<KIND>(q, sum_op, mul_op, dead || seg->weight == nullptr, var == 1, grid,
                                        kLdsHeader + lds_bytes + act_bytes, stream, dead);
             }
+            if (!quad && p.const_vec != nullptr) return ULTRA_ERR_BAD_SHAPE;
             if (!quad) rc = launch_packed<KIND>(q, sum_op, mul_op, seg->weight == nullptr, var, grid, kLdsHeader + lds_bytes, stream);
             if (rc) return rc;
         }
     }
     if (!use_packed && !use_rowgroup) {
+        if (p.const_vec != nullptr) return ULTRA_ERR_BAD_SHAPE;
         rc = launch_ops<KIND>(p, sum_op, mul_op, seg->weight == nullptr, rel_lds, grid,
                               kLdsHeader + (rel_lds ? lds_need : 0), stream);
         if (rc) return rc;
@@ -1613,12 +1653,17 @@
     return n_query > 0 && n_query <= kCbLdsQueries && n_rel > 0 && n_dst > 0 && n_dst * n_query < 0x7fffffffLL;
 }
 
+static long long listed_bits_words(long long n_dst, long long n_query) {
+    return n_query * ((n_dst + 31) / 32) + (n_dst * n_query + 31) / 32;
+}
+
 static int first_layer_sparse_impl(const ultra_segments *by_src, const int32_t *src_ptr, const int32_t *fwd_rank,
                                    const int32_t *run_prefix, const float *relation, const int32_t *boundary_node,
                                    const float *boundary_value, int64_t n_query, const float *weight, const float *bias,
                                    const float *ln_weight, const float *ln_bias, float ln_eps, int relu, int shortcut,
                                    float *update, float *out, int32_t *row_list, int64_t row_list_len, int64_t max_runs,
-                                   int32_t *list_offset, int64_t n_dst, int64_t n_rel, void *stream) {
+                                   int32_t *list_offset, int64_t n_dst, int64_t n_rel, void *stream,
+                                   uint32_t *listed_bits = nullptr, float *const_vec = nullptr) {
     int rc = check_segments(by_src);
     if (rc) return rc;
     if (!ultra_first_layer_sparse_supported(n_dst, n_rel, n_query) || by_src->piece_len <= 0 || max_runs < 0 ||
@@ -1652,7 +1697,14 @@
         fp.bias = bias; fp.gamma = ln_weight; fp.beta = ln_bias; fp.eps = ln_eps; fp.relu = relu; fp.shortcut = shortcut;
         fp.src_ptr = src_ptr; fp.run_prefix = run_prefix; fp.bnode = boundary_node; fp.n_query = (int)n_query;
         fp.list_offset = list_offset; fp.list_len = (int)row_list_len;
-        const unsigned blocks = (unsigned)((fp.n4 + 256 * 8 - 1) / (256 * 8) < 4096 ? (fp.n4 + 256 * 8 - 1) / (256 * 8) : 4096);
+        if (listed_bits != nullptr) {
+            fp.n4 = 0;
+            fp.const_vec = const_vec;
+            fp.bits = listed_bits;
+            fp.n_bits = listed_bits_words(n_dst, n_query);
+        }
+        const long long work = fp.n4 > fp.n_bits ? fp.n4 : fp.n_bits;
+        const unsigned blocks = (unsigned)((work + 256 * 8 - 1) / (256 * 8) < 4096 ? (work + 256 * 8 - 1) / (256 * 8) : 4096);
         hipLaunchKernelGGL(const_fill_kernel, dim3(blocks ? blocks : 1), dim3(256), 0, s, fp);
         HIP_TRY(hipGetLastError());
     }
@@ -1677,6 +1729,13 @@
         else hipLaunchKernelGGL(frontier_kernel<false>, fgrid, dim3(kFrontierThreads), 0, s, p);
         HIP_TRY(hipGetLastError());
     }
+    if (listed_bits != nullptr) {
+        const long long node_words = (n_dst + 31) / 32;
+        const long long lb = (row_list_len + 255) / 256;
+        hipLaunchKernelGGL(list_bits_kernel, dim3((unsigned)(lb < 1 ? 1 : (lb > 4096 ? 4096 : lb))), dim3(256), 0, s, row_list, list_offset + n_query, (int)row_list_len, (int)n_query,
+                           n_dst * n_query, node_words, listed_bits, listed_bits + node_words * n_query);
+        HIP_TRY(hipGetLastError());
+    }
     cp.update = update; cp.out = out; cp.rows = n_dst * n_query; cp.row_list = row_list; cp.list_count = list_offset + n_query;
     cp.list_len = (int)row_list_len;
     hipLaunchKernelGGL((combine_kernel<false, 3>), dim3((unsigned)(2 * di->n_cu)), dim3(kCbWaves * 64), lds_cb, s, cp);
@@ -1693,6 +1752,71 @@
     return first_layer_sparse_impl(by_src, src_ptr, fwd_rank, run_prefix, relation, boundary_node, boundary_value, n_query, weight,
                                    bias, ln_weight, ln_bias, ln_eps, relu, shortcut, out, out, row_list, row_list_len, max_runs,
                                    list_offset, n_dst, n_rel, stream);
+}
+
+static int combine_launch(const CombineParams &p, void *stream);
+
+int ultra_first_layer_sparse_const_f32(const ultra_segments *by_src, const int32_t *src_ptr, const int32_t *fwd_rank,
+                                       const int32_t *run_prefix, const float *relation, const int32_t *boundary_node,
+                                       const float *boundary_value, int64_t n_query, const float *weight, const float *bias,
+                                       const float *ln_weight, const float *ln_bias, float ln_eps, int relu, int shortcut,
+                                       float *out, int32_t *row_list, int64_t row_list_len, int64_t max_runs, int32_t *list_offset,
+                                       int64_t n_dst, int64_t n_rel, uint32_t *listed_bits, int64_t listed_words, float *const_vec,
+                                       void *stream) {
+    if (listed_bits == nullptr || const_vec == nullptr) return ULTRA_ERR_NULL_POINTER;
+    if (n_dst <= 0 || n_query <= 0 || listed_words < listed_bits_words(n_dst, n_query)) return ULTRA_ERR_BAD_SHAPE;
+    return first_layer_sparse_impl(by_src, src_ptr, fwd_rank, run_prefix, relation, boundary_node, boundary_value, n_query, weight,
+                                   bias, ln_weight, ln_bias, ln_eps, relu, shortcut, out, out, row_list, row_list_len, max_runs,
+                                   list_offset, n_dst, n_rel, stream, listed_bits, const_vec);
+}
+
+size_t ultra_listed_bits_words(int64_t n_dst, int64_t n_query) {
+    return n_dst > 0 && n_query > 0 ? (size_t)listed_bits_words(n_dst, n_query) : 0;
+}
+
+int ultra_second_layer_const_supported(const ultra_segments *fwd, int64_t n_src, int64_t n_query, int64_t n_rel) {
+    if (fwd == nullptr || !segments_abi_ok(fwd) || check_segments(fwd) != ULTRA_OK) return 0;
+    if (g_force_general || g_no_quad || fwd->dense != nullptr || fwd->packed == nullptr || fwd->packed_src_shift >= 32 ||
+        fwd->n_hot > 0 || fwd->weight != nullptr || (fwd->packed_dead != nullptr && !g_no_dead_words))
+        return 0;
+    if (n_query <= 0 || n_query > kCbLdsQueries || n_rel <= 0 || n_src <= 0 || fwd->n_rows != n_src) return 0;
+    const unsigned long long F = (unsigned long long)n_query * 64ull;
+    const unsigned long long rel_bytes = (unsigned long long)n_rel * kTile * sizeof(float);
+    const unsigned long long bits_bytes = (unsigned long long)(((n_src + 31) / 32 + 3) & ~3LL) * 4ull + kTile * sizeof(float);
+    const unsigned long long x_bytes = (unsigned long long)n_src * kTile * sizeof(float);
+    if (rel_bytes + bits_bytes > (unsigned long long)kMaxLdsBytes) return 0;
+    if (!g_no_x_lds && rel_bytes + x_bytes <= (unsigned long long)kMaxLdsBytes) return 0;
+    if ((unsigned long long)n_src * F * 4ull >= 0xffff0000ull || ((unsigned long long)fwd->n_edges + 16ull) * 4ull >= 0xffff0000ull ||
+        F * 4ull >= (1ull << 24))
+        return 0;
+    return 1;
+}
+
+int ultra_second_layer_const_f32(const ultra_segments *fwd, const float *relation, const float *input, const int32_t *boundary_node,
+                                 const float *boundary_value, const uint32_t *listed_bits, int64_t listed_words,
+                                 const float *const_vec, int64_t n_query, const float *weight, const float *bias,
+                                 const float *ln_weight, const float *ln_bias, float ln_eps, int relu, int shortcut, float *out,
+                                 void *workspace, size_t workspace_bytes, int64_t n_src, int64_t n_rel, void *stream) {
+    if (!ultra_second_layer_const_supported(fwd, n_src, n_query, n_rel)) return ULTRA_ERR_BAD_SHAPE;
+    if (relation == nullptr || input == nullptr || boundary_node == nullptr || boundary_value == nullptr || listed_bits == nullptr ||
+        const_vec == nullptr || weight == nullptr || bias == nullptr || out == nullptr)
+        return ULTRA_ERR_NULL_POINTER;
+    if (ln_weight != nullptr && ln_bias == nullptr) return ULTRA_ERR_NULL_POINTER;
+    if (listed_words < listed_bits_words(n_src, n_query) || input == out) return ULTRA_ERR_BAD_SHAPE;
+    if ((reinterpret_cast<uintptr_t>(const_vec) | reinterpret_cast<uintptr_t>(input)) & 15u) return ULTRA_ERR_BAD_SHAPE;
+    hipStream_t s = static_cast<hipStream_t>(stream);
+    const long long node_words = (n_src + 31) / 32;
+    const long long F = n_query * 64;
+    KParams p{};
+    p.relation = relation; p.input = input; p.bnode = boundary_node; p.bvec = boundary_value; p.bdim = 64; p.out = out;
+    p.act_bits = listed_bits; p.act_words = (int)node_words; p.const_vec = const_vec;
+    int rc = run_plan<KIND_FWD>(fwd, p, n_src, 0, n_rel, F, ULTRA_SUM_ADD, ULTRA_MUL_MUL, true, workspace, workspace_bytes, s);
+    if (rc) return rc;
+    CombineParams cp{};
+    cp.input = input; cp.update = out; cp.weight = weight; cp.bias = bias; cp.gamma = ln_weight; cp.beta = ln_bias;
+    cp.out = out; cp.rows = n_src * n_query; cp.eps = ln_eps; cp.relu = relu; cp.shortcut = shortcut;
+    cp.in_bits = listed_bits + node_words * n_query; cp.in_cvec = const_vec;
+    return combine_launch(cp, stream);
 }
 
 int ultra_first_layer_sparse_train_f32(const ultra_segments *by_src, const int32_t *src_ptr, const int32_t *fwd_rank,
@@ -1889,6 +2013,10 @@
                                     hipFuncAttributeMaxDynamicSharedMemorySize, (int)lds_max));
         HIP_TRY(hipFuncSetAttribute(reinterpret_cast<const void *>(combine_kernel<true, 0, true>),
                                     hipFuncAttributeMaxDynamicSharedMemorySize, (int)lds_max));
+        HIP_TRY(hipFuncSetAttribute(reinterpret_cast<const void *>(combine_kernel<false, 0, false, true>),
+                                    hipFuncAttributeMaxDynamicSharedMemorySize, (int)lds_max));
+        HIP_TRY(hipFuncSetAttribute(reinterpret_cast<const void *>(combine_kernel<true, 0, false, true>),
+                                    hipFuncAttributeMaxDynamicSharedMemorySize, (int)lds_max));
         attr_set[dev] = true;
     }
     const dim3 grid((unsigned)blocks), block(kCbWaves * 64);
@@ -1899,6 +2027,9 @@
     } else if (p.in_bnode != nullptr) {
         if (prefetch) hipLaunchKernelGGL((combine_kernel<true, 2>), grid, block, lds, st, p);
         else hipLaunchKernelGGL((combine_kernel<false, 2>), grid, block, lds, st, p);
+    } else if (p.in_bits != nullptr) {
+        if (prefetch) hipLaunchKernelGGL((combine_kernel<true, 0, false, true>), grid, block, lds, st, p);
+        else hipLaunchKernelGGL((combine_kernel<false, 0, false, true>), grid, block, lds, st, p);
     } else if (p.z_out != nullptr) {
         if (prefetch) hipLaunchKernelGGL((combine_kernel<true, 0, true>), grid, block, lds, st, p);
         else hipLaunchKernelGGL((combine_kernel<false, 0, true>), grid, block, lds, st, p);
diff --git a/ultra_torchdrug_amd/functional.py b/ultra_torchdrug_amd/functional.py
--- a/ultra_torchdrug_amd/functional.py
+++ b/ultra_torchdrug_amd/functional.py
@@ -186,7 +186,7 @@
 
 
 def first_layer_forward(csr, relation, boundary, weight, bias, ln_weight=None, ln_bias=None, ln_eps=1e-5, relu=True,
-                        shortcut=False, want_list=False):
+                        shortcut=False, want_list=False, const_rows=False):
     if not SPARSE_FIRST_LAYER:
         return None
     b_node, b_value = boundary
@@ -213,6 +213,18 @@
     out = torch.empty(n_dst, n_query, 64, dtype=torch.float32, device=dev)
     row_list = torch.empty(n_query * (max_runs + 1), dtype=torch.int32, device=dev)
     list_offset = torch.empty(n_query + 1, dtype=torch.int32, device=dev)
+    if const_rows:
+        listed_bits = torch.empty(int(lib.ultra_listed_bits_words(n_dst, n_query)), dtype=torch.int32, device=dev)
+        const_vec = torch.empty(64, dtype=torch.float32, device=dev)
+        with torch.cuda.device(dev):
+            _lib.check(lib.ultra_first_layer_sparse_const_f32(
+                csr.by_src.pointer, src_ptr.data_ptr(), fwd_rank.data_ptr(), run_prefix.data_ptr(), relation.data_ptr(),
+                b_node.data_ptr(), b_value.data_ptr(), n_query, weight.contiguous().data_ptr(), bias.contiguous().data_ptr(),
+                ln_weight.contiguous().data_ptr() if ln_weight is not None else None,
+                ln_bias.contiguous().data_ptr() if ln_weight is not None else None, float(ln_eps), int(bool(relu)), int(bool(shortcut)),
+                out.data_ptr(), row_list.data_ptr(), row_list.numel(), int(max_runs), list_offset.data_ptr(), n_dst, n_rel,
+                listed_bits.data_ptr(), listed_bits.numel(), const_vec.data_ptr(), _stream()))
+        return out, row_list, list_offset[n_query:], (listed_bits, const_vec)
     with torch.cuda.device(dev):
         _lib.check(lib.ultra_first_layer_sparse_f32(
             csr.by_src.pointer, src_ptr.data_ptr(), fwd_rank.data_ptr(), run_prefix.data_ptr(), relation.data_ptr(),
@@ -294,6 +306,44 @@
                                                   row_list.numel(), n_query, n_src, bitmap.data_ptr(), c_node.data_ptr(),
                                                   sources.data_ptr(), _stream()))
     return sources
+
+
+CONST_SOURCES = __import__("os").environ.get("ULTRA_CONST_SOURCES", "1") != "0"
+
+
+def const_sources_supported(csr, n_query):
+    if not CONST_SOURCES or not SPARSE_FIRST_LAYER:
+        return False
+    n_dst, n_src, n_rel = csr.shape
+    return n_dst == n_src and bool(_lib.load().ultra_second_layer_const_supported(csr.fwd.pointer, n_src, n_query, n_rel))
+
+
+def second_layer_const_forward(csr, relation, input, boundary, const, weight, bias, ln_weight=None, ln_bias=None, ln_eps=1e-5,
+                               relu=True, shortcut=False):
+    n_dst, n_src, n_rel = csr.shape
+    n_query = input.shape[1]
+    listed_bits, const_vec = const
+    b_node, b_value = boundary
+    F = n_query * 64
+    tensors = [relation, input, weight, bias, b_value, const_vec] + ([ln_weight, ln_bias] if ln_weight is not None else [])
+    if (input.dim() != 3 or tuple(input.shape) != (n_src, n_query, 64) or tuple(relation.shape) != (n_rel, F)
+            or tuple(weight.shape) != (64, 128) or tuple(b_value.shape) != (n_query, 64) or b_node.dtype != torch.int32
+            or any(t.dtype != torch.float32 or not t.is_cuda or t.device != input.device for t in tensors)
+            or listed_bits.dtype != torch.int32 or not input.is_contiguous()):
+        raise RuntimeError("second_layer_const_forward: input (%d, %d, 64), relation (%d, %d), fp32 on one HIP device"
+                           % (n_src, n_query, n_rel, F))
+    relation = relation.contiguous()
+    out = torch.empty_like(input)
+    ws, ws_bytes = _workspace(csr.fwd, F, input.device)
+    lib = _lib.load()
+    with torch.cuda.device(input.device):
+        _lib.check(lib.ultra_second_layer_const_f32(
+            csr.fwd.pointer, relation.data_ptr(), input.data_ptr(), b_node.contiguous().data_ptr(), b_value.contiguous().data_ptr(),
+            listed_bits.data_ptr(), listed_bits.numel(), const_vec.data_ptr(), n_query, weight.contiguous().data_ptr(),
+            bias.contiguous().data_ptr(), ln_weight.contiguous().data_ptr() if ln_weight is not None else None,
+            ln_bias.contiguous().data_ptr() if ln_weight is not None else None, float(ln_eps), int(bool(relu)), int(bool(shortcut)),
+            out.data_ptr(), ws.data_ptr() if ws is not None else None, ws_bytes, n_src, n_rel, _stream()))
+    return out
 
 
 def layer_forward(csr, relation, input, boundary, weight, bias, ln_weight=None, ln_bias=None, ln_eps=1e-5, relu=True,
diff --git a/ultra_torchdrug_amd/model.py b/ultra_torchdrug_amd/model.py
--- a/ultra_torchdrug_amd/model.py
+++ b/ultra_torchdrug_amd/model.py
@@ -342,15 +342,23 @@
         n_node = und.num_node
         hidden = None
         listed = None
+        const_rows = len(stack) > 1 and ops.const_sources_supported(csr, n_query)
+        const = None
         for i, entry in enumerate(stack):
             w, b, g, beta, eps, relu = entry["combine"]
             if i == 0:
-                first_out = ops.first_layer_forward(csr, tables[0], boundary, w, b, g, beta, eps, relu, self.short_cut, want_list=True)
-                hidden, listed = (None, None) if first_out is None else (first_out[0], first_out[1:])
+                first_out = ops.first_layer_forward(csr, tables[0], boundary, w, b, g, beta, eps, relu, self.short_cut, want_list=True,
+                                                    const_rows=const_rows)
+                hidden, listed = (None, None) if first_out is None else (first_out[0], first_out[1:3])
+                if first_out is not None and const_rows:
+                    const = first_out[3]
                 if hidden is None:
                     update = ops.rspmm_frontier(csr, tables[0], boundary).view(n_node, n_query, 64)
                     hidden = ops.combine_forward(None, update, w, b, g, beta, eps, relu, self.short_cut, reuse_update=True,
                                                  input_boundary=boundary)
+            elif i == 1 and const is not None:
+                hidden = ops.second_layer_const_forward(csr, tables[i], hidden, boundary, const, w, b, g, beta, eps, relu,
+                                                        self.short_cut)
             else:
                 if i == len(stack) - 1:
                     first, second = self.mlp.layers
```

Result: faster. 44.33 billion (median of 6 runs) (+1.6%).
